# vga-group/tauray

Measured on AMD Instinct MI355X. Metric: Mray/s (closest-hit + shadow rays traced) @1920x1080, 4 bounces, 1 spp, higher is better.
Workload: dtype f32

## Files before the change

include/trhip.h:

```cpp
#ifndef TRHIP_H
#define TRHIP_H
#include <stddef.h>
#include <stdint.h>

#ifdef __cplusplus
extern "C" {
#endif

typedef struct trhip_device trhip_device;
typedef struct trhip_pt trhip_pt;

int trhip_device_create(int hip_device, trhip_device** out);
void trhip_device_destroy(trhip_device* dev);
const char* trhip_last_error(void);
int trhip_malloc(trhip_device* dev, size_t bytes, void** out);
int trhip_free(trhip_device* dev, void* ptr);
int trhip_upload(trhip_device* dev, void* dst_dev, const void* src_host, size_t bytes, void* stream);
int trhip_download(trhip_device* dev, void* dst_host, const void* src_dev, size_t bytes, void* stream);
int trhip_memset(trhip_device* dev, void* dst_dev, int value, size_t bytes, void* stream);
int trhip_sync(trhip_device* dev, void* stream);
int trhip_stream_create(trhip_device* dev, void** stream_out);
int trhip_stream_destroy(trhip_device* dev, void* stream);
int trhip_stream_wait(trhip_device* dev, void* stream, void* on);
int trhip_stream_pipe_class(trhip_device* dev, void* stream, int32_t* pipe_class_out);
// ... 139 lines not shown
    uint64_t stack_overflows;
} trhip_counters;

typedef struct trhip_timings {
    float path_tracing_ms;
    float trace_closest_ms, trace_shadow_ms, shade_ms, raygen_ms, resolve_ms;
    uint32_t trace_closest_launches, trace_shadow_launches, shade_launches, frames;
} trhip_timings;

int trhip_pt_create(trhip_device* dev, const trhip_pt_options* opt, trhip_pt** out);
int trhip_direct_create(trhip_device* dev, const trhip_pt_options* opt, trhip_pt** out);
void trhip_pt_destroy(trhip_pt* pt);
int trhip_pt_set_distribution(trhip_pt* pt, const trhip_distribution* dist);
int trhip_pt_reset_accumulation(trhip_pt* pt, int reset_sample_counter);
int trhip_pt_set_frame_counter(trhip_pt* pt, uint32_t frame_counter);
int trhip_pt_set_frame_batch(trhip_pt* pt, uint32_t frames);
int trhip_pt_set_lanes(trhip_pt* pt, int lanes);
int trhip_pt_set_frame_slots(trhip_pt* pt, int slots);
int trhip_pt_get_lane_pipes(trhip_pt* pt, int32_t* lanes_out, int32_t pipe_classes_out[4]);
int trhip_pt_set_shard(trhip_pt* pt, uint32_t viewport_base, uint32_t viewport_stride, uint32_t sample_base, uint32_t sample_stride);
int trhip_pt_render(trhip_pt* pt, void* color_dev, uint32_t target_w, uint32_t target_h, uint32_t viewports, void* stream);
typedef struct trhip_pt_targets {
    void* color;
    void* diffuse;
    void* reflection;
    void* albedo;
    void* material;
    void* normal;
    void* pos;
    void* instance_id;
    void* screen_motion;
} trhip_pt_targets;
int trhip_pt_render_targets(trhip_pt* pt, const trhip_pt_targets* targets, uint32_t target_w, uint32_t target_h, uint32_t viewports, void* stream);
int trhip_pt_set_shading_arithmetic(trhip_pt* pt, int ieee);
int trhip_pt_set_specialization(trhip_pt* pt, int enable);
int trhip_pt_precompile(const trhip_pt_options* opt, int shade_tris, int ieee, int count_work, const char* arch);
typedef struct trhip_program_info { int32_t kind, ieee; uint64_t identity; char key[240]; } trhip_program_info;
int trhip_pt_get_program(trhip_pt* pt, trhip_program_info* out);
uint64_t trhip_build_id(void);
const char* trhip_kernel_cache_dir(void);
int trhip_pt_set_profiling(trhip_pt* pt, int count_work, int detailed_timing);
int trhip_pt_get_counters(trhip_pt* pt, trhip_counters* out);
int trhip_pt_reset_counters(trhip_pt* pt);
int trhip_pt_get_timings(trhip_pt* pt, trhip_timings* out);
typedef struct trhip_phase_counters {
    uint64_t lane_node_phases, lane_tri_phases, quad_node_phases, quad_tri_phases;
    uint64_t lane_node_phases_le16, lane_node_visits_le16;
    uint64_t lane_node_phase_hist[8];
    uint64_t closest_node_visits;
} trhip_phase_counters;
int trhip_pt_get_phase_counters(trhip_pt* pt, trhip_phase_counters* out);
typedef struct trhip_light_counters { uint64_t sphere_tests, node_visits, walk_fallbacks; } trhip_light_counters;
int trhip_pt_get_light_counters(trhip_pt* pt, trhip_light_counters* out);
int trhip_calibrate_valu(trhip_device* dev, float* ginst_per_s);
int trhip_calibrate_l1(trhip_device* dev, float* gaccesses_per_s);

int trhip_feature_render(trhip_device* dev, int feature, const trhip_distribution* dist, int projection,
                         uint32_t viewport, float min_ray_dist, const float default_value[4],
                         void* color_dev, uint32_t target_w, uint32_t target_h, void* stream);

int trhip_trace_closest(trhip_device* dev, uint32_t n, const void* rays_dev, const void* seeds_dev,
                        int include_lights, void* hits_dev, void* stream);
int trhip_trace_shadow(trhip_device* dev, uint32_t n, const void* rays_dev, void* visibility_dev, void* stream);

int trhip_stitch(trhip_device* dev, const trhip_distribution* partial_dist, const void* partial_dev,
                 uint32_t partial_w, uint32_t partial_h, void* primary_dev, uint32_t viewports,
                 float blend_ratio, void* stream);
int trhip_stitch_batch(trhip_device* dev, uint32_t count, const trhip_distribution* partial_dists, const void* const* partials_dev,
                       const uint32_t* partial_ws, const uint32_t* partial_hs, void* primary_dev, uint32_t viewports,
                       float blend_ratio, void* stream);

typedef struct trhip_tonemap_info {
    int32_t op;
    float exposure, gamma;
    int32_t alpha_grid_background;
} trhip_tonemap_info;
int trhip_tonemap(trhip_device* dev, const void* in_dev, void* out_dev, uint32_t width, uint32_t height,
                  uint32_t layers, const trhip_tonemap_info* info, void* stream);
int trhip_pt_set_fused_tonemap(trhip_pt* pt, void* display_dev, const trhip_tonemap_info* info);

#ifdef __cplusplus
}
#endif
#endif
```

tauray_amd/_lib.py:

```python
from __future__ import annotations

import ctypes as C
import os

os.environ.setdefault("GPU_MAX_HW_QUEUES", "8")
os.environ.setdefault("HSA_ENABLE_IPC_MODE_LEGACY", "0")

_HERE = os.path.dirname(os.path.abspath(__file__))
LIB_PATH = os.environ.get("TRHIP_LIB", os.path.join(_HERE, "libtrhip.so"))


class TrhipError(RuntimeError):
    pass


class SceneDescC(C.Structure):
    _fields_ = [
        ("instances", C.c_void_p), ("spans", C.c_void_p), ("instance_count", C.c_uint32),
        ("vertices", C.c_void_p), ("vertex_count", C.c_uint32),
        ("indices", C.c_void_p), ("index_count", C.c_uint32),
        ("point_lights", C.c_void_p), ("point_light_count", C.c_uint32),
        ("directional_lights", C.c_void_p), ("directional_light_count", C.c_uint32),
        ("texture_infos", C.c_void_p), ("texture_count", C.c_uint32), ("texels", C.c_void_p),
        ("envmap", C.c_void_p), ("envmap_width", C.c_uint32), ("envmap_height", C.c_uint32),
        ("alias_table", C.c_void_p), ("environment_factor", C.c_float * 4),
        ("cameras", C.c_void_p), ("camera_count", C.c_uint32),
        ("non_opaque", C.c_void_p), ("gather_emissive_triangles", C.c_uint32)]


class AccelInfoC(C.Structure):
    _fields_ = [("triangle_count", C.c_uint32), ("node_count", C.c_uint32), ("tri_light_count", C.c_uint32),
                ("build_ms", C.c_float), ("bounds_min", C.c_float * 3), ("bounds_max", C.c_float * 3),
                ("node_bytes", C.c_uint32), ("leaf_count", C.c_uint32)]


class AccelLayoutC(C.Structure):
    _fields_ = [("strategy", C.c_int32), ("blas_count", C.c_uint32), ("tlas_leaf_count", C.c_uint32), ("blas_updated", C.c_uint32),
                ("node_bytes", C.c_uint64), ("record_bytes", C.c_uint64), ("blas_ms", C.c_float), ("tlas_ms", C.c_float)]


AS_ALL_MERGED, AS_PER_MESH, AS_STATIC_MERGED_DYNAMIC_PER_MESH = 0, 1, 2


class LightAccelInfoC(C.Structure):
    _fields_ = [("requested", C.c_int32), ("in_effect", C.c_int32), ("sphere_lights", C.c_uint32), ("tree_lights", C.c_uint32),
                ("node_count", C.c_uint32), ("auto_threshold", C.c_uint32), ("tree_bytes", C.c_uint64), ("last_ms", C.c_float),
                ("last_was_refit", C.c_int32)]


class LightCountersC(C.Structure):
    _fields_ = [("sphere_tests", C.c_uint64), ("node_visits", C.c_uint64), ("walk_fallbacks", C.c_uint64)]


LIGHT_ACCEL_AUTO, LIGHT_ACCEL_LOOP, LIGHT_ACCEL_TREE = 0, 1, 2


class PtOptionsC(C.Structure):
    _fields_ = [
        ("max_bounces", C.c_int32), ("min_ray_dist", C.c_float), ("rng_seed", C.c_uint32), ("sampler", C.c_int32),
        ("samples_per_pixel", C.c_int32), ("samples_per_pass", C.c_int32), ("projection", C.c_int32),
        ("film", C.c_int32), ("film_radius", C.c_float), ("mis_mode", C.c_int32),
        ("russian_roulette_delta", C.c_float), ("indirect_clamping", C.c_float), ("regularization_gamma", C.c_float),
        ("depth_of_field", C.c_int32), ("nee_point", C.c_float), ("nee_directional", C.c_float),
        ("nee_envmap", C.c_float), ("nee_triangles", C.c_float), ("bounce_mode", C.c_int32),
        ("tri_light_mode", C.c_int32), ("hide_lights", C.c_int32), ("use_white_albedo_on_first_bounce", C.c_int32),
        ("transparent_background", C.c_int32), ("pre_transformed_vertices", C.c_int32)]


class DistributionC(C.Structure):
    _fields_ = [("size_x", C.c_uint32), ("size_y", C.c_uint32), ("strategy", C.c_int32),
                ("index", C.c_uint32), ("count", C.c_uint32), ("primary", C.c_uint32)]


class CountersC(C.Structure):
    _fields_ = [(n, C.c_uint64) for n in ("closest_rays", "shadow_rays", "node_visits", "tri_tests", "alpha_tests",
                                          "surface_hits", "stack_overflows")]


class TimingsC(C.Structure):
    _fields_ = ([(n, C.c_float) for n in ("path_tracing_ms", "trace_closest_ms", "trace_shadow_ms", "shade_ms", "raygen_ms", "resolve_ms")]
                + [(n, C.c_uint32) for n in ("trace_closest_launches", "trace_shadow_launches", "shade_launches", "frames")])


class PhaseCountersC(C.Structure):
    _fields_ = ([(n, C.c_uint64) for n in ("lane_node_phases", "lane_tri_phases", "quad_node_phases", "quad_tri_phases",
                                           "lane_node_phases_le16", "lane_node_visits_le16")] + [("lane_node_phase_hist", C.c_uint64 * 8),
                                                                                                 ("closest_node_visits", C.c_uint64)])


class ProgramInfoC(C.Structure):
    _fields_ = [("kind", C.c_int32), ("ieee", C.c_int32), ("identity", C.c_uint64), ("key", C.c_char * 240)]


class PtTargetsC(C.Structure):
    _fields_ = [(n, C.c_void_p) for n in ("color", "diffuse", "reflection", "albedo", "material", "normal", "pos", "instance_id", "screen_motion")]


class TonemapInfoC(C.Structure):
    _fields_ = [("op", C.c_int32), ("exposure", C.c_float), ("gamma", C.c_float), ("alpha_grid_background", C.c_int32)]


_vp, _u32, _i, _f = C.c_void_p, C.c_uint32, C.c_int, C.c_float
SYMBOLS = {
    "trhip_image_decode": (_i, [_vp, C.c_size_t, C.POINTER(_u32), C.POINTER(_u32), C.POINTER(_u32), C.POINTER(C.POINTER(C.c_uint8))]),
    "trhip_image_free": (None, [C.POINTER(C.c_uint8)]),
    "trhip_exr_decode": (_i, [_vp, C.c_size_t, C.POINTER(_u32), C.POINTER(_u32), C.POINTER(_u32), C.POINTER(C.POINTER(C.c_float))]),
    "trhip_exr_encode": (_i, [_vp, _u32, _u32, _i, _i, _i, C.POINTER(C.POINTER(C.c_uint8)), C.POINTER(C.c_size_t)]),
    "trhip_exr_free": (None, [_vp]),
    "trhip_device_create": (_i, [_i, C.POINTER(_vp)]),
    "trhip_device_destroy": (None, [_vp]),
    "trhip_last_error": (C.c_char_p, []),
    "trhip_malloc": (_i, [_vp, C.c_size_t, C.POINTER(_vp)]),
    "trhip_image_decode_texels": (_i, [C.c_char_p, C.c_size_t, C.POINTER(C.c_uint32), C.POINTER(C.c_uint32), C.POINTER(C.c_uint32), C.POINTER(C.c_uint32), C.POINTER(C.POINTER(C.c_uint8))]),
    "trhip_free": (_i, [_vp, _vp]),
    "trhip_upload": (_i, [_vp, _vp, _vp, C.c_size_t, _vp]),
    "trhip_download": (_i, [_vp, _vp, _vp, C.c_size_t, _vp]),
    "trhip_memset": (_i, [_vp, _vp, _i, C.c_size_t, _vp]),
    "trhip_sync": (_i, [_vp, _vp]),
    "trhip_copy_peer": (_i, [_vp, _vp, _vp, _vp, C.c_size_t, _vp]),
    "trhip_scene_upload": (_i, [_vp, C.POINTER(SceneDescC)]),
    "trhip_scene_update_cameras": (_i, [_vp, _vp, _u32]),
    "trhip_scene_set_previous_cameras": (_i, [_vp, _vp, _u32]),
    "trhip_scene_update_instances": (_i, [_vp, _vp, _u32]),
    "trhip_scene_build_accel": (_i, [_vp, C.POINTER(AccelInfoC)]),
    "trhip_scene_refit_accel": (_i, [_vp, C.POINTER(AccelInfoC)]),
    "trhip_pt_set_frame_batch": (_i, [_vp, C.c_uint32]),
    "trhip_scene_update_lights": (_i, [_vp, _vp, C.c_uint32, _vp, C.c_uint32]),
    "trhip_scene_set_build_mode": (_i, [_vp, _i]),
    "trhip_scene_set_accel_strategy": (_i, [_vp, _i]),
    "trhip_scene_set_dynamic_instances": (_i, [_vp, _vp, _u32]),
    "trhip_scene_get_accel_layout": (_i, [_vp, C.POINTER(AccelLayoutC)]),
    "trhip_scene_set_light_accel": (_i, [_vp, _i]),
    "trhip_scene_get_light_accel": (_i, [_vp, C.POINTER(LightAccelInfoC)]),
    "trhip_pt_get_light_counters": (_i, [_vp, C.POINTER(LightCountersC)]),
    "trhip_stitch_batch": (_i, [_vp, _u32, _vp, _vp, _vp, _vp, _vp, _u32, C.c_float, _vp]),
    "trhip_stream_create": (_i, [_vp, C.POINTER(C.c_void_p)]),
    "trhip_stream_destroy": (_i, [_vp, _vp]),
    "trhip_stream_pipe_class": (_i, [_vp, _vp, C.POINTER(C.c_int32)]),
    "trhip_device_get_info": (_i, [_vp, _vp]),
    "trhip_build_id": (C.c_uint64, []),
    "trhip_stream_wait": (_i, [_vp, _vp, _vp]),
    "trhip_stream_wait_peer": (_i, [_vp, _vp, _vp, _vp]),
    "trhip_pt_set_frame_counter": (_i, [_vp, _u32]),
    "trhip_pt_set_lanes": (_i, [_vp, C.c_int]),
    "trhip_pt_set_frame_slots": (_i, [_vp, C.c_int]),
    "trhip_pt_set_fused_tonemap": (_i, [_vp, _vp, _vp]),
    "trhip_pt_get_lane_pipes": (_i, [_vp, C.POINTER(C.c_int32), C.POINTER(C.c_int32)]),
    "trhip_pt_set_shading_arithmetic": (_i, [_vp, C.c_int]),
    "trhip_pt_set_specialization": (_i, [_vp, C.c_int]),
    "trhip_pt_precompile": (_i, [C.POINTER(PtOptionsC), C.c_int, C.c_int, C.c_int, C.c_char_p]),
    "trhip_kernel_cache_dir": (C.c_char_p, []),
    "trhip_pt_set_shard": (_i, [_vp, _u32, _u32, _u32, _u32]),
    "trhip_scene_set_skin": (_i, [_vp, _u32, _vp, _vp, _u32]),
    "trhip_scene_skin": (_i, [_vp, _u32, _vp, _u32]),
    "trhip_scene_get_vertices": (_i, [_vp, _u32, _vp, _u32]),
    "trhip_scene_get_tri_lights": (_i, [_vp, _vp, _u32]),
    "trhip_pt_create": (_i, [_vp, C.POINTER(PtOptionsC), C.POINTER(_vp)]),
    "trhip_direct_create": (_i, [_vp, C.POINTER(PtOptionsC), C.POINTER(_vp)]),
    "trhip_pt_destroy": (None, [_vp]),
    "trhip_pt_set_distribution": (_i, [_vp, C.POINTER(DistributionC)]),
    "trhip_pt_reset_accumulation": (_i, [_vp, _i]),
    "trhip_pt_render": (_i, [_vp, _vp, _u32, _u32, _u32, _vp]),
    "trhip_pt_render_targets": (_i, [_vp, C.POINTER(PtTargetsC), _u32, _u32, _u32, _vp]),
    "trhip_pt_set_profiling": (_i, [_vp, _i, _i]),
    "trhip_pt_get_counters": (_i, [_vp, C.POINTER(CountersC)]),
    "trhip_pt_reset_counters": (_i, [_vp]),
    "trhip_pt_get_timings": (_i, [_vp, C.POINTER(TimingsC)]),
    "trhip_pt_get_phase_counters": (_i, [_vp, C.POINTER(PhaseCountersC)]),
    "trhip_pt_get_program": (_i, [_vp, C.POINTER(ProgramInfoC)]),
    "trhip_calibrate_valu": (_i, [_vp, C.POINTER(C.c_float)]),
    "trhip_calibrate_l1": (_i, [_vp, C.POINTER(C.c_float)]),
    "trhip_feature_render": (_i, [_vp, _i, C.POINTER(DistributionC), _i, _u32, _f, C.POINTER(_f), _vp, _u32, _u32, _vp]),
    "trhip_trace_closest": (_i, [_vp, _u32, _vp, _vp, _i, _vp, _vp]),
    "trhip_trace_shadow": (_i, [_vp, _u32, _vp, _vp, _vp]),
    "trhip_stitch": (_i, [_vp, C.POINTER(DistributionC), _vp, _u32, _u32, _vp, _u32, _f, _vp]),
    "trhip_tonemap": (_i, [_vp, _vp, _vp, _u32, _u32, _u32, C.POINTER(TonemapInfoC), _vp]),
}

_LIB = None


def lib():
    global _LIB
    if _LIB is None:
        if not os.path.exists(LIB_PATH):
            raise TrhipError(f"{LIB_PATH} is missing: build it with `make -C tauray_amd/csrc` (or __graft_entry__.build())")
        L = C.CDLL(LIB_PATH)
# ... 17 lines not shown
```

tauray_amd/csrc/api.hip:

```cpp
#include <cstdlib>
#include <cstring>
#include <mutex>
#include <string>
#include <vector>

#include "pt.h"
#include "trace.h"
#include "trace_quad.h"
#include "specialize.h"
#include "tonemap.h"
#include "../../include/tauray_image.hh"
#include "../../include/tauray_exr.hh"

namespace tr {

static thread_local std::string g_error;
int set_error(const std::string& msg) { g_error = msg; return 1; }

#define HIPCHK(x) do { hipError_t e_ = (x); if (e_ != hipSuccess) return set_error(std::string(#x) + ": " + hipGetErrorString(e_)); } while (0)

namespace {

constexpr int KB = TR_BLOCK;

// ... 72 lines not shown
            asm volatile("global_load_dwordx4 %0, %1, off" : "=v"(v[u]) : "v"(q) : "memory");
        }
        asm volatile("s_waitcnt vmcnt(0)" ::: "memory");
#pragma unroll
        for (int u = 0; u < 8; ++u) acc += v[u];
    }
    if (acc.x == 123.456f) out[0] = acc.y + acc.z + acc.w;
}

template <bool TWO_LEVEL>
__global__ __launch_bounds__(KB) void k_query_closest(SceneView sv, uint n, const float* rays, const uint* seeds, int include_lights,
                                                      HitRecord* out, uint* overflow_flag, int* qspill) {
    __shared__ int s_stack_rows[TR_STACK_WORDS];
    int* const s_stack = s_stack_rows + TR_STACK_ROW0;
    __shared__ int s_owner[(KB / 64) * TR_OWNER_WORDS];
    int* my_stack = s_stack + threadIdx.x;
    QuadCtx qc;
    qc.wave_stack = s_stack + (threadIdx.x & ~63u);
    qc.owner_tab = s_owner + (threadIdx.x >> 6) * TR_OWNER_WORDS;
    qc.spill = qspill + ((size_t)blockIdx.x * (KB / 64) + (threadIdx.x >> 6)) * (16u * TR_QSPILL);
    int overflow = 0;
    TraceStats st = {};
    for (uint base = blockIdx.x * KB; base < n; base += gridDim.x * KB) {
        const uint i = base + threadIdx.x;
        const bool valid = i < n;
        float r[8] = {0, 0, 0, 0, 0, 0, 0, 0};
        if (valid) for (int k = 0; k < 8; ++k) r[k] = rays[(size_t)i * 8 + k];
        const uint seed = (valid && seeds) ? seeds[i] : 0u;
        HitRecord hit;
#if TR_QUAD_SWITCH > 0
        if (seeds) trace_closest_wave4<0, false, TWO_LEVEL>(sv, valid, F3(r[0], r[1], r[2]), F3(r[4], r[5], r[6]), r[3], r[7], seed, my_stack, qc, hit, st, overflow);
        else trace_closest_wave4<1, false, TWO_LEVEL>(sv, valid, F3(r[0], r[1], r[2]), F3(r[4], r[5], r[6]), r[3], r[7], 0u, my_stack, qc, hit, st, overflow);
#else
        if (valid) {
            if (seeds) trace_closest4<0, false, TWO_LEVEL>(sv, F3(r[0], r[1], r[2]), F3(r[4], r[5], r[6]), r[3], r[7], seed, my_stack, hit, st, overflow);
            else trace_closest4<1, false, TWO_LEVEL>(sv, F3(r[0], r[1], r[2]), F3(r[4], r[5], r[6]), r[3], r[7], 0u, my_stack, hit, st, overflow);
        }
#endif
        if (valid) out[i] = hit;
        if (valid && include_lights) {
            const float tri_t = hit.instance_id >= 0 ? hit.t : r[7];
            uint ri = i;
            asm volatile("" : "+v"(ri));
            const float* q = rays + (size_t)ri * 8;
            const f3 o = F3(q[0], q[1], q[2]), d = F3(q[4], q[5], q[6]);
            if (ray_is_finite(o, d)) {
                const LightHit lh = trace_sphere_lights<false>(sv, o, d, q[3], tri_t, my_stack, st);
                if (lh.light >= 0) out[ri] = HitRecord{-1, lh.light, lh.t, 0.0f, lh.t};
            }
        }
    }
    if (overflow) *overflow_flag = 1;
}
template <bool TWO_LEVEL>
__global__ __launch_bounds__(KB) void k_query_shadow(SceneView sv, uint n, const float* rays, float* out, uint* overflow_flag) {
    __shared__ int s_stack_rows[TR_STACK_WORDS];
    int* const s_stack = s_stack_rows + TR_STACK_ROW0;
    int overflow = 0;
    TraceStats st = {};
    for (uint i = blockIdx.x * KB + threadIdx.x; i < n; i += gridDim.x * KB) {
        const float* r = rays + (size_t)i * 8;
        out[i] = trace_shadow4<false, TWO_LEVEL>(sv, F3(r[0], r[1], r[2]), F3(r[4], r[5], r[6]), r[3], r[7], s_stack + threadIdx.x, st, overflow);
    }
    if (overflow) *overflow_flag = 1;
}

__global__ __launch_bounds__(KB) void k_stitch(LaunchCtx L, const f4* partial, uint pw, uint ph, f4* primary, uint viewports, float blend_ratio) {
    uint per_view = L.strategy == 2 ? L.launch_w : pw * ph;
    uint i = blockIdx.x * KB + threadIdx.x;
    if (i >= per_view * viewports) return;
    uint z = i / per_view, p = i % per_view;
    uint sx, sy, ox, oy;
    if (L.strategy == 2) {
        uint j = permute_region_id(L.index + p, L.size_x, L.size_y, L.count);
        if (j >= L.size_x * L.size_y) return;
        sx = p % L.size_x; sy = p / L.size_x;
        ox = j % L.size_x; oy = j / L.size_x;
    } else {
        sx = p % pw; sy = p / pw;
        ox = sx; oy = sy * L.count + L.index;
        if (oy >= L.size_y) return;
    }
    f4 c = partial[((size_t)z * ph + sy) * pw + sx];
    size_t o = ((size_t)z * L.size_y + oy) * L.size_x + ox;
    if (blend_ratio < 1.0f) c = mix4(primary[o], c, blend_ratio);
    primary[o] = c;
}

#define TR_STITCH_BATCH 15
struct StitchBatch { LaunchCtx L[TR_STITCH_BATCH]; const f4* partial[TR_STITCH_BATCH]; uint pw[TR_STITCH_BATCH], ph[TR_STITCH_BATCH]; };
__global__ __launch_bounds__(KB) void k_stitch_batch(StitchBatch B, f4* primary, uint viewports, float blend_ratio) {
    const uint e = blockIdx.y;
    const LaunchCtx L = B.L[e];
    const uint pw = B.pw[e], ph = B.ph[e];
    const f4* partial = B.partial[e];
    uint per_view = L.strategy == 2 ? L.launch_w : pw * ph;
    uint i = blockIdx.x * KB + threadIdx.x;
    if (i >= per_view * viewports) return;
    uint z = i / per_view, p = i % per_view;
    uint sx, sy, ox, oy;
    if (L.strategy == 2) {
        uint j = permute_region_id(L.index + p, L.size_x, L.size_y, L.count);
        if (j >= L.size_x * L.size_y) return;
        sx = p % L.size_x; sy = p / L.size_x;
        ox = j % L.size_x; oy = j / L.size_x;
    } else {
// ... 573 lines not shown
    return 0;
}
int trhip_pt_set_fused_tonemap(trhip_pt* pt, void* display_dev, const trhip_tonemap_info* info) {
    if (!pt) return set_error("null trhip_pt");
    if (display_dev && !info) return set_error("trhip_pt_set_fused_tonemap: null info");
    if (display_dev && pt->stage->direct) return set_error("trhip_pt_set_fused_tonemap: the direct stage resolves its samples in a kernel of its own; run trhip_tonemap");
    pt->stage->tm_display = display_dev;
    if (info) { pt->stage->tm_info = *info; if (info->op == 0) pt->stage->tm_info.gamma = 1.0f; }
    return 0;
}
int trhip_pt_get_lane_pipes(trhip_pt* pt, int32_t* lanes_out, int32_t pipe_classes_out[4]) {
    if (!pt || !lanes_out || !pipe_classes_out) return set_error("trhip_pt_get_lane_pipes: null argument");
    *lanes_out = pt->stage->last_lanes;
    for (int l = 0; l < 4; ++l) pipe_classes_out[l] = l < pt->stage->last_lanes ? pt->stage->last_lane_pipes[l] : -1;
    return 0;
}
int trhip_pt_set_shading_arithmetic(trhip_pt* pt, int ieee) {
    if (!pt) return set_error("null trhip_pt");
    pt->stage->ieee_shading = ieee ? 1 : 0;
    return 0;
}
int trhip_pt_set_specialization(trhip_pt* pt, int enable) {
    if (!pt) return set_error("null trhip_pt");
    pt->stage->specialize = enable ? 1 : 0;
    return 0;
}
int trhip_pt_precompile(const trhip_pt_options* opt, int shade_tris, int ieee, int count_work, const char* arch) {
    if (!opt) return set_error("trhip_pt_precompile: null options");
    if (is_cli_default_set(*opt) && shade_tris) return 0;
    SpecRequest rq{*opt, shade_tris != 0 && !opt->pre_transformed_vertices, ieee != 0, count_work != 0, SPEC_SHADE, false};
    std::string why;
    for (int program : {SPEC_SHADE, SPEC_RAYGEN}) {
        rq.program = program;
        if (spec_precompile(rq, arch, &why)) return set_error("trhip_pt_precompile: " + why);
    }
    return 0;
}
const char* trhip_kernel_cache_dir(void) {
    static const std::string dir = spec_cache_dir();
    return dir.c_str();
}
int trhip_pt_set_profiling(trhip_pt* pt, int count_work, int detailed_timing) {
    if (!pt) return set_error("null trhip_pt");
    pt->stage->count_work = count_work; pt->stage->detailed_timing = detailed_timing;
    return 0;
}
int trhip_pt_get_counters(trhip_pt* pt, trhip_counters* out) { if (!pt) return set_error("null trhip_pt"); DEVCHK(pt->dev); return pt->stage->get_counters(out, pt->stage->last_stream); }
int trhip_pt_get_light_counters(trhip_pt* pt, trhip_light_counters* out) {
    if (!pt) return set_error("null trhip_pt");
    if (!out) return set_error("trhip_pt_get_light_counters: null output");
    DEVCHK(pt->dev);
    return pt->stage->get_light_counters(out, pt->stage->last_stream);
}
int trhip_pt_reset_counters(trhip_pt* pt) { if (!pt) return set_error("null trhip_pt"); DEVCHK(pt->dev); HIPCHK(hipStreamSynchronize(pt->stage->last_stream)); return pt->stage->reset_counters(); }
int trhip_pt_get_timings(trhip_pt* pt, trhip_timings* out) { if (!pt) return set_error("null trhip_pt"); DEVCHK(pt->dev); return pt->stage->get_timings(out); }
int trhip_pt_get_program(trhip_pt* pt, trhip_program_info* out) { if (!pt) return set_error("null trhip_pt"); if (!out) return set_error("trhip_pt_get_program: null out"); DEVCHK(pt->dev); return pt->stage->get_program(out); }
int trhip_pt_get_phase_counters(trhip_pt* pt, trhip_phase_counters* out) { if (!pt) return set_error("null trhip_pt"); DEVCHK(pt->dev); return pt->stage->get_phase_counters(out, pt->stage->last_stream); }

int trhip_calibrate_valu(trhip_device* dev, float* ginst_per_s) {
    DEVCHK(dev);
    if (!ginst_per_s) return set_error("trhip_calibrate_valu: null out");
    int cus = 256;
    HIPCHK(hipDeviceGetAttribute(&cus, hipDeviceAttributeMultiprocessorCount, dev->hip_device));
    const int blocks = cus * 8, iters = 4096;
    hipEvent_t a, b;
    HIPCHK(hipEventCreate(&a)); HIPCHK(hipEventCreate(&b));
    float best = 0.0f;
    for (int rep = 0; rep < 4; ++rep) {
        HIPCHK(hipEventRecord(a, nullptr));
        hipLaunchKernelGGL(k_calibrate_fma, dim3(blocks), dim3(KB), 0, nullptr, reinterpret_cast<float*>(dev->overflow_flag), iters, 1.0001f, 0.5f);
        HIPCHK(hipEventRecord(b, nullptr));
        HIPCHK(hipEventSynchronize(b));
        float ms = 0;
        HIPCHK(hipEventElapsedTime(&ms, a, b));
        const float g = (float)((double)blocks * (KB / 64) * (double)iters * 64.0 / ((double)ms * 1e6));
        if (rep > 0 && g > best) best = g;
    }
    (void)hipEventDestroy(a); (void)hipEventDestroy(b);
    *ginst_per_s = best;
    return 0;
}

int trhip_calibrate_l1(trhip_device* dev, float* gaccesses_per_s) {
    DEVCHK(dev);
    if (!gaccesses_per_s) return set_error("trhip_calibrate_l1: null out");
    int cus = 256;
    HIPCHK(hipDeviceGetAttribute(&cus, hipDeviceAttributeMultiprocessorCount, dev->hip_device));
    const int blocks = cus * 4, iters = 400;
    char* buf = nullptr;
    HIPCHK(hipMalloc(&buf, 16384 + 64));
    HIPCHK(hipMemset(buf, 0, 16384 + 64));
    hipEvent_t a, b;
    HIPCHK(hipEventCreate(&a)); HIPCHK(hipEventCreate(&b));
    float best = 0.0f;
    for (int rep = 0; rep < 4; ++rep) {
        HIPCHK(hipEventRecord(a, nullptr));
        hipLaunchKernelGGL(k_calibrate_l1, dim3(blocks), dim3(KB), 0, nullptr, buf, iters, reinterpret_cast<float*>(dev->overflow_flag));
        HIPCHK(hipEventRecord(b, nullptr));
        HIPCHK(hipEventSynchronize(b));
        float ms = 0;
        HIPCHK(hipEventElapsedTime(&ms, a, b));
        const float g = (float)((double)blocks * (KB / 64) * (double)iters * 8.0 * 64.0 / ((double)ms * 1e6));
        if (rep > 0 && g > best) best = g;
    }
    (void)hipEventDestroy(a); (void)hipEventDestroy(b);
    (void)hipFree(buf);
    *gaccesses_per_s = best;
    return 0;
}

static LaunchCtx make_launch(const trhip_distribution& d) {
    LaunchCtx L{};
    uint lw, lh;
    get_ray_count(d, lw, lh);
    L.size_x = d.size_x; L.size_y = d.size_y; L.strategy = d.strategy; L.index = d.index; L.primary = d.primary;
    L.count = d.count;
    if (d.strategy == 2) { uint n = d.size_x * d.size_y, b = 31; while ((n >> b) < 128 && b > 0) b--; L.count = b; }
    L.launch_w = lw; L.launch_h = lh;
    return L;
}

int trhip_feature_render(trhip_device* dev, int feature, const trhip_distribution* dist, int projection, uint32_t viewport,
                         float min_ray_dist, const float default_value[4], void* color_dev, uint32_t target_w, uint32_t target_h, void* stream) {
    DEVCHK(dev);
    if (!dev->scene.accel_built) return set_error("trhip_feature_render: call trhip_scene_build_accel first");
    if (viewport >= dev->scene.camera_count) return set_error("trhip_feature_render: viewport out of range");
    LaunchCtx L = make_launch(*dist);
    size_t n = (size_t)L.launch_w * L.launch_h;
    if (n == 0) return 0;
    f4 dv = F4(default_value[0], default_value[1], default_value[2], default_value[3]);
    hipLaunchKernelGGL(dev->scene.two_level ? k_feature<true> : k_feature<false>, dim3((uint)((n + KB - 1) / KB)), dim3(KB), 0, (hipStream_t)stream, dev->scene.view(), L, feature, projection,
                       viewport, min_ray_dist, dv, (f4*)color_dev, target_w, target_h, dev->overflow_flag);
    HIPCHK(hipGetLastError());
    return 0;
}

int trhip_trace_closest(trhip_device* dev, uint32_t n, const void* rays_dev, const void* seeds_dev, int include_lights, void* hits_dev, void* stream) {
    DEVCHK(dev);
    if (!dev->scene.accel_built) return set_error("trhip_trace_closest: call trhip_scene_build_accel first");
    if (n == 0) return 0;
    uint blocks = std::min((n + KB - 1) / KB, QUERY_BLOCKS);
    if (!dev->qspill) HIPCHK(hipMalloc(&dev->qspill, (size_t)QUERY_BLOCKS * (KB / 64) * 16u * TR_QSPILL * sizeof(int)));
    hipLaunchKernelGGL(dev->scene.two_level ? k_query_closest<true> : k_query_closest<false>, dim3(blocks), dim3(KB), 0, (hipStream_t)stream, dev->scene.view(), n, (const float*)rays_dev,
                       (const uint*)seeds_dev, include_lights, (HitRecord*)hits_dev, dev->overflow_flag, dev->qspill);
    HIPCHK(hipGetLastError());
    return 0;
}
int trhip_trace_shadow(trhip_device* dev, uint32_t n, const void* rays_dev, void* visibility_dev, void* stream) {
    DEVCHK(dev);
    if (!dev->scene.accel_built) return set_error("trhip_trace_shadow: call trhip_scene_build_accel first");
    if (n == 0) return 0;
    uint blocks = std::min((n + KB - 1) / KB, 2048u);
    hipLaunchKernelGGL(dev->scene.two_level ? k_query_shadow<true> : k_query_shadow<false>, dim3(blocks), dim3(KB), 0, (hipStream_t)stream, dev->scene.view(), n, (const float*)rays_dev,
                       (float*)visibility_dev, dev->overflow_flag);
    HIPCHK(hipGetLastError());
    return 0;
}

int trhip_stitch(trhip_device* dev, const trhip_distribution* pd, const void* partial_dev, uint32_t pw, uint32_t ph, void* primary_dev,
                 uint32_t viewports, float blend_ratio, void* stream) {
    DEVCHK(dev);
    if (!pd || pd->strategy == 0) return set_error("trhip_stitch: needs a scanline or shuffled-strips partial");
    LaunchCtx L = make_launch(*pd);
    size_t per_view = pd->strategy == 2 ? L.launch_w : (size_t)pw * ph;
    size_t n = per_view * viewports;
    if (n == 0) return 0;
    hipLaunchKernelGGL(k_stitch, dim3((uint)((n + KB - 1) / KB)), dim3(KB), 0, (hipStream_t)stream, L, (const f4*)partial_dev, pw, ph,
                       (f4*)primary_dev, viewports, blend_ratio);
    HIPCHK(hipGetLastError());
    return 0;
}

int trhip_stitch_batch(trhip_device* dev, uint32_t count, const trhip_distribution* pds, const void* const* partials_dev, const uint32_t* pws,
                       const uint32_t* phs, void* primary_dev, uint32_t viewports, float blend_ratio, void* stream) {
    DEVCHK(dev);
    if (count == 0) return 0;
    if (!pds || !partials_dev || !pws || !phs) return set_error("trhip_stitch_batch: null argument");
    for (uint32_t first = 0; first < count; first += TR_STITCH_BATCH) {
        const uint32_t m = std::min<uint32_t>(TR_STITCH_BATCH, count - first);
        StitchBatch B{};
        size_t n_max = 0;
        for (uint32_t k = 0; k < m; ++k) {
            const trhip_distribution& pd = pds[first + k];
            if (pd.strategy == 0) return set_error("trhip_stitch_batch: needs scanline or shuffled-strips partials");
            B.L[k] = make_launch(pd);
            B.partial[k] = (const f4*)partials_dev[first + k]; B.pw[k] = pws[first + k]; B.ph[k] = phs[first + k];
            const size_t per_view = pd.strategy == 2 ? B.L[k].launch_w : (size_t)B.pw[k] * B.ph[k];
            n_max = std::max(n_max, per_view * viewports);
        }
        if (n_max == 0) continue;
        hipLaunchKernelGGL(k_stitch_batch, dim3((uint)((n_max + KB - 1) / KB), m), dim3(KB), 0, (hipStream_t)stream, B, (f4*)primary_dev, viewports,
                           blend_ratio);
    }
    HIPCHK(hipGetLastError());
    return 0;
}

int trhip_tonemap(trhip_device* dev, const void* in_dev, void* out_dev, uint32_t width, uint32_t height, uint32_t layers,
                  const trhip_tonemap_info* info, void* stream) {
    DEVCHK(dev);
// ... 12 lines not shown
```

tauray_amd/csrc/build.h:

```cpp
#pragma once
#include <string>
#include <vector>

#include "common.h"
#include "shading.h"

namespace tr {

int set_error(const std::string& msg);

struct DeviceScene {
    Instance* instances = nullptr;
    MeshSpan* spans = nullptr;
    Vertex* vertices = nullptr;
    uint* indices = nullptr;
    PointLight* point_lights = nullptr;
    DirectionalLight* directional_lights = nullptr;
    TextureInfo* tex_infos = nullptr;
    uint8_t* texels = nullptr;
    f4* envmap = nullptr;
    AliasEntry* alias_table = nullptr;
    CameraData* cameras = nullptr;
    CameraData* prev_cameras = nullptr;
    uint8_t* non_opaque = nullptr;
// ... 22 lines not shown
    uint build_rounds = 0;
    int ploc_radius = 16;
    int optimise_rounds = 8;
    uint leaf_count = 0;
    uint accel_tri_count = 0;
    bool collapse_by_cost = true;
    bool fast_build = false;
    int optimise_modulus = 1;
    int dfs_layout = 1;
    bool accel_built = false;
    uint accel_capacity = 0xFFFFFFFFu;
    void* scratch = nullptr;
    float bounds_lo[3] = {0, 0, 0}, bounds_hi[3] = {0, 0, 0};
    uint* level_nodes = nullptr;
    float* node_bounds = nullptr;
    std::vector<uint> level_offsets;
    bool levels_valid = false;
    size_t scratch_bytes = 0;
    int accel_strategy = TRHIP_AS_ALL_MERGED;
    std::vector<uint8_t> dynamic_marks;
    std::vector<Instance> host_instances;
    struct Blas {
        int root;
        uint node_off, node_slots, tri_off, tri_count;
        uint rep;
        bool world;
    };
    std::vector<Blas> blases;
    std::vector<int> inst_blas;
    std::vector<uint> tlas_src;
    std::vector<uint8_t> blas_dirty;
    bool static_dirty = false;
    std::vector<uint8_t> alpha_dirty;
    uint* alpha_list = nullptr;
    size_t alpha_list_words = 0;
    bool two_level = false;
    TlasLeaf* tlas = nullptr;
    TlasLeaf* tlas_src_leaves = nullptr;
    uint tlas_leaf_count = 0, tlas_node_slots = 0, tlas_capacity = 0;
    size_t node_capacity = 0, tri_capacity = 0;
    trhip_accel_layout layout = {};
    std::vector<uint> host_alpha_base;
    std::vector<uint8_t> host_non_opaque;
    void* tl_aux = nullptr;
    size_t tl_aux_bytes = 0;
    int light_accel_requested = -1;
    int light_in_effect = TRHIP_LIGHT_ACCEL_LOOP;
    std::vector<PointLight> host_point_lights;
    std::vector<uint> light_tree_set;
    std::vector<Bvh4Node> light_nodes;
    uint light_tree_nodes = 0;
    float light_ms = 0.0f;
    int light_last_refit = -1;

    SceneView view() const {
        SceneView v;
        v.instances = instances; v.spans = spans; v.vertices = vertices; v.indices = indices;
        v.point_lights = point_lights; v.directional_lights = directional_lights; v.tri_lights = tri_lights;
        v.tex_infos = tex_infos; v.texels = texels; v.envmap = envmap; v.alias_table = alias_table;
        v.cameras = cameras; v.prev_cameras = prev_cameras ? prev_cameras : cameras; v.obj_spans = spans; v.obj_vertices = vertices; v.shade_tris = shade_tris; v.shade_tangents = shade_tangents; v.tris = tris; v.alpha_tris = alpha_tris; v.nodes4 = nodes4;
        v.environment_factor = environment_factor; v.environment_proj = environment_proj;
        v.instance_count = instance_count; v.point_light_count = point_light_count;
        v.directional_light_count = directional_light_count; v.tri_light_count = tri_light_count;
        v.env_w = env_w; v.env_h = env_h; v.wide_textures = wide_textures; v.tri_count = accel_built ? tri_count : 0; v.node_count = node_count;
        return v;
    }
    void free_accel() {
        if (nodes) (void)hipFree(nodes);
        if (nodes4) (void)hipFree(nodes4);
        if (tris) (void)hipFree(tris);
        if (tri_lights) (void)hipFree(tri_lights);
        if (tlas_src_leaves) (void)hipFree(tlas_src_leaves);
        if (tl_aux) (void)hipFree(tl_aux);
        tl_aux = nullptr; tl_aux_bytes = 0;
        if (alpha_list) (void)hipFree(alpha_list);
        alpha_list = nullptr; alpha_list_words = 0; alpha_dirty.clear();
        tlas = nullptr; tlas_src_leaves = nullptr; tlas_capacity = 0; node_capacity = 0; tri_capacity = 0; two_level = false;
        blases.clear(); inst_blas.clear(); tlas_src.clear(); blas_dirty.clear(); static_dirty = false;
        nodes = nullptr; nodes4 = nullptr; tris = nullptr; tri_lights = nullptr; node_count = 0; tri_light_count = 0; accel_built = false;
        accel_capacity = 0xFFFFFFFFu;
        if (level_nodes) (void)hipFree(level_nodes);
        if (node_bounds) (void)hipFree(node_bounds);
        level_nodes = nullptr; node_bounds = nullptr; level_offsets.clear(); levels_valid = false;
    }
    struct SkinSlot { Vertex* source = nullptr; Skin* skins = nullptr; m4* joints = nullptr; uint joint_capacity = 0; uint vertex_count = 0; };
    std::vector<SkinSlot> skin_slots;
    void free_skins() {
        for (SkinSlot& k : skin_slots) { if (k.source) (void)hipFree(k.source); if (k.skins) (void)hipFree(k.skins); if (k.joints) (void)hipFree(k.joints); }
        skin_slots.clear();
    }
    void free_all() {
        free_accel();
        free_skins();
        void* ptrs[] = {instances, spans, vertices, indices, point_lights, directional_lights, tex_infos, texels, envmap,
                        alias_table, cameras, prev_cameras, non_opaque, tri_prefix, world_spans, world_vertices, scratch, shade_tris, alpha_base, alpha_tris};
        for (void* p : ptrs) if (p) (void)hipFree(p);
        const int strategy = accel_strategy, light_mode = light_accel_requested;
        *this = DeviceScene();
        accel_strategy = strategy;
        light_accel_requested = light_mode;
    }
};

int build_accel(DeviceScene& ds, hipStream_t stream, trhip_accel_info* info);
int ensure_world_vertices(DeviceScene& ds, hipStream_t stream);
int build_shade_tris(DeviceScene& ds, int instance, hipStream_t stream);
int skin_instance(DeviceScene& ds, uint instance, const float* joint_transforms, uint joint_count, hipStream_t stream);
int refit_accel(DeviceScene& ds, hipStream_t stream, trhip_accel_info* info);
void mark_skinned(DeviceScene& ds, uint instance);
int update_light_accel(DeviceScene& ds, bool moved);
uint light_accel_auto_threshold();
int light_accel_requested(const DeviceScene& ds);

}
```

tauray_amd/csrc/bvh_build.hip:

```cpp
#include <algorithm>
#include <cctype>
#include <chrono>
#include <cmath>
#include <map>
#include <tuple>
#include <vector>
#include "build.h"

#include <rocprim/rocprim.hpp>

namespace tr {

namespace {

constexpr int BT = 256;

TR_DEV uint float_flip(float f) { uint u = __float_as_uint(f); return (u & 0x80000000u) ? ~u : (u | 0x80000000u); }
TR_HD float float_unflip(uint u) {
    uint v = (u & 0x80000000u) ? (u & 0x7FFFFFFFu) : ~u;
    float f;
#if defined(__HIP_DEVICE_COMPILE__)
    f = __uint_as_float(v);
#else
    memcpy(&f, &v, 4);
// ... 378 lines not shown
    if (dec) ncand = collapse_children(children, dec, (int)i, cand);
    while (!dec && ncand < W) {
        int best = -1; float best_area = -1.0f;
        for (int c = 0; c < ncand; ++c) {
            if (cand[c] < 0) continue;
            const float* b = node_box + 6 * (size_t)cand[c];
            float dx = b[3] - b[0], dy = b[4] - b[1], dz = b[5] - b[2];
            float area = dx * dy + dy * dz + dz * dx;
            if (area > best_area) { best_area = area; best = c; }
        }
        if (best < 0) break;
        const int2 ch = children[cand[best]];
        cand[best] = ch.x; cand[ncand++] = ch.y;
    }
    Bvh4Node out;
    for (int c = 0; c < 4; ++c) {
        if (c < ncand) {
            const float* b = cand[c] >= 0 ? node_box + 6 * (size_t)cand[c] : leaf_box + 6 * (size_t)(~cand[c]);
            out.lox[c] = b[0]; out.loy[c] = b[1]; out.loz[c] = b[2]; out.hix[c] = b[3]; out.hiy[c] = b[4]; out.hiz[c] = b[5];
            out.child[c] = cand[c] >= 0 ? new_id[cand[c]] : cand[c];
        } else {
            out.lox[c] = out.loy[c] = out.loz[c] = __builtin_huge_valf();
            out.hix[c] = out.hiy[c] = out.hiz[c] = -__builtin_huge_valf();
            out.child[c] = 0x7FFFFFFF;
        }
        out.pad[c] = 0;
    }
    nodes4[(size_t)new_id[i]] = out;
}

__global__ __launch_bounds__(BT) void k_extract_tri_lights(SceneView sv, const uint* tri_prefix, TriLight* out) {
    uint gid = blockIdx.x * BT + threadIdx.x;
    if (gid >= sv.tri_count) return;
    uint inst, prim;
    locate_triangle(tri_prefix, sv.instance_count, gid, inst, prim);
    const Instance& o = sv.instances[inst];
    if (o.light_base_id < 0) return;
    const MeshSpan sp = sv.spans[inst];
    const uint* ix = sv.indices + sp.index_offset + 3u * prim;
    const Vertex* vb = sv.vertices + sp.vertex_offset;
    const Vertex v0 = vb[ix[0]], v1 = vb[ix[1]], v2 = vb[ix[2]];
    TriLight l;
    l.emission_tex_id = o.mat.emission_tex_id;
    l.emission_factor = rgb_to_r9g9b9e5(F3(o.mat.emission_factor));
    l.instance_id = inst;
    l.primitive_id = prim;
    l.pos[0] = transform_point(o.model, v0.pos);
    l.pos[1] = transform_point(o.model, v1.pos);
    l.pos[2] = transform_point(o.model, v2.pos);
    l.uv[0] = pack_half2x16(v0.uv); l.uv[1] = pack_half2x16(v1.uv); l.uv[2] = pack_half2x16(v2.uv);
    out[(uint)o.light_base_id + prim] = l;
}

#define HIPCHK(x) do { hipError_t e_ = (x); if (e_ != hipSuccess) return set_error(std::string(#x) + ": " + hipGetErrorString(e_)); } while (0)

}

__global__ __launch_bounds__(BT) void k_pre_transform_vertices(uint vertex_count, const Instance* instance, const Vertex* in, Vertex* out) {
    uint i = blockIdx.x * BT + threadIdx.x;
    if (i >= vertex_count) return;
    const m4 model = instance->model;
    const m3 mn = upper3(instance->model_normal);
    const float det = mn.c[0].x * (mn.c[1].y * mn.c[2].z - mn.c[2].y * mn.c[1].z)
                    - mn.c[1].x * (mn.c[0].y * mn.c[2].z - mn.c[2].y * mn.c[0].z)
                    + mn.c[2].x * (mn.c[0].y * mn.c[1].z - mn.c[1].y * mn.c[0].z);
    Vertex v = in[i];
    v.pos = transform_point(model, v.pos);
    v.normal = normalize(mul(mn, v.normal));
    f3 t = normalize(mul(mn, F3(v.tangent)));
    v.tangent = F4(t, v.tangent.w);
    if (det < 0) { v.normal = -v.normal; v.tangent = F4(-t.x, -t.y, -t.z, -v.tangent.w); }
    out[i] = v;
}

int ensure_world_vertices(DeviceScene& ds, hipStream_t stream) {
    if (ds.world_vertices || ds.world_vertex_count == 0) return 0;
    HIPCHK(hipMalloc(&ds.world_vertices, (size_t)ds.world_vertex_count * sizeof(Vertex)));
    for (uint i = 0; i < ds.instance_count; ++i) {
        const MeshSpan& sp = ds.host_spans[i];
        if (sp.vertex_count == 0) continue;
        hipLaunchKernelGGL(k_pre_transform_vertices, dim3((sp.vertex_count + BT - 1) / BT), dim3(BT), 0, stream, sp.vertex_count, ds.instances + i,
                           ds.vertices + sp.vertex_offset, ds.world_vertices + ds.host_world_spans[i].vertex_offset);
    }
    HIPCHK(hipGetLastError());
    return 0;
}

__global__ __launch_bounds__(BT) void k_skinning(uint vertex_count, const Vertex* source, const Skin* skins, const m4* joints, uint joint_count, Vertex* destination) {
    uint i = blockIdx.x * BT + threadIdx.x;
    if (i >= vertex_count) return;
    const Skin s = skins[i];
    float a[4][4];
    for (int c = 0; c < 4; ++c) {
        f4 col = F4(0);
        for (int k = 0; k < 4; ++k) {
            const uint j = s.joints[k] < joint_count ? s.joints[k] : 0u;
            const f4 t = joints[j].c[c] * s.weights[k];
            col = k == 0 ? t : col + t;
        }
        a[0][c] = col.x; a[1][c] = col.y; a[2][c] = col.z; a[3][c] = col.w;
    }
    const float s0 = a[0][0] * a[1][1] - a[1][0] * a[0][1], s1 = a[0][0] * a[1][2] - a[1][0] * a[0][2], s2 = a[0][0] * a[1][3] - a[1][0] * a[0][3];
    const float s3 = a[0][1] * a[1][2] - a[1][1] * a[0][2], s4 = a[0][1] * a[1][3] - a[1][1] * a[0][3], s5 = a[0][2] * a[1][3] - a[1][2] * a[0][3];
    const float c5 = a[2][2] * a[3][3] - a[3][2] * a[2][3], c4 = a[2][1] * a[3][3] - a[3][1] * a[2][3], c3 = a[2][1] * a[3][2] - a[3][1] * a[2][2];
    const float c2 = a[2][0] * a[3][3] - a[3][0] * a[2][3], c1 = a[2][0] * a[3][2] - a[3][0] * a[2][2], c0 = a[2][0] * a[3][1] - a[3][0] * a[2][1];
    const float det = s0 * c5 - s1 * c4 + s2 * c3 + s3 * c2 - s4 * c1 + s5 * c0;
    float inv[3][3];
    inv[0][0] = ( a[1][1] * c5 - a[1][2] * c4 + a[1][3] * c3) / det;
    inv[0][1] = (-a[0][1] * c5 + a[0][2] * c4 - a[0][3] * c3) / det;
    inv[0][2] = ( a[3][1] * s5 - a[3][2] * s4 + a[3][3] * s3) / det;
    inv[1][0] = (-a[1][0] * c5 + a[1][2] * c2 - a[1][3] * c1) / det;
    inv[1][1] = ( a[0][0] * c5 - a[0][2] * c2 + a[0][3] * c1) / det;
    inv[1][2] = (-a[3][0] * s5 + a[3][2] * s2 - a[3][3] * s1) / det;
    inv[2][0] = ( a[1][0] * c4 - a[1][1] * c2 + a[1][3] * c0) / det;
    inv[2][1] = (-a[0][0] * c4 + a[0][1] * c2 - a[0][3] * c0) / det;
    inv[2][2] = ( a[3][0] * s4 - a[3][1] * s2 + a[3][3] * s0) / det;
    const Vertex src = source[i];
    Vertex dst = src;
    dst.pos = F3(a[0][0] * src.pos.x + a[0][1] * src.pos.y + a[0][2] * src.pos.z + a[0][3],
                 a[1][0] * src.pos.x + a[1][1] * src.pos.y + a[1][2] * src.pos.z + a[1][3],
                 a[2][0] * src.pos.x + a[2][1] * src.pos.y + a[2][2] * src.pos.z + a[2][3]);
    const f3 n = src.normal, t = F3(src.tangent);
    dst.normal = normalize(F3(inv[0][0] * n.x + inv[1][0] * n.y + inv[2][0] * n.z + 0.0f, inv[0][1] * n.x + inv[1][1] * n.y + inv[2][1] * n.z + 0.0f,
                              inv[0][2] * n.x + inv[1][2] * n.y + inv[2][2] * n.z + 0.0f));
    const f3 tt = normalize(F3(inv[0][0] * t.x + inv[1][0] * t.y + inv[2][0] * t.z + 0.0f, inv[0][1] * t.x + inv[1][1] * t.y + inv[2][1] * t.z + 0.0f,
// ... 144 lines not shown
int refit_accel(DeviceScene& ds, hipStream_t stream, trhip_accel_info* info) {
    if (ds.two_level) {
        if (ds.accel_tri_count != ds.tri_count || ds.tlas_capacity != ds.tlas_leaf_count)
            return set_error("trhip_scene_refit_accel: no acceleration structure to refit; call trhip_scene_build_accel first");
        return refit_two_level(ds, stream, info);
    }
    const uint n = ds.leaf_count;
    if (ds.accel_tri_count != ds.tri_count || ds.accel_capacity == 0xFFFFFFFFu || (n > 0 && !ds.tris) || (n > 1 && !ds.nodes4))
        return set_error("trhip_scene_refit_accel: no acceleration structure to refit; call trhip_scene_build_accel first");
    hipEvent_t e0, e1;
    HIPCHK(hipEventCreate(&e0)); HIPCHK(hipEventCreate(&e1));
    HIPCHK(hipEventRecord(e0, stream));
    SceneView sv = ds.view();
    const uint n1 = ds.node_count;
    if (n1 > 0 && !ds.levels_valid) {
        if (!ds.level_nodes) HIPCHK(hipMalloc(&ds.level_nodes, (size_t)n1 * 4));
        if (!ds.node_bounds) HIPCHK(hipMalloc(&ds.node_bounds, (size_t)n1 * 24));
        uint* counter = nullptr;
        HIPCHK(hipMalloc(&counter, 4));
        const uint root = 0;
        HIPCHK(hipMemcpyAsync(ds.level_nodes, &root, 4, hipMemcpyHostToDevice, stream));
        ds.level_offsets.assign(1, 0u);
        uint begin = 0, count = 1;
        while (count > 0) {
            ds.level_offsets.push_back(begin + count);
            if (begin + count >= n1) break;
            HIPCHK(hipMemsetAsync(counter, 0, 4, stream));
            hipLaunchKernelGGL(k_expand_level, dim3((count + BT - 1) / BT), dim3(BT), 0, stream, count, ds.level_nodes + begin, ds.nodes4,
                               ds.level_nodes + begin + count, counter);
            uint next = 0;
            HIPCHK(hipMemcpyAsync(&next, counter, 4, hipMemcpyDeviceToHost, stream));
            HIPCHK(hipStreamSynchronize(stream));
            begin += count; count = next;
            if (ds.level_offsets.size() > 4096) { (void)hipFree(counter); return set_error("trhip_scene_refit_accel: hierarchy too deep"); }
        }
        (void)hipFree(counter);
        ds.levels_valid = true;
        if (getenv("TRHIP_DEBUG"))
            fprintf(stderr, "[trhip] 4-wide tree: %u live nodes of %u slots in %zu levels, %.3f children per node\n", ds.level_offsets.back(), n1,
                    ds.level_offsets.size() - 1, (double)(n + ds.level_offsets.back() - 1) / (double)ds.level_offsets.back());
    }
    if (n > 0) hipLaunchKernelGGL(k_retransform, dim3((n + BT - 1) / BT), dim3(BT), 0, stream, sv, n, ds.tris, ds.alpha_base, ds.alpha_tris);
    for (size_t l = ds.level_offsets.size(); l-- > 1;) {
        const uint lo = ds.level_offsets[l - 1], cnt = ds.level_offsets[l] - lo;
        if (cnt) hipLaunchKernelGGL(k_refit_level, dim3((cnt + BT - 1) / BT), dim3(BT), 0, stream, cnt, ds.level_nodes + lo, ds.nodes4, ds.tris, ds.node_bounds);
    }
    HIPCHK(hipGetLastError());
    ds.accel_built = true;
    if (ds.gather_emissive_triangles && ds.host_tri_light_count > 0 && ds.tri_lights) {
        HIPCHK(hipMemsetAsync(ds.tri_lights, 0, (size_t)ds.host_tri_light_count * sizeof(TriLight), stream));
        SceneView sv2 = ds.view();
        hipLaunchKernelGGL(k_extract_tri_lights, dim3((ds.tri_count + BT - 1) / BT), dim3(BT), 0, stream, sv2, ds.tri_prefix, ds.tri_lights);
    }
    HIPCHK(hipEventRecord(e1, stream));
    HIPCHK(hipEventSynchronize(e1));
    float ms = 0;
    HIPCHK(hipEventElapsedTime(&ms, e0, e1));
    (void)hipEventDestroy(e0); (void)hipEventDestroy(e1);
    ds.layout.blas_updated = 1; ds.layout.blas_ms = ms;
    if (info) {
        memset(info, 0, sizeof(*info));
        info->triangle_count = ds.tri_count; info->leaf_count = n; info->node_count = ds.node_count; info->node_bytes = 112u; info->tri_light_count = ds.tri_light_count;
        info->build_ms = ms;
        for (int k = 0; k < 3; ++k) { info->bounds_min[k] = ds.bounds_lo[k]; info->bounds_max[k] = ds.bounds_hi[k]; }
    }
    return 0;
}

static int reorder_into_treelets(DeviceScene& ds, hipStream_t stream, uint n_nodes, uint n_tris, uint treelet_nodes, bool reorder_tris) {
    if (n_nodes == 0 || n_tris == 0) return 0;
    HIPCHK(hipStreamSynchronize(stream));
    std::vector<Bvh4Node> nodes(n_nodes), out_nodes;
    std::vector<TriRecord> tris(n_tris), out_tris;
    HIPCHK(hipMemcpy(nodes.data(), ds.nodes4, (size_t)n_nodes * sizeof(Bvh4Node), hipMemcpyDeviceToHost));
    HIPCHK(hipMemcpy(tris.data(), ds.tris, (size_t)n_tris * sizeof(TriRecord), hipMemcpyDeviceToHost));
    std::vector<int> new_id(n_nodes, -1);
    std::vector<uint> order;
    order.reserve(n_nodes);
    std::vector<uint> roots = {0u};
    auto area = [&](const Bvh4Node& nd, int c) {
        const float dx = nd.hix[c] - nd.lox[c], dy = nd.hiy[c] - nd.loy[c], dz = nd.hiz[c] - nd.loz[c];
        return dx * dy + dy * dz + dz * dx;
    };
    std::vector<std::pair<float, uint>> heap;
    while (!roots.empty()) {
        const uint root = roots.back(); roots.pop_back();
        heap.clear();
        heap.push_back({__builtin_huge_valf(), root});
        uint taken = 0;
        std::vector<uint> rest;
        while (!heap.empty()) {
            std::pop_heap(heap.begin(), heap.end());
            const uint nd = heap.back().second; heap.pop_back();
            if (taken >= treelet_nodes) { rest.push_back(nd); continue; }
            new_id[nd] = (int)order.size(); order.push_back(nd); taken++;
            for (int c = 0; c < 4; ++c) {
                const int ch = nodes[nd].child[c];
                if (ch >= 0 && ch != 0x7FFFFFFF) { heap.push_back({area(nodes[nd], c), (uint)ch}); std::push_heap(heap.begin(), heap.end()); }
            }
        }
        for (size_t k = rest.size(); k-- > 0;) roots.push_back(rest[k]);
    }
    out_nodes.resize(n_nodes);
    std::vector<int> new_tri(n_tris, -1);
    uint next_tri = 0;
    for (size_t k = 0; k < order.size(); ++k) {
// ... 289 lines not shown
                const uint8_t* dec = nullptr;
                if (dp_collapse) {
                    OptTree t{(uint)(n - 1), n, children, node_box, leaf_box, reinterpret_cast<int*>(base + o_uparent)};
                    if (!optimise) hipLaunchKernelGGL(k_opt_parents, dim3(iblocks), dim3(BT), 0, stream, t);
                    HIPCHK(hipMemsetAsync(arrive, 0, (size_t)(n - 1) * 4, stream));
                    hipLaunchKernelGGL(k_collapse_cost, dim3(blocks), dim3(BT), 0, stream, t, arrive, reinterpret_cast<float*>(base + o_ccost), reinterpret_cast<uint8_t*>(base + o_cdec));
                    dec = reinterpret_cast<const uint8_t*>(base + o_cdec);
                }
                hipLaunchKernelGGL(k_collapse4, dim3(iblocks), dim3(BT), 0, stream, n - 1, children, node_box, leaf_box, new_id, dec, out_nodes);
            }
        }
        HIPCHK(hipGetLastError());
        if (experiments && getenv("TRHIP_PAIR_LEAVES") && atoi(getenv("TRHIP_PAIR_LEAVES")) != 0 && n > 2) {
#if TR_PAIR_LEAVES
            if (int rc = pair_leaves_postpass(ds, stream, n - 1, n)) return rc;
#else
            return set_error("TRHIP_PAIR_LEAVES needs a library built with -DTR_PAIR_LEAVES=1 (the traversal has to know the pair references)");
#endif
        }
        if (const char* e = experiments ? getenv("TRHIP_TREELET") : nullptr) {
            if (n > 2 && atoi(e) > 0) if (int rc = reorder_into_treelets(ds, stream, n - 1, n, (uint)atoi(e), !getenv("TRHIP_TREELET_KEEP_TRIS"))) return rc;
        }
    }
    return 0;
}

static int build_two_level(DeviceScene& ds, hipStream_t stream, trhip_accel_info* info);
static int refit_two_level(DeviceScene& ds, hipStream_t stream, trhip_accel_info* info);

int build_accel(DeviceScene& ds, hipStream_t stream, trhip_accel_info* info) {
    if (ds.accel_strategy != TRHIP_AS_ALL_MERGED) return build_two_level(ds, stream, info);
    const uint n_scene = ds.tri_count;
    hipEvent_t e0, e1;
    HIPCHK(hipEventCreate(&e0)); HIPCHK(hipEventCreate(&e1));
    HIPCHK(hipEventRecord(e0, stream));
    ds.accel_built = false;
    ds.levels_valid = false;
    SceneView sv = ds.view();
    sv.tri_count = n_scene;
    const uint n_tri = n_scene;
    const uint n_cap = n_tri;
    uint n = n_tri;
    const size_t n1 = n_cap > 1 ? n_cap - 1 : 0;
    if (ds.two_level) ds.free_accel();
    TreePlan P;
    if (int rc = plan_tree(ds, stream, n_cap, P)) return rc;
    uint* cbounds = P.cbounds();
    {
        const uint init[32] = {0xFFFFFFFFu, 0xFFFFFFFFu, 0xFFFFFFFFu, 0, 0, 0, 0, 0, 0, 0, 0, 0, 0, 0, 0, 0, 0xFFFFFFFFu, 0xFFFFFFFFu, 0xFFFFFFFFu, 0, 0, 0, 0, 0, 0, 0, 0, 0, 0, 0, 0, 0};
        HIPCHK(hipMemcpyAsync(cbounds, init, sizeof(init), hipMemcpyHostToDevice, stream));
    }
    if (ds.accel_capacity != n_cap) {
        ds.free_accel();
        if (n_cap > 0) HIPCHK(hipMalloc(&ds.tris, (size_t)n_cap * sizeof(TriRecord)));
        if (n1 > 0) {
            if ((uint64_t)n1 * sizeof(Bvh4Node) > 0xFFFFFFFFull) return set_error("trhip_scene_build_accel: more than 2^25 nodes");
            HIPCHK(hipMalloc(&ds.nodes4, n1 * sizeof(Bvh4Node)));
        }
        ds.accel_capacity = n_cap;
    }
    if (n_tri > 0) {
        TriRecord* unsorted = P.unsorted();
        const uint tblocks = (n_tri + BT - 1) / BT;
        hipLaunchKernelGGL(k_pretransform, dim3(tblocks < 1024u ? tblocks : 1024u), dim3(BT), 0, stream, sv, ds.tri_prefix, ds.non_opaque, ds.alpha_base, ds.alpha_tris, unsorted, cbounds);
    }
    if (int rc = build_tree(ds, stream, P, n, ds.tris, ds.nodes4, true)) return rc;
    ds.leaf_count = n;
    ds.node_count = n > 1 ? n - 1 : 0;
    ds.accel_tri_count = n_tri;
    ds.accel_built = true;
    ds.tri_light_count = 0;
    if (ds.gather_emissive_triangles && ds.host_tri_light_count > 0) {
        if (!ds.tri_lights) HIPCHK(hipMalloc(&ds.tri_lights, (size_t)ds.host_tri_light_count * sizeof(TriLight)));
        HIPCHK(hipMemsetAsync(ds.tri_lights, 0, (size_t)ds.host_tri_light_count * sizeof(TriLight), stream));
        ds.tri_light_count = ds.host_tri_light_count;
        SceneView sv2 = ds.view();
        hipLaunchKernelGGL(k_extract_tri_lights, dim3((n_tri + BT - 1) / BT), dim3(BT), 0, stream, sv2, ds.tri_prefix, ds.tri_lights);
        HIPCHK(hipGetLastError());
    }
    HIPCHK(hipEventRecord(e1, stream));
    HIPCHK(hipEventSynchronize(e1));
    float ms = 0;
    HIPCHK(hipEventElapsedTime(&ms, e0, e1));
    (void)hipEventDestroy(e0); (void)hipEventDestroy(e1);
    uint hb[6];
    HIPCHK(hipMemcpy(hb, cbounds, sizeof(hb), hipMemcpyDeviceToHost));
    for (int k = 0; k < 3; ++k) { ds.bounds_lo[k] = float_unflip(hb[k]); ds.bounds_hi[k] = float_unflip(hb[3 + k]); }
    ds.layout = {};
    ds.layout.strategy = TRHIP_AS_ALL_MERGED; ds.layout.blas_count = 1; ds.layout.blas_updated = 1;
    ds.layout.node_bytes = (uint64_t)ds.node_count * sizeof(Bvh4Node); ds.layout.record_bytes = (uint64_t)n * sizeof(TriRecord);
    ds.layout.blas_ms = ms;
    if (info) {
        info->triangle_count = n_tri;
        info->leaf_count = n;
        info->node_count = ds.node_count;
        info->node_bytes = 112u;
        info->tri_light_count = ds.tri_light_count;
        info->build_ms = ms;
        for (int k = 0; k < 3; ++k) { info->bounds_min[k] = float_unflip(hb[k]); info->bounds_max[k] = float_unflip(hb[3 + k]); }
    }
    return 0;
}

namespace {

__global__ __launch_bounds__(BT) void k_group_records(SceneView sv, const uint* list, const uint* prefix, uint n_list, uint n, int world,
                                                      const uint8_t* non_opaque, const uint* alpha_base, AlphaTri* alpha_tris, TriRecord* out) {
    const uint gid = blockIdx.x * BT + threadIdx.x;
    if (gid >= n) return;
    uint slot, prim;
    locate_triangle(prefix, n_list, gid, slot, prim);
    const uint inst = list[slot];
    const MeshSpan sp = sv.obj_spans[inst];
    const uint* ix = sv.indices + sp.index_offset + 3u * prim;
    const Vertex* vb = sv.obj_vertices + sp.vertex_offset;
    f3 p0 = vb[ix[0]].pos, p1 = vb[ix[1]].pos, p2 = vb[ix[2]].pos;
    TriRecord t;
    if (world) {
        const m4 model = sv.instances[inst].model;
        p0 = transform_point(model, p0); p1 = transform_point(model, p1); p2 = transform_point(model, p2);
        t.inst_flags = inst | (non_opaque[inst] ? 0x80000000u : 0u);
        t.alpha = non_opaque[inst] ? alpha_word(sv.instances[inst].mat, alpha_base[inst] + prim, alpha_tris, vb[ix[0]].uv, vb[ix[1]].uv, vb[ix[2]].uv) : 0u;
    } else {
        t.inst_flags = inst;
        t.alpha = 0u;
    }
    t.prim = prim;
    t.v0[0] = p0.x; t.v0[1] = p0.y; t.v0[2] = p0.z;
    t.v1[0] = p1.x; t.v1[1] = p1.y; t.v1[2] = p1.z;
    t.v2[0] = p2.x; t.v2[1] = p2.y; t.v2[2] = p2.z;
    out[gid] = t;
}
// ... 615 lines not shown
```

tauray_amd/csrc/common.h:

```cpp
#pragma once
#include <hip/hip_runtime.h>
#include <hip/hip_fp16.h>
#include <stdint.h>
#include <string.h>
#include <cstring>

#include "../../include/trhip.h"

#define TR_DEV __device__ __forceinline__
#define TR_HD __host__ __device__ __forceinline__

namespace tr {

typedef uint32_t uint;

struct f2 { float x, y; };
struct f3 { float x, y, z; };
struct f4 { float x, y, z, w; };
struct u4 { uint x, y, z, w; };
struct u2 { uint x, y; };

TR_HD f2 F2(float a, float b) { return {a, b}; }
TR_HD f2 F2(float a) { return {a, a}; }
TR_HD f3 F3(float a, float b, float c) { return {a, b, c}; }
// ... 132 lines not shown
#define TR_INST_FROM_RECORD 0xFFFFFFFFu
#define TR_TLAS_IDENTITY 1u
struct alignas(64) TlasLeaf {
    float xf[12];
    int blas_root;
    uint inst_word;
    uint alpha_base;
    uint flags;
};
static_assert(sizeof(TlasLeaf) == 64, "TLAS leaf layout");

struct SceneView {
    const Instance* instances;
    const MeshSpan* spans;
    const Vertex* vertices;
    const uint* indices;
    const PointLight* point_lights;
    const DirectionalLight* directional_lights;
    const TriLight* tri_lights;
    const TextureInfo* tex_infos;
    const uint8_t* texels;
    const f4* envmap;
    const AliasEntry* alias_table;
    const CameraData* cameras;
    const CameraData* prev_cameras;
    const MeshSpan* obj_spans;
    const Vertex* obj_vertices;
    const ShadeTri* shade_tris;
    const f4* shade_tangents;
    const TriRecord* tris;
    const AlphaTri* alpha_tris;
    const Bvh4Node* nodes4;
    f4 environment_factor;
    int environment_proj;
    uint instance_count, point_light_count, directional_light_count, tri_light_count;
    uint env_w, env_h;
    uint tri_count, node_count;
    uint wide_textures;
};
TR_HD const TlasLeaf* tlas_leaves(const SceneView& sv) { return reinterpret_cast<const TlasLeaf*>(sv.nodes4 + sv.node_count); }

#define TR_LIGHT_KAPPA 0.001953125f
struct alignas(16) LightTreeHeader { uint use_tree, node_count, leaf_count, pad; };
static_assert(sizeof(LightTreeHeader) == 16, "light tree header layout");
TR_HD size_t light_tree_node_offset(uint point_light_count) { return ((size_t)point_light_count * sizeof(PointLight) + sizeof(LightTreeHeader) + 127) & ~(size_t)127; }
TR_HD size_t light_allocation_bytes(uint point_light_count) {
    return light_tree_node_offset(point_light_count) + (size_t)(point_light_count > 1 ? point_light_count - 1 : 1) * sizeof(Bvh4Node);
}
TR_HD const LightTreeHeader* light_tree_header(const SceneView& sv) { return reinterpret_cast<const LightTreeHeader*>(sv.point_lights + sv.point_light_count); }
TR_HD const Bvh4Node* light_tree_nodes(const SceneView& sv) {
    return reinterpret_cast<const Bvh4Node*>(reinterpret_cast<const char*>(sv.point_lights) + light_tree_node_offset(sv.point_light_count));
}

}
```

tauray_amd/csrc/path_tracer.hip:

```cpp
#include <cstdio>
#include <cstdlib>
#include <type_traits>
#include <vector>

#include "pt_kernels.h"
#include "resolve_kernel.h"
#include "specialize.h"
#include "build_id.inc"

namespace tr {

namespace {

#ifndef TR_CLOSEST_WAVES
#define TR_CLOSEST_WAVES 6
#endif
#ifndef TR_SHADOW_WAVES
#define TR_SHADOW_WAVES 8
#endif
#ifndef TR_CLOSEST_WAVES_2L
#define TR_CLOSEST_WAVES_2L 5
#endif
#ifndef TR_SHADOW_WAVES_2L
#define TR_SHADOW_WAVES_2L 6
#endif

template <bool COUNT, bool SOLO, bool WIDE = true, bool TWO_LEVEL = false>
__global__ __launch_bounds__(KB, TWO_LEVEL ? TR_CLOSEST_WAVES_2L : TR_CLOSEST_WAVES) void k_trace_closest(SceneView sv, PtParams P, PathBuffers pb, int bounce, const uint* queue,
                                                      uint* bc) {
    if (!WIDE) sv.wide_textures = 0;
    __shared__ int s_stack_rows[TR_STACK_WORDS];
    int* const s_stack = s_stack_rows + TR_STACK_ROW0;
    __shared__ int s_owner[(KB / 64) * TR_OWNER_WORDS];
    TL(__shared__ uint s_tl[(KB / 64) * TL_WORDS]; for (uint i = threadIdx.x; i < (KB / 64) * TL_WORDS; i += KB) s_tl[i] = 0; __syncthreads();)
    const QuadCtx qc = make_quad_ctx(s_stack, s_owner, pb TL(, s_tl));
    const uint n = queue ? bc[BC_QUEUE] : P.n_ids;
    TraceStats st = {};
    uint rays = 0, max_vis = 0;
    int overflow = 0;
    const uint wave_id = (blockIdx.x * KB + threadIdx.x) >> 6, n_waves = (gridDim.x * KB) >> 6;
    bool first = true;
    while (true) {
        uint base = 0;
        if (first) base = wave_id * 64u;
        else {
            if (n <= n_waves * 64u) break;
            if ((threadIdx.x & 63) == 0) base = n_waves * 64u + atomicAdd(&bc[BC_CUR_CLOSEST], 64u);
            base = __shfl(base, 0);
        }
        first = false;
        if (base >= n) break;
        closest_lane<COUNT, TWO_LEVEL>(sv, P, pb, bounce, queue, base + (threadIdx.x & 63), n, s_stack + threadIdx.x, qc, st, overflow, max_vis, rays);
    }
    flush_trace_counters<COUNT>(P, pb, overflow, 1000 + bounce, rays, 0u, st, max_vis);
    TL(__syncthreads(); for (uint i = threadIdx.x; i < (KB / 64) * TL_WORDS; i += KB) if (s_tl[i]) atomicAdd(&g_timeline[i % TL_WORDS], (unsigned long long)s_tl[i]);)
}

template <bool COUNT, bool WIDE = true, bool TWO_LEVEL = false>
__global__ __launch_bounds__(KB, TWO_LEVEL ? TR_SHADOW_WAVES_2L : TR_SHADOW_WAVES) void k_trace_shadow(SceneView sv, PtParams P, PathBuffers pb, uint* bc) {
    if (!WIDE) sv.wide_textures = 0;
    __shared__ int s_stack_rows[TR_STACK_WORDS];
    int* const s_stack = s_stack_rows + TR_STACK_ROW0;
    __shared__ int s_owner[(KB / 64) * TR_OWNER_WORDS];
    const QuadCtx qc = make_quad_ctx(s_stack, s_owner, pb);
    const uint n = bc[BC_SHADOW];
    TraceStats st = {};
    uint rays = 0;
    int overflow = 0;
    const uint wave_id = (blockIdx.x * KB + threadIdx.x) >> 6, n_waves = (gridDim.x * KB) >> 6;
    bool first = true;
    while (true) {
// ... 15 lines not shown
#define TR_TAIL_PIECES 0
#endif
#ifndef TR_TAIL16_DIV
#define TR_TAIL16_DIV 8
#endif
#ifndef TR_TAIL32_DIV
#define TR_TAIL32_DIV 8
#endif
template <bool WIDE, bool TWO_LEVEL = false>
__global__ __launch_bounds__(KB, TWO_LEVEL ? TR_CLOSEST_WAVES_2L : TR_CLOSEST_WAVES) void k_trace_fused(SceneView sv, PtParams P, PathBuffers pb, int bounce, const uint* queue,
                                                                      uint* bc, uint* bc_prev) {
    if (!WIDE) sv.wide_textures = 0;
    __shared__ int s_stack_rows[TR_STACK_WORDS];
    int* const s_stack = s_stack_rows + TR_STACK_ROW0;
    __shared__ int s_owner[(KB / 64) * TR_OWNER_WORDS];
    const QuadCtx qc = make_quad_ctx(s_stack, s_owner, pb);
    const uint nc = bc[BC_QUEUE], ns = bc_prev[BC_SHADOW];
    const uint chunks_c = (nc + 63u) >> 6, total = chunks_c + ((ns + 63u) >> 6);
    TraceStats st = {};
    uint closest_rays = 0, shadow_rays = 0, max_vis = 0;
    int overflow = 0;
    const uint wave_id = (blockIdx.x * KB + threadIdx.x) >> 6, n_waves = (gridDim.x * KB) >> 6;
#if TR_TAIL_PIECES
    const uint dyn = total > n_waves ? total - n_waves : 0u;
    const uint tail16 = dyn < n_waves / TR_TAIL16_DIV ? dyn : n_waves / TR_TAIL16_DIV;
    const uint tail32 = dyn - tail16 < n_waves / TR_TAIL32_DIV ? dyn - tail16 : n_waves / TR_TAIL32_DIV;
    const uint full = total - tail16 - tail32, pieces = full + 2u * tail32 + 4u * tail16;
#else
    const uint pieces = total;
#endif
    bool first = true;
    while (true) {
        uint p = 0;
        if (first) p = wave_id;
        else {
            if (pieces <= n_waves) break;
            if ((threadIdx.x & 63) == 0) p = n_waves + atomicAdd(&bc[BC_CUR_CLOSEST], 1u);
            p = __shfl(p, 0);
        }
        first = false;
        if (p >= pieces) break;
        uint g = p, off = 0u, size = 64u;
#if TR_TAIL_PIECES
        if (p >= full) {
            const uint q = p - full;
            if (q < 2u * tail32) { g = full + (q >> 1); off = (q & 1u) << 5; size = 32u; }
            else { const uint r = q - 2u * tail32; g = full + tail32 + (r >> 2); off = (r & 3u) << 4; size = 16u; }
        }
#endif
        const uint lane = threadIdx.x & 63;
        const uint slot = lane < size ? off + lane : 0xFFFFFFFFu;
        if (g < chunks_c) closest_lane<false, TWO_LEVEL>(sv, P, pb, bounce, queue, slot == 0xFFFFFFFFu ? slot : (g << 6) + slot, nc, s_stack + threadIdx.x, qc, st, overflow, max_vis, closest_rays);
        else shadow_lane<false, TWO_LEVEL>(sv, P, pb, slot == 0xFFFFFFFFu ? slot : ((g - chunks_c) << 6) + slot, ns, s_stack + threadIdx.x, qc, st, overflow, shadow_rays);
    }
    flush_trace_counters<false>(P, pb, overflow, 3000 + bounce, closest_rays, shadow_rays, st, max_vis);
}


TR_DEV void write_first_hit_gbuffer(const SceneView& sv, const PtParams& P, uint launch_id, const SurfacePoint& v, const SampledMaterial& mat, bool surface,
                                    int4 h) {
    if (P.samples_accumulated + P.previous_samples != 0) return;
    if (!(P.T.albedo || P.T.material || P.T.normal || P.T.pos || P.T.instance_id || P.T.screen_motion)) return;
    uint lx, ly, lz;
    launch_coord(P.L, launch_id, lx, ly, lz);
    int wx, wy;
    if (!get_write_pixel_pos(P.L, lx, ly, wx, wy) || (uint)wx >= P.target_w || (uint)wy >= P.target_h) return;
    const size_t pix = ((size_t)lz * P.target_h + (uint)wy) * P.target_w + (uint)wx;
    if (P.T.albedo) reinterpret_cast<f4*>(P.T.albedo)[pix] = mat.albedo;
    if (P.T.material)
        reinterpret_cast<f4*>(P.T.material)[pix] = F4(mat.metallic, mat.roughness, (mat.ior_out / mat.ior_in) * 0.25f, mat.transmittance);
    if (P.T.normal) {
        f3 nn = v.mapped_normal / (fabsf(v.mapped_normal.x) + fabsf(v.mapped_normal.y) + fabsf(v.mapped_normal.z));
        f2 o = nn.z >= 0.0f ? F2(nn.x, nn.y)
                            : F2((1 - fabsf(nn.y)) * ((nn.x >= 0.0f ? 1.0f : 0.0f) * 2 - 1), (1 - fabsf(nn.x)) * ((nn.y >= 0.0f ? 1.0f : 0.0f) * 2 - 1));
        reinterpret_cast<f2*>(P.T.normal)[pix] = o;
    }
    if (P.T.pos) reinterpret_cast<f4*>(P.T.pos)[pix] = F4(v.pos, 0);
    if (P.T.instance_id) reinterpret_cast<int*>(P.T.instance_id)[pix] = surface ? h.x : -1;
    if (P.T.screen_motion) {
        const f3 prev_pos = surface ? surface_prev_pos(sv, h.x, h.y, __int_as_float(h.z), __int_as_float(h.w)) : v.pos;
        const f3 m = get_camera_projection(sv.prev_cameras[global_viewport(P, lz)], P.opt.projection, prev_pos);
        reinterpret_cast<f2*>(P.T.screen_motion)[pix] = F2(m.x, m.y);
    }
}

__global__ __launch_bounds__(KB) void k_first_hit_gbuffer(SceneView sv, PtParams P, PathBuffers pb) {
    uint i = blockIdx.x * KB + threadIdx.x;
    if (i >= P.n_ids) return;
    const uint id = i + P.id_offset;
    const u4 misc = pb.misc[id];
    if (misc.w & 1u) return;
    const int4 h = pb.hit[id];
    uint lx, ly, lz;
    launch_coord(P.L, misc.z, lx, ly, lz);
    int px, py;
    if (!get_pixel_pos(P.L, lx, ly, px, py)) return;
    LocalSampler ls = init_local_sampler(u4{(uint)px, (uint)py, global_viewport(P, lz), P.rng_sample}, sample_counter_of(P, lz), P.rng_seed, P.opt.sampler);
    f2 cam_offset = F2(0.0f);
    if (P.opt.film != 0) {
        f4 r = u4_to_unit(pcg4d(ls.rs));
        if (P.opt.film == 1) cam_offset = F2(r.x, r.y) * 2.0f - 1.0f;
        else cam_offset = sample_blackman_harris_concentric_disk(F2(r.x, r.y)) * 2.0f;
        cam_offset = cam_offset * (2.0f * P.opt.film_radius);
    }
    f2 dof_u = F2(0.5f);
    if (P.opt.depth_of_field) { f4 r = u4_to_unit(pcg4d(ls.rs)); dof_u = F2(r.x, r.y); }
// ... 368 lines not shown
    if (frame_batch > 1 && (accumulated_samples != 0 || direct)) return set_error("trhip_pt_render: a frame batch renders independent frames of the path tracer (reset the accumulation first)");
    if (opt.samples_per_pass <= 0 || opt.samples_per_pixel % opt.samples_per_pass != 0)
        return set_error("trhip_pt_render: samples_per_pixel must be a multiple of samples_per_pass");
    if (dist.size_x == 0 || dist.size_y == 0) return set_error("trhip_pt_render: distribution not set");
    PtParams P{};
    P.opt = opt;
    uint lw, lh;
    get_ray_count(dist, lw, lh);
    P.L.size_x = dist.size_x; P.L.size_y = dist.size_y; P.L.strategy = dist.strategy; P.L.index = dist.index;
    P.L.count = dist.strategy == 2 ? calculate_shuffled_strips_b(dist.size_x, dist.size_y) : dist.count;
    P.L.primary = dist.primary; P.L.launch_w = lw; P.L.launch_h = lh;
    P.viewports = viewports;
    const size_t n = (size_t)lw * lh * viewports;
    if (n == 0) return 0;
    if (n > 0xFFFFFFF0ull) return set_error("trhip_pt_render: launch too large");
    P.n_launch = (uint)n; P.id_offset = 0; P.n_ids = (uint)n;
    P.max_sobol_bounces = (uint)(opt.max_bounces > 8 ? 8 : opt.max_bounces);
    P.sample_counter = frame_counter * (uint)opt.samples_per_pixel * shard_sample_stride;
    P.vp_base = shard_vp_base; P.vp_stride = shard_vp_stride;
    P.frame_views = frame_views; P.frame_counter_step = (uint)opt.samples_per_pixel * shard_sample_stride;
    { uint s = opt.rng_seed; P.rng_seed = s != 0 ? pcg(s) : 0; }
    P.samples_accumulated = accumulated_samples;
    P.target_w = target_w; P.target_h = target_h;
    P.nee_point = opt.nee_point > 0; P.nee_dir = opt.nee_directional > 0; P.nee_env = opt.nee_envmap > 0; P.nee_tri = opt.nee_triangles > 0;
    {
        float point = (P.nee_point && scene->point_light_count > 0) ? opt.nee_point : 0.0f;
        float tri = (P.nee_tri && scene->tri_light_count > 0) ? opt.nee_triangles : 0.0f;
        float dir = (P.nee_dir && scene->directional_light_count > 0) ? opt.nee_directional : 0.0f;
        float env = (P.nee_env && scene->environment_proj >= 0) ? opt.nee_envmap : 0.0f;
        float sum = point + tri + dir + env;
        float inv_sum = sum <= 0.0f ? 0.0f : (1.0f / sum + 1e-5f);
        P.prob_point = point * inv_sum; P.prob_tri = tri * inv_sum; P.prob_dir = dir * inv_sum; P.prob_env = env * inv_sum;
    }
    P.count_work = 1;
    P.bounce_words = (uint)BC_STRIDE * ((uint)opt.max_bounces + 2u);
    P.fused_resolve = opt.samples_per_pass == 1;
    P.T = targets;
    P.tm_display = nullptr; P.tm_op = tm_info.op; P.tm_exposure = tm_info.exposure; P.tm_gamma = tm_info.gamma; P.tm_grid = tm_info.alpha_grid_background;
    const bool timing = detailed_timing != 0;
    static const bool sample_lanes_enabled = !(getenv("TRHIP_SAMPLE_LANES") && atoi(getenv("TRHIP_SAMPLE_LANES")) == 0);
    const int passes_total = opt.samples_per_pixel / opt.samples_per_pass;
    const int sample_lane_count = std::min(passes_total, PT_LANES);
    const bool sample_lanes = sample_lanes_enabled && !direct && !timing && lanes == 0 && opt.samples_per_pass == 1 && passes_total >= 2 &&
                              n * (size_t)sample_lane_count * 224u <= ((size_t)8 << 30);
    if (int rc = ensure_buffers(sample_lanes ? n * (size_t)sample_lane_count : n, targets.diffuse || targets.reflection)) return rc;
    PathBuffers& pb = impl->pb;
    SceneView sv = scene->view();
    if (opt.pre_transformed_vertices) {
        if (int rc = ensure_world_vertices(*scene, stream)) return rc;
        sv.vertices = scene->world_vertices; sv.spans = scene->world_spans;
    }
    const bool count = count_work != 0;
    const bool two_level = scene->two_level;
    const Program prog = choose_program();
    const bool wide = prog.wide, cli_set = prog.cli_set, shade_fast = prog.shade_fast;
    const SpecKernels *spec_shade = prog.shade, *spec_raygen = prog.raygen;
    auto launch_raygen = [&](uint blocks, hipStream_t on, const PtParams& LP, const PathBuffers& lb) {
        if (spec_raygen) {
            SceneView a0 = sv; PtParams a1 = LP; PathBuffers a2 = lb;
            void* args[] = {&a0, &a1, &a2};
            (void)hipModuleLaunchKernel(spec_raygen->raygen, blocks, 1, 1, KB, 1, 1, 0, on, args, nullptr);
        } else hipLaunchKernelGGL(k_raygen<SpecGeneral>, dim3(blocks), dim3(KB), 0, on, sv, LP, lb);
    };
    auto launch_shade = [&](bool count, bool last, uint blocks, hipStream_t on, const PtParams& LP, const PathBuffers& lb, int bounce, const uint* q, uint* bc, uint* qn) {
        if (spec_shade) {
            SceneView a0 = sv; PtParams a1 = LP; PathBuffers a2 = lb;
            void* args[] = {&a0, &a1, &a2, &bounce, &q, &bc, &qn};
            (void)hipModuleLaunchKernel(last ? spec_shade->shade_last : spec_shade->shade, blocks, 1, 1, KB, 1, 1, 0, on, args, nullptr);
        } else if (shade_fast) launch_shade_fast(cli_set, count, last, blocks, on, sv, LP, lb, bounce, q, bc, qn);
        else if (last) {
            if (count) hipLaunchKernelGGL((k_shade<true, true>), dim3(blocks), dim3(KB), 0, on, sv, LP, lb, bounce, q, bc, qn);
            else if (cli_set) hipLaunchKernelGGL((k_shade<false, true, SpecCli>), dim3(blocks), dim3(KB), 0, on, sv, LP, lb, bounce, q, bc, qn);
            else hipLaunchKernelGGL((k_shade<false, true>), dim3(blocks), dim3(KB), 0, on, sv, LP, lb, bounce, q, bc, qn);
        }
        else if (count) hipLaunchKernelGGL((k_shade<true, false>), dim3(blocks), dim3(KB), 0, on, sv, LP, lb, bounce, q, bc, qn);
        else if (cli_set) hipLaunchKernelGGL((k_shade<false, false, SpecCli>), dim3(blocks), dim3(KB), 0, on, sv, LP, lb, bounce, q, bc, qn);
        else hipLaunchKernelGGL((k_shade<false, false>), dim3(blocks), dim3(KB), 0, on, sv, LP, lb, bounce, q, bc, qn);
    };
    static const int lanes_env = getenv("TRHIP_LANES") ? atoi(getenv("TRHIP_LANES")) : PT_LANES;
    static const bool overlap_enabled = !(getenv("TRHIP_OVERLAP") && atoi(getenv("TRHIP_OVERLAP")) == 0);
    static const size_t lanes_min_paths = getenv("TRHIP_LANES_MIN_PATHS") ? (size_t)atol(getenv("TRHIP_LANES_MIN_PATHS")) : (size_t)100000;
    static const size_t slots2_min_paths = getenv("TRHIP_SLOTS2_MIN_PATHS") ? (size_t)atol(getenv("TRHIP_SLOTS2_MIN_PATHS")) : (size_t)50000;
    const int auto_lanes = frame_slots >= 3 ? 1
                         : frame_slots == 2 ? (n < slots2_min_paths ? 1 : std::min(lanes_env, 2))
                         : (n < lanes_min_paths ? 1 : std::max(1, std::min(n < 2 * lanes_min_paths ? std::min(lanes_env, 2) : lanes_env, PT_LANES)));
    const int n_lanes = sample_lanes ? sample_lane_count : (timing ? 1 : (lanes > 0 ? std::min(lanes, PT_LANES) : auto_lanes));
    static const bool fused_enabled = !(getenv("TRHIP_FUSED") && atoi(getenv("TRHIP_FUSED")) == 0);
    const bool first_hit_targets = targets.albedo || targets.material || targets.normal || targets.pos || targets.instance_id || targets.screen_motion;
    const bool fused = fused_enabled && !timing && !count;
    const bool overlap = overlap_enabled && !timing && !fused && n_lanes == 1;
    if (!direct && (overlap || n_lanes > 1)) {
        int main_cls = -1;
        if (stream == last_main && impl->main_cls >= 0) main_cls = impl->main_cls;
        else if (stream != last_main || impl->main_tries < 16) {
            (void)stream_pool_class(stream, &main_cls, false);
            impl->main_tries = stream != last_main ? 1 : impl->main_tries + 1;
        }
        const bool main_changed = stream != last_main || main_cls != impl->main_cls;
        impl->main_cls = main_cls;
        if (main_changed && main_cls >= 0 && impl->side) {
            bool collide = false;
            for (int l = 1; l < PT_LANES; ++l) {
                hipStream_t ls = l == 1 ? impl->side : impl->lane_stream[l];
                int c = -1;
                if (ls && stream_pool_class(ls, &c, false) == 0 && c == main_cls) collide = true;
            }
// ... 114 lines not shown
    struct LaneCtx { hipStream_t ls; PtParams LP; PathBuffers lb; uint blocks_all, blocks_q, blocks_f; bool shadow_in_flight; };
    LaneCtx lane_ctx[PT_LANES * 4];
    int lanes_used = 0;
    for (int slice = 0; slice < n_slices; ++slice) {
        const int lane = slice % n_lanes;
        LaneCtx& c = lane_ctx[slice];
        c.ls = lane == 0 ? stream : (lane == 1 ? impl->side : impl->lane_stream[lane]);
        c.LP = P;
        c.LP.id_offset = sample_lanes ? 0u : (uint)slice * per_lane;
        if (c.LP.id_offset >= n) break;
        c.LP.n_ids = std::min(per_lane, (uint)n - c.LP.id_offset);
        PathBuffers& lb = c.lb;
        lb = pb;
        lb.counters = pb.counters + lane * CNT_WORDS;
        lb.bounce = pb.bounce + (size_t)lane * P.bounce_words;
        lb.qspill = pb.qspill + (size_t)lane * impl->qspill_lane_words;
        const size_t q0 = sample_lanes ? (size_t)lane * n : (size_t)c.LP.id_offset;
        lb.queue[0] = pb.queue[0] + q0; lb.queue[1] = pb.queue[1] + q0;
        lb.sh_org_tmax = pb.sh_org_tmax + q0; lb.sh_dir_id = pb.sh_dir_id + q0;
        lb.sh_contrib = pb.sh_contrib + q0; lb.sh_lobes = pb.sh_lobes + q0;
        if (sample_lanes) {
            const size_t o = (size_t)lane * n;
            lb.org_pdf += o; lb.dir_reg += o; lb.atten_alpha += o; lb.diffuse += o; lb.reflection += o; lb.plobes += o; lb.first_mat += o; lb.first_emis += o;
            lb.rng += o; lb.misc += o; lb.hit += o;
        }
        c.blocks_all = (c.LP.n_ids + KB - 1) / KB;
        c.blocks_q = c.blocks_all < grid_cap ? c.blocks_all : grid_cap;
        c.blocks_f = std::min(grid_cap, c.blocks_all * fused_grid_factor());
        c.shadow_in_flight = false;
        lanes_used = slice + 1;
    }
    const int passes = passes_total;
    bool merged_raygen = false;
    auto enqueue_pass = [&](int lane, int pass, int only) -> int {
        LaneCtx& c = lane_ctx[lane];
        const hipStream_t ls = c.ls;
        PtParams& LP = c.LP;
        PathBuffers& lb = c.lb;
        const uint blocks_all = c.blocks_all, blocks_q = c.blocks_q, blocks_f = c.blocks_f;
        bool& shadow_in_flight = c.shadow_in_flight;
        {
            LP.previous_samples = (uint)pass * (uint)opt.samples_per_pass;
            for (int s = 0; s < opt.samples_per_pass; ++s) {
                LP.sample_in_pass = (uint)s;
                LP.rng_sample = shard_sample_base + shard_sample_stride * (LP.previous_samples + LP.sample_in_pass);
                if ((only == -2 || only == -1) && !merged_raygen) timed(T_RAYGEN, ls, [&] {
                    launch_raygen(blocks_all, ls, LP, lb);
                });
                for (int bounce = 0; bounce < opt.max_bounces; ++bounce) {
                    if (only != -2 && only != bounce) continue;
                    const uint* q = bounce == 0 ? nullptr : lb.queue[bounce & 1];
                    uint* qn = lb.queue[(bounce + 1) & 1];
                    uint* bc = lb.bounce + BC_STRIDE * bounce;
                    if (fused && bounce > 0) {
                        hipLaunchKernelGGL((two_level ? k_trace_fused<true, true> : (wide ? k_trace_fused<true> : k_trace_fused<false>)), dim3(blocks_f), dim3(KB), 0, ls, sv, LP, lb, bounce, q, bc, bc - BC_STRIDE);
                    } else {
                        timed(T_CLOSEST, ls, [&] {
                            auto kc = two_level ? (count ? k_trace_closest<true, false, true, true> : k_trace_closest<false, false, true, true>)
                                    : count ? k_trace_closest<true, false> : (timing ? (wide ? k_trace_closest<false, true, true> : k_trace_closest<false, true, false>)
                                                                                     : (wide ? k_trace_closest<false, false, true> : k_trace_closest<false, false, false>));
                            hipLaunchKernelGGL(kc, dim3(std::min(blocks_all, closest_cap)), dim3(KB), 0, ls, sv, LP, lb, bounce, q, bc);
                        });
                    }
                    if (shadow_in_flight) { HIPCHK(hipStreamWaitEvent(ls, impl->ev_join, 0)); shadow_in_flight = false; }
                    timed(T_SHADE, ls, [&] {
#if TR_SHADE_NOLOOP
                        const uint blocks_s = blocks_all;
#else
                        static const uint shade_cap_env = getenv("TRHIP_SHADE_BLOCKS") ? (uint)atoi(getenv("TRHIP_SHADE_BLOCKS")) : 0u;
                        const uint shade_cap = shade_cap_env ? shade_cap_env : ((pixel_lanes || (n_lanes == 2 && frame_slots == 2)) ? 768u : 2048u);
                        const uint blocks_s = timing ? blocks_q : (blocks_all < shade_cap ? blocks_all : shade_cap);
#endif
                        static const bool last_variant = !(getenv("TRHIP_SHADE_LAST") && atoi(getenv("TRHIP_SHADE_LAST")) == 0);
                        const bool last = last_variant && bounce == opt.max_bounces - 1;
                        launch_shade(count, last, blocks_s, ls, LP, lb, bounce, q, bc, qn);
                    });
                    if (bounce == 0 && first_hit_targets && s == opt.samples_per_pass - 1 && LP.samples_accumulated + LP.previous_samples == 0)
                        hipLaunchKernelGGL(k_first_hit_gbuffer, dim3(blocks_all), dim3(KB), 0, ls, sv, LP, lb);
                    if (bounce < opt.max_bounces - 1 && !fused) {
                        hipStream_t ss = ls;
                        if (overlap) {
                            HIPCHK(hipEventRecord(impl->ev_fork, ls));
                            HIPCHK(hipStreamWaitEvent(impl->side, impl->ev_fork, 0));
                            ss = impl->side;
                        }
                        timed(T_SHADOW, ss, [&] {
                            auto ks = two_level ? (count ? k_trace_shadow<true, true, true> : k_trace_shadow<false, true, true>)
                                                : count ? k_trace_shadow<true> : (wide ? k_trace_shadow<false, true> : k_trace_shadow<false, false>);
                            PathBuffers sb = lb;
                            if (overlap) sb.qspill = pb.qspill + impl->qspill_lane_words;
                            hipLaunchKernelGGL(ks, dim3(std::min(blocks_all, shadow_cap)), dim3(KB), 0, ss, sv, LP, sb, bc);
                        });
                        if (overlap) { HIPCHK(hipEventRecord(impl->ev_join, impl->side)); shadow_in_flight = true; }
                    }
                }
                if (only != -2 && only != opt.max_bounces) continue;
                if (shadow_in_flight) { HIPCHK(hipStreamWaitEvent(ls, impl->ev_join, 0)); shadow_in_flight = false; }
                if (!LP.fused_resolve) hipLaunchKernelGGL(k_accumulate_sample, dim3(blocks_all), dim3(KB), 0, ls, LP, lb);
            }
            if (only != -2 && only != opt.max_bounces) return 0;
            if (sample_lanes && pass > 0) HIPCHK(hipStreamWaitEvent(ls, impl->pass_done[(pass - 1) % n_lanes], 0));
            LP.tm_display = (pass == passes - 1 && !direct) ? reinterpret_cast<f4*>(tm_display) : nullptr;
            timed(T_RESOLVE, ls, [&] { hipLaunchKernelGGL(k_resolve, dim3(blocks_all), dim3(KB), 0, ls, LP, lb); });
            if (sample_lanes && pass + 1 < passes) HIPCHK(hipEventRecord(impl->pass_done[lane], ls));
        }
        return 0;
    };
    static const char* order_env = getenv("TRHIP_ENQUEUE");
    const bool interleave = order_env ? strcmp(order_env, "lanes") != 0 : (impl->prev_frame_ms > 0.0f && impl->prev_frame_ms < 3.0f);
    static const bool merged_raygen_enabled = !(getenv("TRHIP_MERGED_RAYGEN") && atoi(getenv("TRHIP_MERGED_RAYGEN")) == 0);
    merged_raygen = merged_raygen_enabled && interleave && !sample_lanes && lanes_used > 1 && lanes_used == n_lanes && passes == 1 &&
                               opt.samples_per_pass == 1;
    if (merged_raygen) {
        PtParams RP = lane_ctx[0].LP;
        RP.id_offset = 0; RP.n_ids = (uint)n;
        RP.bounce_words = P.bounce_words * (uint)n_lanes;
        RP.previous_samples = 0; RP.sample_in_pass = 0;
        RP.rng_sample = shard_sample_base;
        launch_raygen((RP.n_ids + KB - 1) / KB, stream, RP, lane_ctx[0].lb);
    }
    if (n_lanes > 1) {
        HIPCHK(hipEventRecord(impl->ev_fork, stream));
        HIPCHK(hipStreamWaitEvent(impl->side, impl->ev_fork, 0));
        for (int l = 2; l < n_lanes; ++l) HIPCHK(hipStreamWaitEvent(impl->lane_stream[l], impl->ev_fork, 0));
    }
    if (sample_lanes) {
        for (int pass = 0; pass < passes; ++pass) if (int rc = enqueue_pass(pass % lanes_used, pass, -2)) return rc;
    } else if (interleave && lanes_used > 1 && passes == 1 && opt.samples_per_pass == 1) {
// ... 30 lines not shown
}

int PtStage::get_counters(trhip_counters* out, hipStream_t stream) {
    memset(out, 0, sizeof(*out));
    if (!impl->pb.counters) return 0;
    HIPCHK(hipStreamSynchronize(stream));
    uint hl[PT_LANES][CNT_WORDS];
    HIPCHK(hipMemcpy(hl, impl->pb.counters, sizeof(hl), hipMemcpyDeviceToHost));
    uint* h = hl[0];
    auto rd = [&](int i) { uint64_t v = 0; for (int l = 0; l < PT_LANES; ++l) v += (uint64_t)hl[l][i] | ((uint64_t)hl[l][i + 1] << 32); return v; };
    out->closest_rays = rd(CNT_CLOSEST); out->shadow_rays = rd(CNT_SHADOWRAYS); out->node_visits = rd(CNT_NODES);
    out->tri_tests = rd(CNT_TRIS); out->alpha_tests = rd(CNT_ALPHA); out->surface_hits = rd(CNT_SURF);
    for (int l = 1; l < PT_LANES; ++l) { h[CNT_OVERFLOW] |= hl[l][CNT_OVERFLOW]; h[CNT_MAXSP] = std::max(h[CNT_MAXSP], hl[l][CNT_MAXSP]); h[CNT_MAXVIS] = std::max(h[CNT_MAXVIS], hl[l][CNT_MAXVIS]); }
    out->stack_overflows = h[CNT_OVERFLOW];
    if (getenv("TRHIP_DEBUG"))
        fprintf(stderr, "[trhip] closest-hit loop: %llu node phases (%llu with <= 16 active rays serving %llu visits, %llu with <= 8), %llu triangle phases; quad tail: %llu node phases, %llu triangle phases; %llu node visits\n",
                (unsigned long long)rd(CNT_PH_NODE), (unsigned long long)rd(CNT_PH_NODE16), (unsigned long long)rd(CNT_LV_NODE16), (unsigned long long)rd(CNT_PH_NODE8),
                (unsigned long long)rd(CNT_PH_TRI), (unsigned long long)rd(CNT_PH_QNODE), (unsigned long long)rd(CNT_PH_QTRI), (unsigned long long)rd(CNT_NODES));
    if (getenv("TRHIP_DEBUG")) {
        fprintf(stderr, "[trhip] per-lane node phases by live rays (1-8, 9-16, ..., 57-64):");
        for (int b = 0; b < 8; ++b) fprintf(stderr, " %llu", (unsigned long long)rd(CNT_PH_HIST + 2 * b));
        fprintf(stderr, "\n");
    }
    if (getenv("TRHIP_DEBUG")) { float* f = (float*)(h + CNT_DBG); fprintf(stderr, "[trhip] overflow %u src %u; max stack depth %u; max node visits per ray %u; worst ray o=(%g %g %g) d=(%g %g %g) bounce %g id %g pdf %g reg %g\n", h[CNT_OVERFLOW], h[CNT_DBG + 12], h[CNT_MAXSP], h[CNT_MAXVIS], f[0], f[1], f[2], f[3], f[4], f[5], f[6], f[7], f[8], f[9]); }
    return 0;
}

int PtStage::get_phase_counters(trhip_phase_counters* out, hipStream_t stream) {
    memset(out, 0, sizeof(*out));
    if (!impl->pb.counters) return 0;
    HIPCHK(hipStreamSynchronize(stream));
    uint hl[PT_LANES][CNT_WORDS];
    HIPCHK(hipMemcpy(hl, impl->pb.counters, sizeof(hl), hipMemcpyDeviceToHost));
    auto rd = [&](int i) { uint64_t v = 0; for (int l = 0; l < PT_LANES; ++l) v += (uint64_t)hl[l][i] | ((uint64_t)hl[l][i + 1] << 32); return v; };
    out->lane_node_phases = rd(CNT_PH_NODE); out->lane_tri_phases = rd(CNT_PH_TRI);
    out->quad_node_phases = rd(CNT_PH_QNODE); out->quad_tri_phases = rd(CNT_PH_QTRI);
    out->lane_node_phases_le16 = rd(CNT_PH_NODE16); out->lane_node_visits_le16 = rd(CNT_LV_NODE16);
    out->closest_node_visits = rd(CNT_CNODES);
    for (int b = 0; b < 8; ++b) out->lane_node_phase_hist[b] = rd(CNT_PH_HIST + 2 * b);
    return 0;
}

int PtStage::get_light_counters(trhip_light_counters* out, hipStream_t stream) {
    memset(out, 0, sizeof(*out));
    if (!impl->pb.counters) return 0;
    HIPCHK(hipStreamSynchronize(stream));
    uint hl[PT_LANES][CNT_WORDS];
    HIPCHK(hipMemcpy(hl, impl->pb.counters, sizeof(hl), hipMemcpyDeviceToHost));
    auto rd = [&](int i) { uint64_t v = 0; for (int l = 0; l < PT_LANES; ++l) v += (uint64_t)hl[l][i] | ((uint64_t)hl[l][i + 1] << 32); return v; };
    out->sphere_tests = rd(CNT_LTESTS); out->node_visits = rd(CNT_LNODES); out->walk_fallbacks = rd(CNT_LFALLBACKS);
    return 0;
}

int PtStage::reset_counters() {
    if (impl->pb.counters) HIPCHK(hipMemset(impl->pb.counters, 0, PT_LANES * CNT_WORDS * sizeof(uint)));
    if (int rc = resolve_pending()) return rc;
    for (int k = 0; k < T_KINDS; ++k) { impl->acc_ms[k] = 0; impl->acc_launches[k] = 0; }
    impl->frames = 0;
    return 0;
}

int PtStage::resolve_pending() {
    for (auto& sp : impl->pending) {
        HIPCHK(hipEventSynchronize(sp.b));
        float ms = 0;
        HIPCHK(hipEventElapsedTime(&ms, sp.a, sp.b));
        impl->acc_ms[sp.kind] += ms;
        impl->acc_launches[sp.kind]++;
        impl->pool.push_back(sp.a); impl->pool.push_back(sp.b);
    }
    impl->pending.clear();
    return 0;
}

int PtStage::get_timings(trhip_timings* out) {
    memset(out, 0, sizeof(*out));
    if (timing_pending) {
        HIPCHK(hipEventSynchronize(impl->ev[1]));
        HIPCHK(hipEventElapsedTime(&out->path_tracing_ms, impl->ev[0], impl->ev[1]));
    }
    if (int rc = resolve_pending()) return rc;
    out->trace_closest_ms = impl->acc_ms[T_CLOSEST]; out->trace_shadow_ms = impl->acc_ms[T_SHADOW]; out->shade_ms = impl->acc_ms[T_SHADE];
    out->raygen_ms = impl->acc_ms[T_RAYGEN]; out->resolve_ms = impl->acc_ms[T_RESOLVE];
    out->trace_closest_launches = impl->acc_launches[T_CLOSEST]; out->trace_shadow_launches = impl->acc_launches[T_SHADOW];
    out->shade_launches = impl->acc_launches[T_SHADE]; out->frames = impl->frames;
    return 0;
}

}

extern "C" uint64_t trhip_build_id(void) { return (uint64_t)TRHIP_BUILD_ID; }

#if TR_TIMELINE
extern "C" int trhip_debug_timeline(unsigned long long* out, int reset) {
    if (hipDeviceSynchronize() != hipSuccess) return 1;
    if (out && hipMemcpyFromSymbol(out, HIP_SYMBOL(tr::g_timeline), sizeof(unsigned long long) * tr::TL_WORDS) != hipSuccess) return 1;
    if (reset) { static unsigned long long zero[tr::TL_WORDS]; if (hipMemcpyToSymbol(HIP_SYMBOL(tr::g_timeline), zero, sizeof(zero)) != hipSuccess) return 1; }
    return 0;
}
#endif
```

tauray_amd/csrc/pt.h:

```cpp
#pragma once
#include "build.h"

namespace tr {

void get_ray_count(const trhip_distribution& d, uint& w, uint& h);

int stream_pool_acquire(hipStream_t* out, const hipStream_t* overlap_with = nullptr, int n_overlap = 0);
void stream_pool_release(hipStream_t s);
int stream_pool_class(hipStream_t s, int* cls, bool blocking = false);
int stream_pool_pipe_classes(int* classes_out, int* streams_out);

class PtStage {
public:
    PtStage(DeviceScene* scene, const trhip_pt_options& opt);
    ~PtStage();
    int render(const trhip_pt_targets& targets, uint target_w, uint target_h, uint viewports, hipStream_t stream);
    int get_counters(trhip_counters* out, hipStream_t stream);
    int reset_counters();
    int get_timings(trhip_timings* out);
    int get_phase_counters(trhip_phase_counters* out, hipStream_t stream);
    int get_light_counters(trhip_light_counters* out, hipStream_t stream);
    int get_program(trhip_program_info* out);

    DeviceScene* scene;
    trhip_pt_options opt;
    trhip_distribution dist;
    uint frame_counter = 0;
    uint accumulated_samples = 0;
    int count_work = 0, detailed_timing = 0;
    uint shard_vp_base = 0, shard_vp_stride = 1, shard_sample_base = 0, shard_sample_stride = 1;
    int frame_slots = 0;
    int lanes = 0;
    int last_lanes = 0, last_lane_pipes[4] = {-1, -1, -1, -1};
    hipStream_t last_main = nullptr;
    void* tm_display = nullptr;
    trhip_tonemap_info tm_info{};
    uint frame_batch = 1;
    int ieee_shading = -1;
    int specialize = -1;
    bool direct = false;
    hipStream_t last_stream = nullptr;

    struct Program { bool cli_set, shade_fast, wide; const struct SpecKernels *shade, *raygen; };
    Program choose_program();

private:
    struct Impl;
    Impl* impl;
    bool timing_pending = false;
    int ensure_buffers(size_t n, bool lobe_sums);
    int resolve_pending();
    void free_buffers();
};

}
```

tauray_amd/csrc/pt_state.h:

```cpp
#pragma once
#include "shading.h"

#ifndef TR_BLOCK
#define TR_BLOCK 256
#endif

namespace tr {

constexpr int KB = TR_BLOCK;

struct PathBuffers {
    f4* org_pdf;
    f4* dir_reg;
    f4* atten_alpha;
    f4* diffuse;
    f4* reflection;
    f2* plobes;
    f4* first_mat;
    f4* first_emis;
    u4* rng;
    u4* misc;
    int4* hit;
    f4* sum_color;
    f4* sum_diffuse;
    f4* sum_reflection;
    f4* sh_org_tmax;
    f4* sh_dir_id;
    f4* sh_contrib;
    f2* sh_lobes;
    f4* sh_cweight;
    uint* queue[2];
    uint* bounce;
    int* qspill;
    uint* counters;
};

enum { BC_QUEUE = 0, BC_SHADOW = 64, BC_CUR_CLOSEST = 128, BC_CUR_SHADOW = 192, BC_STRIDE = 256 };
enum { CNT_OVERFLOW = 2, CNT_CLOSEST = 4, CNT_SHADOWRAYS = 6, CNT_NODES = 8, CNT_TRIS = 10, CNT_ALPHA = 12, CNT_SURF = 14, CNT_MAXVIS = 16, CNT_DBG = 17,
       CNT_MAXSP = 30, CNT_CNODES = 32, CNT_PH_NODE = 34, CNT_PH_TRI = 36, CNT_PH_NODE16 = 38, CNT_PH_NODE8 = 40, CNT_LV_NODE16 = 42, CNT_PH_QNODE = 44, CNT_PH_QTRI = 46, CNT_PH_HIST = 48, CNT_LTESTS = 64, CNT_LNODES = 66, CNT_LFALLBACKS = 68, CNT_WORDS = 70 };

struct PtParams {
    trhip_pt_options opt;
    LaunchCtx L;
    uint viewports;
    uint n_launch;
    uint id_offset, n_ids;
    uint max_sobol_bounces;
    uint sample_counter, rng_seed;
    uint previous_samples;
    uint sample_in_pass;
    uint rng_sample;
    uint vp_base, vp_stride;
    uint frame_views;
    uint frame_counter_step;
    uint samples_accumulated;
    uint target_w, target_h;
    float prob_point, prob_tri, prob_dir, prob_env;
    int nee_point, nee_tri, nee_dir, nee_env;
    int count_work;
    uint bounce_words;
    int fused_resolve;
    trhip_pt_targets T;
    f4* tm_display;
    int tm_op; float tm_exposure, tm_gamma; int tm_grid;
};


namespace {

TR_DEV void add64(uint* counters, int idx, uint v) {
    if (v) atomicAdd(reinterpret_cast<unsigned long long*>(counters + idx), (unsigned long long)v);
}

TR_DEV uint wave_append(uint* counter, bool pred) {
    unsigned long long mask = __ballot(pred);
    uint n = __popcll(mask);
    uint base = 0;
    int lane = threadIdx.x & 63;
    int leader = __ffsll((long long)mask) - 1;
    if (pred && lane == leader) base = atomicAdd(counter, n);
    base = __shfl(base, leader < 0 ? 0 : leader);
    uint rank = __popcll(mask & ((1ull << lane) - 1ull));
    return base + rank;
}

TR_DEV void block_append2(uint* counter_a, bool pred_a, uint& slot_a, uint* counter_b, bool pred_b, uint& slot_b) {
    __shared__ uint s_cnt[2][KB / 64];
    __shared__ uint s_base[2];
    const unsigned long long ma = __ballot(pred_a), mb = __ballot(pred_b);
    const uint lane = threadIdx.x & 63u, wave = threadIdx.x >> 6;
    if (lane == 0) { s_cnt[0][wave] = (uint)__popcll(ma); s_cnt[1][wave] = (uint)__popcll(mb); }
    __syncthreads();
// ... 21 lines not shown
```

tauray_amd/csrc/trace.h:

```cpp
#pragma once
#include "common.h"
#include "rng.h"
#include "texture.h"
#include "trace_timeline.h"

namespace tr {

#ifndef TR_BLOCK
#define TR_BLOCK 256
#endif
#ifndef TR_VOTE
#define TR_VOTE 32
#endif
#ifndef TR_VOTE_SHADOW_WAVE
#define TR_VOTE_SHADOW_WAVE 16
#endif
#ifndef TR_SLAB_PAD
#define TR_SLAB_PAD 1.000004f
#endif
#define TR_LDS_STACK 16
#ifndef TR_SPILL_STACK
#define TR_SPILL_STACK 112
#endif

struct RayPre {
    f3 op;
    f3 ip;
    float Sx, Sy;
    uint nkx, nky, nkz;
};
TR_DEV uint tri_component_offset(uint nk) { return (nk >> 3) & 12u; }

TR_DEV RayPre make_ray(f3 org, f3 dir) {
    RayPre r;
    float ax = fabsf(dir.x), ay = fabsf(dir.y), az = fabsf(dir.z);
    int kz = (ax > ay) ? (ax > az ? 0 : 2) : (ay > az ? 1 : 2);
    int kx = kz + 1; if (kx == 3) kx = 0;
    int ky = kx + 1; if (ky == 3) ky = 0;
    if (comp(dir, kz) < 0.0f) { int t = kx; kx = ky; ky = t; }
    const float dkx = comp(dir, kx), dky = comp(dir, ky), dkz = comp(dir, kz);
    r.Sx = dkx / dkz;
    r.Sy = dky / dkz;
    r.op = F3(comp(org, kx), comp(org, ky), comp(org, kz));
    r.ip = F3(1.0f / dkx, 1.0f / dky, 1.0f / dkz);
    r.nkx = ((uint)kx << 5) | ((__float_as_uint(r.ip.x) >> 31) << 4);
    r.nky = ((uint)ky << 5) | ((__float_as_uint(r.ip.y) >> 31) << 4);
    r.nkz = ((uint)kz << 5) | ((__float_as_uint(r.ip.z) >> 31) << 4);
    return r;
}

TR_DEV bool ray_is_finite(f3 o, f3 d) {
    return isfinite(o.x) && isfinite(o.y) && isfinite(o.z) && isfinite(d.x) && isfinite(d.y) && isfinite(d.z) &&
           (d.x != 0.0f || d.y != 0.0f || d.z != 0.0f);
}

#ifndef TR_PAIR_LEAVES
#define TR_PAIR_LEAVES 0
#endif
TR_DEV uint leaf_index(uint complemented_ref) { return TR_PAIR_LEAVES ? (complemented_ref & 0x3FFFFFFFu) : complemented_ref; }
TR_DEV bool leaf_is_pair(uint complemented_ref) { return TR_PAIR_LEAVES && (complemented_ref & 0x40000000u) != 0; }
#if TR_PAIR_LEAVES
#define TR_LEAF_MEMBERS(ref, more) for (uint member = 0; member <= (leaf_is_pair(ref) ? 1u : 0u) && (more); ++member)
#else
#define TR_LEAF_MEMBERS(ref, more) constexpr uint member = 0;
#endif

struct TriHit { float t, bu, bv; uint inst_flags, prim, alpha; };

#ifndef TR_SETPRIO
#define TR_SETPRIO 0
#endif
#if TR_SETPRIO == 1
#define TR_PRIO_BEGIN() __builtin_amdgcn_s_setprio(0)
#define TR_PRIO_ISSUED() __builtin_amdgcn_s_setprio(2)
#elif TR_SETPRIO == 2
#define TR_PRIO_BEGIN() __builtin_amdgcn_s_setprio(2)
#define TR_PRIO_ISSUED() __builtin_amdgcn_s_setprio(0)
#else
#define TR_PRIO_BEGIN()
#define TR_PRIO_ISSUED()
#endif

TR_DEV bool tri_intersect(const RayPre& r, const TriRecord* tris, uint index, float tmin, float tmax, TriHit& o TL(, TlPhase* tlp = nullptr)) {
#pragma clang fp contract(off)
    TR_PRIO_BEGIN();
#ifndef TR_TRI_FETCH_DWORDS
    const f4* p = reinterpret_cast<const f4*>(reinterpret_cast<const char*>(tris) + (size_t)index * (uint)sizeof(TriRecord));
    const f4 q0 = p[0], q1 = p[1], q2 = p[2];
    TR_PRIO_ISSUED();
    o.inst_flags = __float_as_uint(q2.y); o.prim = __float_as_uint(q2.z); o.alpha = __float_as_uint(q2.w);
    const uint kx4 = tri_component_offset(r.nkx), ky4 = tri_component_offset(r.nky), kz4 = tri_component_offset(r.nkz);
    auto pick = [](float x, float y, float z, uint k4) { const float xy = k4 == 4u ? y : x; return k4 == 8u ? z : xy; };
    const float v0x = pick(q0.x, q0.y, q0.z, kx4), v1x = pick(q0.w, q1.x, q1.y, kx4), v2x = pick(q1.z, q1.w, q2.x, kx4);
    const float v0y = pick(q0.x, q0.y, q0.z, ky4), v1y = pick(q0.w, q1.x, q1.y, ky4), v2y = pick(q1.z, q1.w, q2.x, ky4);
    const float v0z = pick(q0.x, q0.y, q0.z, kz4), v1z = pick(q0.w, q1.x, q1.y, kz4), v2z = pick(q1.z, q1.w, q2.x, kz4);
#else
    const char* base = reinterpret_cast<const char*>(tris);
    const uint rec = index * (uint)sizeof(TriRecord);
    const uint ox = rec + tri_component_offset(r.nkx), oy = rec + tri_component_offset(r.nky), oz = rec + tri_component_offset(r.nkz);
    const float v0x = *reinterpret_cast<const float*>(base + (size_t)ox), v1x = *reinterpret_cast<const float*>(base + (size_t)ox + 12), v2x = *reinterpret_cast<const float*>(base + (size_t)ox + 24);
    const float v0y = *reinterpret_cast<const float*>(base + (size_t)oy), v1y = *reinterpret_cast<const float*>(base + (size_t)oy + 12), v2y = *reinterpret_cast<const float*>(base + (size_t)oy + 24);
    const float v0z = *reinterpret_cast<const float*>(base + (size_t)oz), v1z = *reinterpret_cast<const float*>(base + (size_t)oz + 12), v2z = *reinterpret_cast<const float*>(base + (size_t)oz + 24);
    const uint* tail = reinterpret_cast<const uint*>(base + (size_t)rec + 36);
    o.inst_flags = tail[0]; o.prim = tail[1]; o.alpha = tail[2];
#endif
    TL(if (tlp) tlp->loads_issued();)
    const float Akz = v0z - r.op.z, Bkz = v1z - r.op.z, Ckz = v2z - r.op.z;
    const float Ax = (v0x - r.op.x) - r.Sx * Akz, Ay = (v0y - r.op.y) - r.Sy * Akz;
    const float Bx = (v1x - r.op.x) - r.Sx * Bkz, By = (v1y - r.op.y) - r.Sy * Bkz;
    const float Cx = (v2x - r.op.x) - r.Sx * Ckz, Cy = (v2y - r.op.y) - r.Sy * Ckz;
    float U = Cx * By - Cy * Bx;
    float V = Ax * Cy - Ay * Cx;
    float W = Bx * Ay - By * Ax;
    if (U == 0.0f || V == 0.0f || W == 0.0f) {
        double CxBy = (double)Cx * (double)By, CyBx = (double)Cy * (double)Bx;
        U = (float)(CxBy - CyBx);
        double AxCy = (double)Ax * (double)Cy, AyCx = (double)Ay * (double)Cx;
        V = (float)(AxCy - AyCx);
// ... 533 lines not shown
```

tauray_amd/csrc/trace_lanes.h:

```cpp
#pragma once
#include "trace.h"
#include "trace_quad.h"
#include "pt_state.h"

namespace tr {

namespace {

template <bool COUNT, bool TWO_LEVEL = false>
TR_DEV void closest_lane(const SceneView& sv, const PtParams& P, const PathBuffers& pb, int bounce, const uint* queue, uint qi, uint n, int* lds_stack,
                         const QuadCtx& qc, TraceStats& st, int& overflow, uint& max_vis, uint& rays) {
    bool valid = qi < n;
    uint id = 0;
    u4 misc = {0, 0, 0, 1};
    f4 o = F4(0), d = F4(0);
    TL(const unsigned long long tl_chunk = tl_now();)
    if (valid) { id = queue ? queue[qi] : qi + P.id_offset; misc = pb.misc[id]; o = pb.org_pdf[id]; d = pb.dir_reg[id]; valid = !(misc.w & 1u); }
    TL(tl_data_arrived(); tl_misc(qc.tl, 3, tl_now() - tl_chunk);)
    for (int b = 0; b < bounce; ++b) pcg(misc.x);
    HitRecord hit;
    const uint before = st.nodes;
#if TR_QUAD_SWITCH > 0
    trace_closest_wave4<0, COUNT, TWO_LEVEL>(sv, valid, F3(o), F3(d), bounce == 0 ? 0.0f : P.opt.min_ray_dist, __builtin_huge_valf(), misc.x,
                                  lds_stack, qc, hit, st, overflow);
#else
    if (valid) trace_closest4<0, COUNT, TWO_LEVEL>(sv, F3(o), F3(d), bounce == 0 ? 0.0f : P.opt.min_ray_dist, __builtin_huge_valf(),
                                        misc.x, lds_stack, hit, st, overflow);
#endif
    if (COUNT) st.cnodes += st.nodes - before;
    if (!valid) return;
    if (COUNT) {
        const uint vis = st.nodes - before;
        max_vis = max(max_vis, vis);
        if (vis > 100000u && vis > atomicMax(&pb.counters[CNT_MAXVIS], vis)) {
            float* dbg = reinterpret_cast<float*>(pb.counters + CNT_DBG);
            dbg[0] = o.x; dbg[1] = o.y; dbg[2] = o.z; dbg[3] = d.x; dbg[4] = d.y; dbg[5] = d.z; dbg[6] = (float)bounce; dbg[7] = (float)id;
            dbg[8] = o.w; dbg[9] = d.w;
        }
    }
    const float tri_t = hit.instance_id >= 0 ? hit.t : __builtin_huge_valf();
    pb.hit[id] = make_int4(hit.instance_id, hit.primitive_id, __float_as_int(hit.u), __float_as_int(hit.v));
    if (!(P.opt.hide_lights && bounce == 0)) {
        uint rid = id;
        asm volatile("" : "+v"(rid));
        const f3 lo = F3(pb.org_pdf[rid]), ld = F3(pb.dir_reg[rid]);
        if (ray_is_finite(lo, ld)) {
            const LightHit lh = trace_sphere_lights<COUNT>(sv, lo, ld, bounce == 0 ? 0.0f : P.opt.min_ray_dist, tri_t, lds_stack, st);
            if (lh.light >= 0) pb.hit[rid] = make_int4(-1, lh.light, __float_as_int(lh.t), 0);
        }
    }
    rays++;
    TL(tl_misc(qc.tl, 5, tl_now() - tl_chunk);)
}

TR_DEV QuadCtx make_quad_ctx(int* s_stack, int* s_owner, const PathBuffers& pb TL(, uint* s_tl = nullptr)) {
    QuadCtx qc;
    TL(qc.tl = s_tl ? s_tl + (threadIdx.x >> 6) * TL_WORDS : nullptr;)
    const uint wave = threadIdx.x >> 6;
    qc.wave_stack = s_stack + (threadIdx.x & ~63u);
    qc.owner_tab = s_owner + wave * TR_OWNER_WORDS;
    qc.spill = pb.qspill + ((size_t)blockIdx.x * (KB / 64) + wave) * (16u * TR_QSPILL);
    return qc;
}

template <bool COUNT, bool TWO_LEVEL, typename CONTRIB, typename LOBES>
TR_DEV void shadow_ray(const SceneView& sv, const PtParams& P, const PathBuffers& pb, bool valid, f4 o, f4 d, CONTRIB&& contrib, LOBES&& lobes, int* lds_stack, const QuadCtx& qc,
                       TraceStats& st, int& overflow, uint& rays) {
#if TR_QUAD_SWITCH > 0 && !defined(TR_NO_SHADOW_QUADS)
    float vis = trace_shadow_wave4<COUNT, TWO_LEVEL>(sv, valid, F3(o), F3(d), P.opt.min_ray_dist, o.w, lds_stack, qc, st, overflow);
#else
    float vis = 1.0f;
    if (valid) vis = trace_shadow4<COUNT, TWO_LEVEL>(sv, F3(o), F3(d), P.opt.min_ray_dist, o.w, lds_stack, st, overflow);
#endif
    if (!valid) return;
    const uint id = __float_as_uint(d.w);
    if (vis != 0.0f) {
        const f4 c = contrib();
        float m = c.w * vis;
        if (c.w > 0.0f && m > P.opt.indirect_clamping) vis *= P.opt.indirect_clamping / m;
        const f3 radiance = F3(c.x * vis, c.y * vis, c.z * vis);
        const f2 w = lobes();
        if (w.x != 0.0f) { f4 d4 = pb.diffuse[id]; d4.x += radiance.x * w.x; d4.y += radiance.y * w.x; d4.z += radiance.z * w.x; pb.diffuse[id] = d4; }
        if (w.y != 0.0f) { f4 r4 = pb.reflection[id]; r4.x += radiance.x * w.y; r4.y += radiance.y * w.y; r4.z += radiance.z * w.y; pb.reflection[id] = r4; }
    }
    rays++;
}
template <bool COUNT, bool TWO_LEVEL = false>
TR_DEV void shadow_lane(const SceneView& sv, const PtParams& P, const PathBuffers& pb, uint qi, uint n, int* lds_stack, const QuadCtx& qc,
                        TraceStats& st, int& overflow, uint& rays) {
    const bool valid = qi < n;
    f4 o = F4(0), d = F4(0);
    if (valid) { o = pb.sh_org_tmax[qi]; d = pb.sh_dir_id[qi]; }
    shadow_ray<COUNT, TWO_LEVEL>(sv, P, pb, valid, o, d, [&] { return pb.sh_contrib[qi]; }, [&] { return pb.sh_lobes[qi]; }, lds_stack, qc, st, overflow, rays);
}

template <bool COUNT>
TR_DEV void flush_trace_counters(const PtParams& P, const PathBuffers& pb, int overflow, int overflow_tag, uint closest_rays, uint shadow_rays,
                                 TraceStats st, uint max_vis) {
    if (overflow) { pb.counters[CNT_OVERFLOW] = 1; pb.counters[CNT_DBG + 12] = (uint)overflow_tag; }
    if (!P.count_work) return;
    for (int off = 32; off > 0; off >>= 1) {
        closest_rays += __shfl_xor(closest_rays, off); shadow_rays += __shfl_xor(shadow_rays, off);
        if (COUNT) {
            st.nodes += __shfl_xor(st.nodes, off); st.tris += __shfl_xor(st.tris, off); st.alpha += __shfl_xor(st.alpha, off);
            st.ph_node += __shfl_xor(st.ph_node, off); st.ph_tri += __shfl_xor(st.ph_tri, off); st.ph_node16 += __shfl_xor(st.ph_node16, off);
            st.ph_node8 += __shfl_xor(st.ph_node8, off); st.lv_node16 += __shfl_xor(st.lv_node16, off);
            st.ph_qnode += __shfl_xor(st.ph_qnode, off); st.ph_qtri += __shfl_xor(st.ph_qtri, off); st.cnodes += __shfl_xor(st.cnodes, off);
            st.ltests += __shfl_xor(st.ltests, off); st.lnodes += __shfl_xor(st.lnodes, off); st.lfallbacks += __shfl_xor(st.lfallbacks, off);
            for (int b = 0; b < 8; ++b) st.ph_hist[b] += __shfl_xor(st.ph_hist[b], off);
            st.maxsp = max(st.maxsp, (uint)__shfl_xor(st.maxsp, off)); max_vis = max(max_vis, (uint)__shfl_xor(max_vis, off));
        }
    }
    if ((threadIdx.x & 63) == 0) {
        add64(pb.counters, CNT_CLOSEST, closest_rays);
        add64(pb.counters, CNT_SHADOWRAYS, shadow_rays);
        if (COUNT) {
            add64(pb.counters, CNT_NODES, st.nodes); add64(pb.counters, CNT_TRIS, st.tris); add64(pb.counters, CNT_ALPHA, st.alpha);
            add64(pb.counters, CNT_PH_NODE, st.ph_node); add64(pb.counters, CNT_PH_TRI, st.ph_tri); add64(pb.counters, CNT_PH_NODE16, st.ph_node16);
            add64(pb.counters, CNT_PH_NODE8, st.ph_node8); add64(pb.counters, CNT_LV_NODE16, st.lv_node16);
            add64(pb.counters, CNT_PH_QNODE, st.ph_qnode); add64(pb.counters, CNT_PH_QTRI, st.ph_qtri); add64(pb.counters, CNT_CNODES, st.cnodes);
            add64(pb.counters, CNT_LTESTS, st.ltests); add64(pb.counters, CNT_LNODES, st.lnodes); add64(pb.counters, CNT_LFALLBACKS, st.lfallbacks);
            for (int b = 0; b < 8; ++b) add64(pb.counters, CNT_PH_HIST + 2 * b, st.ph_hist[b]);
            atomicMax(&pb.counters[CNT_MAXSP], st.maxsp); atomicMax(&pb.counters[CNT_MAXVIS], max_vis);
        }
    }
}

}

}
```

tauray_amd/csrc/trace_quad.h:

```cpp
#pragma once
#include "trace.h"

namespace tr {

#ifndef TR_QUAD_SWITCH
#define TR_QUAD_SWITCH 16
#endif
#ifndef TR_QUAD_VOTE
#define TR_QUAD_VOTE 4
#endif
#define TR_QSPILL TR_SPILL_STACK
static_assert(TR_QUAD_SWITCH <= 16, "a wave has sixteen quads");

#define TR_OWNER_WORDS 16

struct QuadCtx {
    int* wave_stack;
    int* owner_tab;
    int* spill;
    TL(uint* tl;)
};

template <int CTRL> TR_DEV int quad_perm(int v) { return __builtin_amdgcn_update_dpp(0, v, CTRL, 0xF, 0xF, true); }
TR_DEV int qrot1(int v) { return quad_perm<0x39>(v); }
TR_DEV int qrot2(int v) { return quad_perm<0x4E>(v); }
TR_DEV int qrot3(int v) { return quad_perm<0x93>(v); }
TR_DEV float qrot1f(float v) { return __int_as_float(qrot1(__float_as_int(v))); }
TR_DEV float qrot2f(float v) { return __int_as_float(qrot2(__float_as_int(v))); }
TR_DEV int bperm(int byte_addr, int v) { return __builtin_amdgcn_ds_bpermute(byte_addr, v); }
TR_DEV float bpermf(int byte_addr, float v) { return __int_as_float(__builtin_amdgcn_ds_bpermute(byte_addr, __float_as_int(v))); }

TR_DEV int quad_lane() {
    int l;
    asm volatile("v_mbcnt_lo_u32_b32 %0, -1, 0\n\tv_mbcnt_hi_u32_b32 %0, -1, %0" : "=v"(l));
    return l & 3;
}

TR_DEV void wave_sync_lds() {
    __builtin_amdgcn_fence(__ATOMIC_RELEASE, "workgroup");
    __builtin_amdgcn_wave_barrier();
    __builtin_amdgcn_fence(__ATOMIC_ACQUIRE, "workgroup");
}

#ifndef TR_QUAD_FETCH
#define TR_QUAD_FETCH 0
#endif
struct QuadRay {
    RayPre r;
    float tmin;
#if TR_QUAD_FETCH
    uint off_a, off_b;
#endif
};

TR_DEV void quad_transpose(int q, float& r0, float& r1, float& r2, float& r3) {
    const bool odd = (q & 1) != 0, hi = (q & 2) != 0;
    auto swap1 = [&](float& a, float& b) {
        const float t = __int_as_float(quad_perm<0xB1>(__float_as_int(odd ? a : b)));
        a = odd ? t : a; b = odd ? b : t;
    };
    auto swap2 = [&](float& a, float& b) {
        const float t = __int_as_float(quad_perm<0x4E>(__float_as_int(hi ? a : b)));
// ... 90 lines not shown
            const int k = e - TR_LDS_STACK;
            if (k < TR_QSPILL) qc.spill[d.my_rank * TR_QSPILL + k] = spill[k < TR_SPILL_STACK ? k : TR_SPILL_STACK - 1];
            else overflow++;
        }
    }
    wave_sync_lds();
    d.has_ray = d.qd < n_act;
    const int owner = d.has_ray ? qc.owner_tab[d.qd] : lane;
    d.src = owner << 2;
    d.back = d.my_rank << 4;
    const int src = d.src;
    qr.r.op = F3(bpermf(src, r.op.x), bpermf(src, r.op.y), bpermf(src, r.op.z));
    qr.r.ip = F3(bpermf(src, r.ip.x), bpermf(src, r.ip.y), bpermf(src, r.ip.z));
    qr.r.Sx = bpermf(src, r.Sx); qr.r.Sy = bpermf(src, r.Sy);
    const uint packed = (uint)bperm(src, (int)(r.nkx | (r.nky << 8) | (r.nkz << 16)));
    qr.r.nkx = packed & 0xFFu; qr.r.nky = (packed >> 8) & 0xFFu; qr.r.nkz = (packed >> 16) & 0xFFu;
    qr.tmin = bpermf(src, tmin);
#if TR_QUAD_FETCH
    {
        const uint flip = (uint)(d.q & 1) << 4;
        qr.off_a = ((d.q & 2) ? qr.r.nky : qr.r.nkx) ^ flip;
        qr.off_b = (d.q & 2) ? 96u : (qr.r.nkz ^ flip);
    }
#endif
    qnode = bperm(src, node);
    qs.lds = qc.wave_stack + owner;
    qs.glob = qc.spill + d.qd * TR_QSPILL;
    qs.sp = bperm(src, stk.sp);
    qs.overflow = 0;
    return d;
}

TR_DEV void quad_descend(bool inner, uint key, int c, QuadStack& qs, int& qnode, bool& qlive) {
    const uint k1 = (uint)qrot1((int)key), k2 = (uint)qrot2((int)key), k3 = (uint)qrot3((int)key);
    const int rank = (int)(k1 < key) + (int)(k2 < key) + (int)(k3 < key);
    int n_inner = inner ? 1 : 0;
    n_inner += qrot1(n_inner); n_inner += qrot2(n_inner);
    int nx = (inner && rank == 0) ? c : 0;
    nx |= qrot1(nx); nx |= qrot2(nx);
    if (n_inner > 0) {
        if (inner && rank >= 1) qs.store(qs.sp + n_inner - 1 - rank, c);
        qs.sp += n_inner - 1;
        qnode = nx;
    } else if (qs.sp == 0) qlive = false;
    else { qs.sp--; qnode = qs.load(qs.sp); }
}

TR_DEV void quad_inherited_leaf(int q, int& pend, QuadStack& qs, int& qnode, bool& qlive) {
    if (q == 0) pend = ~qnode;
    if (qs.sp == 0) qlive = false;
    else { qs.sp--; qnode = qs.load(qs.sp); }
}

template <int ALPHA_MODE, bool COUNT, bool TWO_LEVEL = false>
TR_DEV void trace_closest_wave4(const SceneView& sv, bool valid, f3 org, f3 dir, float tmin, float tmax, uint seed,
                                int* lds_stack, const QuadCtx& qc, HitRecord& hit, TraceStats& st, int& overflow) {
    hit.instance_id = -1; hit.primitive_id = -1; hit.u = 0; hit.v = 0; hit.t = -1.0f;
    if constexpr (TWO_LEVEL) {
        if (valid) trace_closest4_2l<ALPHA_MODE, COUNT>(sv, org, dir, tmin, tmax, seed, lds_stack, hit, st, overflow);
        return;
    }
    float best_t = tmax, best_u = 0.0f, best_v = 0.0f;
    uint best_inst = 0xFFFFFFFFu, best_prim = 0xFFFFFFFFu;
    RayPre r = make_ray(org, dir);
    const bool finite_ray = valid && ray_is_finite(org, dir);
    bool live = finite_ray && sv.tri_count > 0;
    LaneStack stk;
    int spill[TR_SPILL_STACK];
    stk.init(lds_stack);
    int node = sv.node_count > 0 ? 0 : -1;
    TL(const unsigned long long tl_enter = tl_now(), tl_wall0 = tl_wall();)

    auto consider = [&](const TriHit& tr, float t, float bu, float bv) {
        const uint inst = tr.inst_flags & 0x7FFFFFFFu;
        const bool closer = t < best_t || (t == best_t && best_inst != 0xFFFFFFFFu && (inst < best_inst || (inst == best_inst && tr.prim < best_prim)));
        if (closer) {
            bool accept = true;
            if (tr.inst_flags & 0x80000000u) {
                if (COUNT) st.alpha++;
                const float a = candidate_alpha(sv, tr.alpha, bu, bv);
                const float cutoff = ALPHA_MODE == 0 ? alpha_cutoff_hash(seed, (int)inst, (int)tr.prim) : 0.0001f;
                accept = !(a <= cutoff);
            }
            if (accept) { best_t = t; best_inst = inst; best_prim = tr.prim; best_u = bu; best_v = bv; }
        }
    };

    while (true) {
        const unsigned long long act = __ballot(live);
        if (__popcll(act) <= TR_QUAD_SWITCH) break;
        if (live) {
            const bool at_leaf = node < 0;
#if TR_VOTE > 0
            const int n_leaf = __popcll(__ballot(at_leaf)), n_all = __popcll(__ballot(true));
            const bool leaf_phase = n_leaf >= (TR_VOTE < ((n_all + 1) >> 1) ? TR_VOTE : ((n_all + 1) >> 1)) || n_leaf == n_all;
#else
            const bool leaf_phase = at_leaf;
#endif
            if (COUNT) {
                const unsigned long long m = __ballot(true);
                if ((int)(threadIdx.x & 63) == __ffsll((long long)m) - 1) {
                    if (!leaf_phase) { st.ph_node++; st.ph_hist[(__popcll(m) - 1) >> 3]++; if (__popcll(m) <= 16) { st.ph_node16++; st.lv_node16 += (uint)__popcll(__ballot(!at_leaf)); } if (__popcll(m) <= 8) st.ph_node8++; }
                    else st.ph_tri++;
                }
            }
            if (at_leaf == leaf_phase) {
                bool descend = false;
                TL(TlPhase tlp; const int tl_units = __popcll(__ballot(true)); tlp.begin();)
                if (!at_leaf) {
                    Hit4 h;
                    box4_intersect(r, sv.nodes4, node, tmin, best_t, h TL(, &tlp));
                    if (COUNT) st.nodes++;
                    TR_CE4(0, 1) TR_CE4(2, 3) TR_CE4(0, 2) TR_CE4(1, 3) TR_CE4(1, 2)
                    TL(asm volatile("" : "+v"(h.t[0]), "+v"(h.t[1]), "+v"(h.t[2]), "+v"(h.t[3]), "+v"(h.c[0]), "+v"(h.c[1]), "+v"(h.c[2]), "+v"(h.c[3])); tlp.mark_a();)
                    if (h.t[0] < __builtin_huge_valf()) {
                        const int m = (int)(h.t[1] < __builtin_huge_valf()) + (int)(h.t[2] < __builtin_huge_valf()) + (int)(h.t[3] < __builtin_huge_valf());
                        stk.push_sorted(spill, m, h.c[1], h.c[2], h.c[3]);
                        if (COUNT) st.maxsp = max(st.maxsp, (uint)stk.sp);
                        node = h.c[0];
                        descend = true;
                    }
                } else {
                    TriHit tr;
                    if (COUNT) st.tris++;
#if TR_TIMELINE
                    const bool tl_hit = tri_intersect(r, sv.tris, (uint)~node, tmin, __builtin_huge_valf(), tr, &tlp);
                    tlp.mark_a();
                    if (tl_hit) { tlp.alpha = (tr.inst_flags & 0x80000000u) != 0 && (tr.t < best_t || tr.t == best_t); consider(tr, tr.t, tr.bu, tr.bv); }
                    tlp.mark_b();
#else
                    TR_LEAF_MEMBERS((uint)~node, true)
                    if (tri_intersect(r, sv.tris, leaf_index((uint)~node) + member, tmin, __builtin_huge_valf(), tr)) consider(tr, tr.t, tr.bu, tr.bv);
#endif
                }
                if (!descend) {
                    if (stk.sp == 0) live = false;
                    else node = stk.pop(spill);
                }
                TL(tlp.end(qc.tl, leaf_phase ? TL_LT : TL_LN, tl_units, (tl_units - 1) >> 3, leaf_phase ? TL_LT_WAIT_HIST : TL_LN_WAIT_HIST);)
            }
        }
    }

    const unsigned long long act = __ballot(live);
    const int n_act = __popcll(act);
#ifdef TR_QUAD_DEBUG
    const float dbg_u = live ? (float)stk.sp : -1.0f, dbg_v = live ? (float)((node < 0 ? 1000 : 0) + n_act) : -1.0f;
#endif
    if (n_act > 0) {
        QuadRay qr; QuadStack qs; int qnode;
        TL(const unsigned long long tl_deal = tl_now();)
        if (live) stk.flush(spill);
        const QuadDeal deal = quad_deal(act, live, r, tmin, node, stk, spill, qc, overflow, qr, qs, qnode);
        const int src = deal.src;
        const uint qseed = (uint)bperm(src, (int)seed);
        float lt = bpermf(src, best_t), lu = bpermf(src, best_u), lv = bpermf(src, best_v);
        uint linst = (uint)bperm(src, (int)best_inst), lprim = (uint)bperm(src, (int)best_prim);
        float qbest = lt;
        bool qlive = deal.has_ray;
        int pend = -1;
#if TR_TAIL_PREFETCH
        int qpf = 0;
#endif
        TL(tl_misc(qc.tl, 2, tl_now() - tl_deal);)
        while (true) {
            int w = pend >= 0 ? 1 : 0;
            w |= qrot1(w); w |= qrot2(w);
            const bool qwait = w != 0;
            if (__ballot(qlive || qwait) == 0) break;
            const bool can_node = qlive && !qwait;
            const bool tri_phase = __popcll(__ballot(pend >= 0)) >= TR_QUAD_VOTE || __ballot(can_node) == 0;
            if (COUNT && (threadIdx.x & 63) == 0) { if (tri_phase) st.ph_qtri++; else st.ph_qnode++; }
            if (tri_phase) {
                if (pend >= 0) {
                    TL(TlPhase tlp; const int tl_units = __popcll(__ballot(true)); tlp.begin();)
                    TriHit tr;
                    if (COUNT) st.tris++;
                    TR_LEAF_MEMBERS((uint)pend, true)
                    if (tri_intersect(qr.r, sv.tris, leaf_index((uint)pend) + member, qr.tmin, __builtin_huge_valf(), tr TL(, &tlp))) {
                        const float t = tr.t, bu = tr.bu, bv = tr.bv;
                        const uint inst = tr.inst_flags & 0x7FFFFFFFu;
                        bool accept = t < lt || (t == lt && linst != 0xFFFFFFFFu && (inst < linst || (inst == linst && tr.prim < lprim)));
                        if (accept && (tr.inst_flags & 0x80000000u)) {
                            if (COUNT) st.alpha++;
                            const float a = candidate_alpha(sv, tr.alpha, bu, bv);
                            const float cutoff = ALPHA_MODE == 0 ? alpha_cutoff_hash(qseed, (int)inst, (int)tr.prim) : 0.0001f;
                            accept = !(a <= cutoff);
                        }
                        lt = accept ? t : lt; lu = accept ? bu : lu; lv = accept ? bv : lv;
                        linst = accept ? inst : linst; lprim = accept ? tr.prim : lprim;
                    }
                    TL(tlp.end(qc.tl, TL_QT, tl_units, (tl_units - 1) >> 3, -1);)
                }
                pend = -1;
                float m = lt;
                m = fminf(m, qrot1f(m)); m = fminf(m, qrot2f(m));
                qbest = fminf(qbest, m);
            } else if (can_node && qnode < 0) quad_inherited_leaf(quad_lane(), pend, qs, qnode, qlive);
            else if (can_node) {
                bool hitb; float t0;
                TL(TlPhase tlp; const int tl_units = __popcll(__ballot(true)) >> 2; tlp.begin();)
                const int q = quad_lane();
#if TR_TAIL_PREFETCH
                const int c = quad_child_box(qr, sv.nodes4, qnode, q, qbest, hitb, t0 TL(, &tlp), qpf);
#else
                const int c = quad_child_box(qr, sv.nodes4, qnode, q, qbest, hitb, t0 TL(, &tlp));
#endif
                if (COUNT && q == 0) st.nodes++;
                const bool inner = hitb && c >= 0;
#if TR_TAIL_PREFETCH
                if (inner) qpf = *reinterpret_cast<const int*>(reinterpret_cast<const char*>(sv.nodes4) + ((size_t)(uint)c << 7) + 96);
#endif
                if (hitb && c < 0) pend = ~c;
                quad_descend(inner, inner ? ((__float_as_uint(t0) & ~3u) | (uint)q) : 0xFFFFFFFFu, c, qs, qnode, qlive);
                if (COUNT) st.maxsp = max(st.maxsp, (uint)qs.sp);
                TL(tlp.end(qc.tl, TL_QN, tl_units, (tl_units - 1) >> 1, TL_QN_WAIT_HIST);)
            }
        }
        {
            float ot = qrot1f(lt), ou = qrot1f(lu), ov = qrot1f(lv); uint oi = (uint)qrot1((int)linst), op = (uint)qrot1((int)lprim);
            bool take = ot < lt || (ot == lt && (oi < linst || (oi == linst && op < lprim)));
            lt = take ? ot : lt; lu = take ? ou : lu; lv = take ? ov : lv; linst = take ? oi : linst; lprim = take ? op : lprim;
            ot = qrot2f(lt); ou = qrot2f(lu); ov = qrot2f(lv); oi = (uint)qrot2((int)linst); op = (uint)qrot2((int)lprim);
            take = ot < lt || (ot == lt && (oi < linst || (oi == linst && op < lprim)));
            lt = take ? ot : lt; lu = take ? ou : lu; lv = take ? ov : lv; linst = take ? oi : linst; lprim = take ? op : lprim;
        }
        int qo = qs.overflow;
        qo += qrot1(qo); qo += qrot2(qo);
        const int back = deal.back;
        const float rt = bpermf(back, lt), ru = bpermf(back, lu), rv = bpermf(back, lv);
        const uint ri = (uint)bperm(back, (int)linst), rp = (uint)bperm(back, (int)lprim);
        const int ro = bperm(back, qo);
        if (live) { best_t = rt; best_u = ru; best_v = rv; best_inst = ri; best_prim = rp; overflow += ro; }
    }
    overflow += stk.overflow ? 1 : 0;
    TL(tl_misc(qc.tl, 0, 1); tl_misc(qc.tl, 1, tl_now() - tl_enter); tl_misc(qc.tl, 4, tl_wall() - tl_wall0);)

    bool found = best_inst != 0xFFFFFFFFu;
    if (found) { hit.instance_id = (int)best_inst; hit.primitive_id = (int)best_prim; hit.u = best_u; hit.v = best_v; }
    hit.t = found ? best_t : -1.0f;
#ifdef TR_QUAD_DEBUG
    hit.u = dbg_u; hit.v = dbg_v;
#endif
}

template <bool COUNT, bool TWO_LEVEL = false>
TR_DEV float trace_shadow_wave4(const SceneView& sv, bool valid, f3 org, f3 dir, float tmin, float tmax, int* lds_stack, const QuadCtx& qc,
                                TraceStats& st, int& overflow) {
    if constexpr (TWO_LEVEL) return valid ? trace_shadow4_2l<COUNT>(sv, org, dir, tmin, tmax, lds_stack, st, overflow) : 1.0f;
    float visibility = 1.0f;
    bool live = valid && sv.tri_count > 0 && ray_is_finite(org, dir);
    RayPre r = make_ray(org, dir);
    LaneStack stk;
    int spill[TR_SPILL_STACK];
    stk.init(lds_stack);
    int node = sv.node_count > 0 ? 0 : -1;
    while (true) {
        if (__popcll(__ballot(live)) <= TR_QUAD_SWITCH) break;
#if TR_VOTE_SHADOW_WAVE > 0
        bool go = live;
        if (live) {
            const bool at_leaf = node < 0;
            const int n_leaf = __popcll(__ballot(at_leaf)), n_all = __popcll(__ballot(true));
            const bool leaf_phase = n_leaf >= TR_VOTE_SHADOW_WAVE || n_leaf == n_all;
            go = at_leaf == leaf_phase;
        }
        if (go) {
#else
        if (live) {
#endif
            bool descend = false;
            if (node >= 0) {
                Hit4 h;
                box4_intersect(r, sv.nodes4, node, tmin, tmax, h);
                if (COUNT) st.nodes++;
                descend = shadow_descend(h, stk, spill, node);
            } else {
                TriHit tr;
                if (COUNT) st.tris++;
                TR_LEAF_MEMBERS((uint)~node, live)
                if (tri_intersect(r, sv.tris, leaf_index((uint)~node) + member, tmin, tmax, tr)) {
                    if (!(tr.inst_flags & 0x80000000u)) { visibility = 0.0f; live = false; }
                    else {
                        if (COUNT) st.alpha++;
                        const float alpha = candidate_alpha(sv, tr.alpha, tr.bu, tr.bv);
                        visibility *= 1.0f - alpha;
                        if (visibility == 0.0f) live = false;
// ... 71 lines not shown
```

tauray_amd/renderer.py:

```python
from __future__ import annotations

import ctypes as C
import os
from dataclasses import dataclass, field
from typing import List, Optional

import numpy as np

from . import _lib
from ._lib import (AccelInfoC, AccelLayoutC, CountersC, DistributionC, LightAccelInfoC, LightCountersC, PtOptionsC, SceneDescC, TimingsC,
                   TonemapInfoC, TrhipError, check)
from .distribution import (DISTRIBUTION_DUPLICATE, DISTRIBUTION_SCANLINE, DISTRIBUTION_SHUFFLED_STRIPS, DistributionParams,
                           get_device_distribution_params, get_distribution_target_size)
from .scene import SceneDesc, build_alias_table

FILM_POINT, FILM_BOX, FILM_BLACKMAN_HARRIS = 0, 1, 2
MIS_DISABLED, MIS_BALANCE_HEURISTIC, MIS_POWER_HEURISTIC = 0, 1, 2
BOUNCE_HEMISPHERE, BOUNCE_COSINE_HEMISPHERE, BOUNCE_MATERIAL = 0, 1, 2
TRI_LIGHT_AREA, TRI_LIGHT_SOLID_ANGLE, TRI_LIGHT_HYBRID = 0, 1, 2
SAMPLER_UNIFORM_RANDOM, SAMPLER_SOBOL_OWEN, SAMPLER_SOBOL_Z_ORDER_2D, SAMPLER_SOBOL_Z_ORDER_3D = 0, 1, 2, 3
TONEMAP_LINEAR, TONEMAP_GAMMA_CORRECTION, TONEMAP_FILMIC, TONEMAP_REINHARD, TONEMAP_REINHARD_LUMINANCE = 0, 1, 2, 3, 4
FEATURE_ALBEDO, FEATURE_WORLD_NORMAL, FEATURE_VIEW_NORMAL, FEATURE_WORLD_POS, FEATURE_VIEW_POS, FEATURE_DISTANCE = 0, 1, 2, 3, 4, 5
FEATURE_INSTANCE_ID = 9


def make_options(**kw) -> PtOptionsC:
    o = PtOptionsC(max_bounces=8, min_ray_dist=1e-4, rng_seed=0, sampler=SAMPLER_UNIFORM_RANDOM, samples_per_pixel=1,
                   samples_per_pass=1, projection=0, film=FILM_POINT, film_radius=0.5, mis_mode=MIS_POWER_HEURISTIC,
                   russian_roulette_delta=0.0, indirect_clamping=0.0, regularization_gamma=0.0, depth_of_field=0,
                   nee_point=1.0, nee_directional=1.0, nee_envmap=1.0, nee_triangles=1.0, bounce_mode=BOUNCE_MATERIAL,
                   tri_light_mode=TRI_LIGHT_SOLID_ANGLE, hide_lights=0, use_white_albedo_on_first_bounce=0,
                   transparent_background=0, pre_transformed_vertices=0)
    for k, v in kw.items():
        if not hasattr(o, k):
            raise AttributeError(f"unknown path tracer option {k!r}")
        setattr(o, k, v)
    return o


def options_for_scene(scene: SceneDesc, **kw) -> PtOptionsC:
    o = make_options(**kw)
    if len(scene.point_lights) == 0:
        o.nee_point = 0.0
    if len(scene.directional_lights) == 0:
        o.nee_directional = 0.0
    if scene.envmap is None:
        o.nee_envmap = 0.0
    if not scene.has_tri_lights():
        o.nee_triangles = 0.0
    if scene.cameras and "projection" not in kw:
        o.projection = scene.cameras[0].projection
    return o


def copy_options(o: PtOptionsC, **changes) -> PtOptionsC:
    c = PtOptionsC()
    C.memmove(C.byref(c), C.byref(o), C.sizeof(PtOptionsC))
    for k, v in changes.items():
        setattr(c, k, v)
    return c


class DeviceBuffer:
# ... 223 lines not shown
            check(_lib.lib().trhip_scene_build_accel(self.ctx.h, C.byref(info)))
        self.accel.update(node_count=info.node_count, build_ms=info.build_ms, tri_light_count=info.tri_light_count,
                          bounds_min=tuple(info.bounds_min), bounds_max=tuple(info.bounds_max), leaf_count=info.leaf_count)
        return self.accel

    def set_skin(self, instance: int, skins: np.ndarray, source: Optional[np.ndarray] = None):
        from .scene import SKIN
        skins = np.ascontiguousarray(skins, dtype=SKIN)
        src_ptr = None
        if source is not None:
            source = np.ascontiguousarray(source)
            if len(source) != len(skins):
                raise ValueError("set_skin: source and skins differ in length")
            src_ptr = source.ctypes.data
        check(_lib.lib().trhip_scene_set_skin(self.ctx.h, instance, src_ptr, skins.ctypes.data if len(skins) else None, len(skins)))

    def skin(self, instance: int, joint_transforms: np.ndarray, refit: Optional[bool] = True):
        j = np.ascontiguousarray(np.asarray(joint_transforms, dtype=np.float32).reshape(-1, 4, 4).transpose(0, 2, 1))
        check(_lib.lib().trhip_scene_skin(self.ctx.h, instance, j.ctypes.data, len(j)))
        return None if refit is None else self._accel_after_change(refit)

    def vertices(self, instance: int) -> np.ndarray:
        from .scene import VERTEX
        n = int(self.scene.spans[instance]["vertex_count"])
        out = np.zeros(n, dtype=VERTEX)
        if n:
            check(_lib.lib().trhip_scene_get_vertices(self.ctx.h, instance, out.ctypes.data, n))
        return out

    def tri_lights(self) -> np.ndarray:
        from .scene import TRI_LIGHT
        n = self.accel["tri_light_count"]
        out = np.zeros(n, dtype=TRI_LIGHT)
        if n:
            check(_lib.lib().trhip_scene_get_tri_lights(self.ctx.h, out.ctypes.data, n))
        return out

    def trace_closest(self, rays: np.ndarray, seeds: Optional[np.ndarray] = None, include_lights=False) -> np.ndarray:
        rays = np.ascontiguousarray(rays, dtype=np.float32).reshape(-1, 8)
        n = len(rays)
        hit_dtype = np.dtype([("instance_id", "<i4"), ("primitive_id", "<i4"), ("bary_u", "<f4"), ("bary_v", "<f4"), ("t", "<f4")])
        if n == 0:
            return np.zeros(0, dtype=hit_dtype)
        d_rays = self.ctx.alloc(rays.nbytes).upload(rays)
        d_seeds = None
        if seeds is not None:
            seeds = np.ascontiguousarray(seeds, dtype=np.uint32)
            d_seeds = self.ctx.alloc(seeds.nbytes).upload(seeds)
        d_hits = self.ctx.alloc(n * 20)
        check(_lib.lib().trhip_trace_closest(self.ctx.h, n, d_rays.ptr, d_seeds.ptr if d_seeds else None,
                                             1 if include_lights else 0, d_hits.ptr, None))
        return d_hits.download((n,), hit_dtype)

    def trace_shadow(self, rays: np.ndarray) -> np.ndarray:
        rays = np.ascontiguousarray(rays, dtype=np.float32).reshape(-1, 8)
        n = len(rays)
        if n == 0:
            return np.zeros(0, dtype=np.float32)
        d_rays = self.ctx.alloc(rays.nbytes).upload(rays)
        d_vis = self.ctx.alloc(n * 4)
        check(_lib.lib().trhip_trace_shadow(self.ctx.h, n, d_rays.ptr, d_vis.ptr, None))
        return d_vis.download((n,), np.float32)


def _dist_c(p: DistributionParams) -> DistributionC:
    return DistributionC(int(p.size[0]), int(p.size[1]), int(p.strategy), int(p.index), int(p.count), 1 if p.primary else 0)


class PathTracerStage:

    _create = "trhip_pt_create"

    def __init__(self, ctx: Context, scene_stage: SceneStage, options: PtOptionsC, distribution: Optional[DistributionParams] = None):
        self.ctx, self.ss, self.opt = ctx, scene_stage, options
        h = C.c_void_p()
        check(getattr(_lib.lib(), self._create)(ctx.h, C.byref(options), C.byref(h)))
        self.h = h.value
        self.distribution = None
        if distribution is not None:
            self.reset_distribution_params(distribution)

    def reset_distribution_params(self, distribution: DistributionParams):
        d = _dist_c(distribution)
        check(_lib.lib().trhip_pt_set_distribution(self.h, C.byref(d)))
        self.distribution = distribution

    def set_shard(self, viewport_base=0, viewport_stride=1, sample_base=0, sample_stride=1):
        check(_lib.lib().trhip_pt_set_shard(self.h, viewport_base, viewport_stride, sample_base, sample_stride))

    def set_frame_counter(self, frame_counter: int):
        check(_lib.lib().trhip_pt_set_frame_counter(self.h, frame_counter))

    def set_frame_batch(self, frames: int):
        check(_lib.lib().trhip_pt_set_frame_batch(self.h, int(frames)))

    def set_shading_arithmetic(self, ieee: bool):
        check(_lib.lib().trhip_pt_set_shading_arithmetic(self.h, int(bool(ieee))))

    def set_specialization(self, enable: bool):
        check(_lib.lib().trhip_pt_set_specialization(self.h, int(bool(enable))))

    def set_lanes(self, lanes: int):
        check(_lib.lib().trhip_pt_set_lanes(self.h, lanes))

    def set_fused_tonemap(self, display, info):
        check(_lib.lib().trhip_pt_set_fused_tonemap(self.h, None if display is None else _ptr(display), None if info is None else C.byref(info)))

    def lane_pipes(self):
        if not hasattr(_lib.lib(), "trhip_pt_get_lane_pipes"):
            return 0, []
        n = C.c_int32(0)
        cls = (C.c_int32 * 4)()
        check(_lib.lib().trhip_pt_get_lane_pipes(self.h, C.byref(n), cls))
        return n.value, [cls[i] for i in range(n.value)]

    def set_frame_slots(self, slots: int):
        if hasattr(_lib.lib(), "trhip_pt_set_frame_slots"):
            check(_lib.lib().trhip_pt_set_frame_slots(self.h, slots))

    def reset_accumulated_samples(self):
        check(_lib.lib().trhip_pt_reset_accumulation(self.h, 0))

    def reset_sample_counter(self):
        check(_lib.lib().trhip_pt_reset_accumulation(self.h, 1))

    def run(self, color_target, viewports=1, stream=None):
        tw, th = get_distribution_target_size(self.distribution)
        check(_lib.lib().trhip_pt_render(self.h, _ptr(color_target), tw, th, viewports, stream))

    TARGETS = {"color": (4, np.float32), "diffuse": (4, np.float32), "reflection": (4, np.float32), "albedo": (4, np.float32),
               "material": (4, np.float32), "normal": (2, np.float32), "pos": (4, np.float32), "instance_id": (1, np.int32),
               "screen_motion": (2, np.float32)}

    def run_targets(self, targets: dict, viewports=1, stream=None):
        unknown = set(targets) - set(self.TARGETS)
        if unknown:
            raise ValueError(f"unknown gbuffer targets: {sorted(unknown)}")
        t = _lib.PtTargetsC()
        for name, buf in targets.items():
            setattr(t, name, _ptr(buf))
        tw, th = get_distribution_target_size(self.distribution)
        check(_lib.lib().trhip_pt_render_targets(self.h, C.byref(t), tw, th, viewports, stream))

    def set_profiling(self, count_work=False, detailed_timing=False):
        check(_lib.lib().trhip_pt_set_profiling(self.h, int(count_work), int(detailed_timing)))

    def counters(self) -> dict:
        c = CountersC()
        check(_lib.lib().trhip_pt_get_counters(self.h, C.byref(c)))
        return {n: int(getattr(c, n)) for n, _ in CountersC._fields_}

    def reset_counters(self):
        check(_lib.lib().trhip_pt_reset_counters(self.h))

    def light_counters(self) -> dict:
        c = LightCountersC()
        check(_lib.lib().trhip_pt_get_light_counters(self.h, C.byref(c)))
        return {n: int(getattr(c, n)) for n, _ in LightCountersC._fields_}

    def timings(self) -> dict:
        t = TimingsC()
        check(_lib.lib().trhip_pt_get_timings(self.h, C.byref(t)))
        return {n: float(getattr(t, n)) for n, _ in TimingsC._fields_}

    def program(self) -> dict:
        from ._lib import ProgramInfoC
        p = ProgramInfoC()
        if not hasattr(_lib.lib(), "trhip_pt_get_program"):
            return {"kind": "general", "ieee": False, "identity": 0, "key": "unknown: the library predates trhip_pt_get_program"}
        check(_lib.lib().trhip_pt_get_program(self.h, C.byref(p)))
        return {"kind": ("general", "cli", "compiled")[p.kind], "ieee": bool(p.ieee), "identity": int(p.identity), "key": p.key.decode()}

    def phase_counters(self) -> dict:
        from ._lib import PhaseCountersC
        p = PhaseCountersC()
        check(_lib.lib().trhip_pt_get_phase_counters(self.h, C.byref(p)))
        out = {n: int(getattr(p, n)) for n, _ in PhaseCountersC._fields_ if n != "lane_node_phase_hist"}
        out["lane_node_phase_hist"] = [int(x) for x in p.lane_node_phase_hist]
        return out

    def close(self):
        if self.h:
            _lib.lib().trhip_pt_destroy(self.h)
            self.h = None

    def __del__(self):
        try:
            self.close()
        except Exception:
            pass


class DirectStage(PathTracerStage):
    _create = "trhip_direct_create"


class FeatureStage:

    def __init__(self, ctx: Context, scene_stage: SceneStage, feature: int, distribution: DistributionParams, projection=0,
                 min_ray_dist=1e-4, default_value=(np.nan,) * 4):
        self.ctx, self.ss, self.feature, self.distribution = ctx, scene_stage, feature, distribution
        self.projection, self.min_ray_dist, self.default_value = projection, min_ray_dist, default_value

    def run(self, color_target, viewport=0, stream=None):
        tw, th = get_distribution_target_size(self.distribution)
        d = _dist_c(self.distribution)
        dv = (C.c_float * 4)(*self.default_value)
        check(_lib.lib().trhip_feature_render(self.ctx.h, self.feature, C.byref(d), self.projection, viewport, self.min_ray_dist, dv,
                                              _ptr(color_target), tw, th, stream))


# ... 367 lines not shown
```

Measured before the change: 3739.

## Add terminal-bounce closest query that tests emitters first and stops early when blocked

On the last bounce, a closest-hit ray only matters if it reaches an emitter. The new terminal kernel first intersects a small gathered set of emitter triangles, bounded by their box, to set a tight best_t. The BVH walk then stops as soon as a closer non-emitter surface is found, and the ray is marked blocked. Emitter gathering runs at build time, and the query is auto-enabled when there are few emitters and a merged structure. The cost is extra kernel variants, more register pressure in the shared traversal template, and a host sync during accel build.

Result: faster. 3924, median of 6 (+5.0%).

```diff
diff --git a/include/trhip.h b/include/trhip.h
--- a/include/trhip.h
+++ b/include/trhip.h
@@ -215,6 +215,11 @@
 int trhip_pt_get_phase_counters(trhip_pt* pt, trhip_phase_counters* out);
 typedef struct trhip_light_counters { uint64_t sphere_tests, node_visits, walk_fallbacks; } trhip_light_counters;
 int trhip_pt_get_light_counters(trhip_pt* pt, trhip_light_counters* out);
+#define TRHIP_TERMINAL_QUERY_AUTO 0
+#define TRHIP_TERMINAL_QUERY_OFF 1
+int trhip_pt_set_terminal_query(trhip_pt* pt, int mode);
+typedef struct trhip_terminal_counters { uint64_t blocked_rays, fallback_rays; uint32_t in_effect, emitter_triangles, threshold, pad; } trhip_terminal_counters;
+int trhip_pt_get_terminal_counters(trhip_pt* pt, trhip_terminal_counters* out);
 int trhip_calibrate_valu(trhip_device* dev, float* ginst_per_s);
 int trhip_calibrate_l1(trhip_device* dev, float* gaccesses_per_s);
 
@@ -224,6 +229,8 @@
 
 int trhip_trace_closest(trhip_device* dev, uint32_t n, const void* rays_dev, const void* seeds_dev,
                         int include_lights, void* hits_dev, void* stream);
+int trhip_trace_terminal(trhip_device* dev, uint32_t n, const void* rays_dev, const void* seeds_dev, const void* fallback_dev,
+                         void* hits_dev, void* stream);
 int trhip_trace_shadow(trhip_device* dev, uint32_t n, const void* rays_dev, void* visibility_dev, void* stream);
 
 int trhip_stitch(trhip_device* dev, const trhip_distribution* partial_dist, const void* partial_dev,
diff --git a/tauray_amd/_lib.py b/tauray_amd/_lib.py
--- a/tauray_amd/_lib.py
+++ b/tauray_amd/_lib.py
@@ -53,6 +53,15 @@
 
 
 LIGHT_ACCEL_AUTO, LIGHT_ACCEL_LOOP, LIGHT_ACCEL_TREE = 0, 1, 2
+
+
+class TerminalCountersC(C.Structure):
+    _fields_ = [("blocked_rays", C.c_uint64), ("fallback_rays", C.c_uint64), ("in_effect", C.c_uint32), ("emitter_triangles", C.c_uint32),
+                ("threshold", C.c_uint32), ("pad", C.c_uint32)]
+
+
+TERMINAL_QUERY_AUTO, TERMINAL_QUERY_OFF = 0, 1
+HIT_BLOCKED = -2
 
 
 class PtOptionsC(C.Structure):
@@ -133,6 +142,9 @@
     "trhip_scene_set_light_accel": (_i, [_vp, _i]),
     "trhip_scene_get_light_accel": (_i, [_vp, C.POINTER(LightAccelInfoC)]),
     "trhip_pt_get_light_counters": (_i, [_vp, C.POINTER(LightCountersC)]),
+    "trhip_pt_set_terminal_query": (_i, [_vp, _i]),
+    "trhip_pt_get_terminal_counters": (_i, [_vp, C.POINTER(TerminalCountersC)]),
+    "trhip_trace_terminal": (_i, [_vp, _u32, _vp, _vp, _vp, _vp, _vp]),
     "trhip_stitch_batch": (_i, [_vp, _u32, _vp, _vp, _vp, _vp, _vp, _u32, C.c_float, _vp]),
     "trhip_stream_create": (_i, [_vp, C.POINTER(C.c_void_p)]),
     "trhip_stream_destroy": (_i, [_vp, _vp]),
diff --git a/tauray_amd/csrc/api.hip b/tauray_amd/csrc/api.hip
--- a/tauray_amd/csrc/api.hip
+++ b/tauray_amd/csrc/api.hip
@@ -148,6 +148,32 @@
     }
     if (overflow) *overflow_flag = 1;
 }
+__global__ __launch_bounds__(KB) void k_query_terminal(SceneView sv, uint n, const float* rays, const uint* seeds, const uint* fallback, HitRecord* out, uint* overflow_flag,
+                                                       int* qspill) {
+    __shared__ int s_stack_rows[TR_STACK_WORDS];
+    int* const s_stack = s_stack_rows + TR_STACK_ROW0;
+    __shared__ int s_owner[(KB / 64) * TR_OWNER_WORDS];
+    int* my_stack = s_stack + threadIdx.x;
+    QuadCtx qc;
+    qc.wave_stack = s_stack + (threadIdx.x & ~63u);
+    qc.owner_tab = s_owner + (threadIdx.x >> 6) * TR_OWNER_WORDS;
+    qc.spill = qspill + ((size_t)blockIdx.x * (KB / 64) + (threadIdx.x >> 6)) * (16u * TR_QSPILL);
+    int overflow = 0;
+    TraceStats st = {};
+    for (uint base = blockIdx.x * KB; base < n; base += gridDim.x * KB) {
+        const uint i = base + threadIdx.x;
+        const bool valid = i < n;
+        float r[8] = {0, 0, 0, 0, 0, 0, 0, 0};
+        if (valid) for (int k = 0; k < 8; ++k) r[k] = rays[(size_t)i * 8 + k];
+        const uint seed = (valid && seeds) ? seeds[i] : 0u;
+        TerminalRay term = {valid && !(fallback && fallback[i] != 0u), false};
+        HitRecord hit;
+        if (seeds) trace_closest_wave4<0, false, false, true>(sv, valid, F3(r[0], r[1], r[2]), F3(r[4], r[5], r[6]), r[3], r[7], seed, my_stack, qc, hit, st, overflow, &term);
+        else trace_closest_wave4<1, false, false, true>(sv, valid, F3(r[0], r[1], r[2]), F3(r[4], r[5], r[6]), r[3], r[7], 0u, my_stack, qc, hit, st, overflow, &term);
+        if (valid) out[i] = term.blocked ? HitRecord{TR_HIT_BLOCKED, -1, 0.0f, 0.0f, -1.0f} : hit;
+    }
+    if (overflow) *overflow_flag = 1;
+}
 template <bool TWO_LEVEL>
 __global__ __launch_bounds__(KB) void k_query_shadow(SceneView sv, uint n, const float* rays, float* out, uint* overflow_flag) {
     __shared__ int s_stack_rows[TR_STACK_WORDS];
@@ -827,6 +853,20 @@
     DEVCHK(pt->dev);
     return pt->stage->get_light_counters(out, pt->stage->last_stream);
 }
+int trhip_pt_set_terminal_query(trhip_pt* pt, int mode) {
+    if (!pt) return set_error("null trhip_pt");
+    if (mode != TRHIP_TERMINAL_QUERY_AUTO && mode != TRHIP_TERMINAL_QUERY_OFF)
+        return set_error("trhip_pt_set_terminal_query: unknown mode " + std::to_string(mode) + " (0 auto, 1 off)");
+    pt->stage->terminal_query = mode;
+    return 0;
+}
+int trhip_pt_get_terminal_counters(trhip_pt* pt, trhip_terminal_counters* out) {
+    if (!pt) return set_error("null trhip_pt");
+    if (!out) return set_error("trhip_pt_get_terminal_counters: null output");
+    DEVCHK(pt->dev);
+    if (pt->stage->terminal_query_in_effect() < 0) return set_error("trhip_pt_get_terminal_counters: TRHIP_TERMINAL_QUERY is not auto or off");
+    return pt->stage->get_terminal_counters(out, pt->stage->last_stream);
+}
 int trhip_pt_reset_counters(trhip_pt* pt) { if (!pt) return set_error("null trhip_pt"); DEVCHK(pt->dev); HIPCHK(hipStreamSynchronize(pt->stage->last_stream)); return pt->stage->reset_counters(); }
 int trhip_pt_get_timings(trhip_pt* pt, trhip_timings* out) { if (!pt) return set_error("null trhip_pt"); DEVCHK(pt->dev); return pt->stage->get_timings(out); }
 int trhip_pt_get_program(trhip_pt* pt, trhip_program_info* out) { if (!pt) return set_error("null trhip_pt"); if (!out) return set_error("trhip_pt_get_program: null out"); DEVCHK(pt->dev); return pt->stage->get_program(out); }
@@ -921,6 +961,20 @@
     HIPCHK(hipGetLastError());
     return 0;
 }
+int trhip_trace_terminal(trhip_device* dev, uint32_t n, const void* rays_dev, const void* seeds_dev, const void* fallback_dev, void* hits_dev, void* stream) {
+    DEVCHK(dev);
+    const DeviceScene& s = dev->scene;
+    if (!s.accel_built) return set_error("trhip_trace_terminal: call trhip_scene_build_accel first");
+    if (s.two_level || !s.tris) return set_error("trhip_trace_terminal: the terminal query walks an all-merged structure");
+    if (s.emitter_count > TR_EMITTER_MAX) return set_error("trhip_trace_terminal: " + std::to_string(s.emitter_count) + " emitter triangles, the query tests at most " + std::to_string(TR_EMITTER_MAX));
+    if (n == 0) return 0;
+    uint blocks = std::min((n + KB - 1) / KB, QUERY_BLOCKS);
+    if (!dev->qspill) HIPCHK(hipMalloc(&dev->qspill, (size_t)QUERY_BLOCKS * (KB / 64) * 16u * TR_QSPILL * sizeof(int)));
+    hipLaunchKernelGGL(k_query_terminal, dim3(blocks), dim3(KB), 0, (hipStream_t)stream, s.view(), n, (const float*)rays_dev, (const uint*)seeds_dev, (const uint*)fallback_dev,
+                       (HitRecord*)hits_dev, dev->overflow_flag, dev->qspill);
+    HIPCHK(hipGetLastError());
+    return 0;
+}
 int trhip_trace_shadow(trhip_device* dev, uint32_t n, const void* rays_dev, void* visibility_dev, void* stream) {
     DEVCHK(dev);
     if (!dev->scene.accel_built) return set_error("trhip_trace_shadow: call trhip_scene_build_accel first");
diff --git a/tauray_amd/csrc/build.h b/tauray_amd/csrc/build.h
--- a/tauray_amd/csrc/build.h
+++ b/tauray_amd/csrc/build.h
@@ -98,6 +98,8 @@
     uint light_tree_nodes = 0;
     float light_ms = 0.0f;
     int light_last_refit = -1;
+    uint sphere_light_count() const { uint c = 0; for (const PointLight& pl : host_point_lights) c += pl.radius != 0.0f ? 1u : 0u; return c; }
+    uint emitter_count = 0xFFFFFFFFu;
 
     SceneView view() const {
         SceneView v;
@@ -124,6 +126,7 @@
         tlas = nullptr; tlas_src_leaves = nullptr; tlas_capacity = 0; node_capacity = 0; tri_capacity = 0; two_level = false;
         blases.clear(); inst_blas.clear(); tlas_src.clear(); blas_dirty.clear(); static_dirty = false;
         nodes = nullptr; nodes4 = nullptr; tris = nullptr; tri_lights = nullptr; node_count = 0; tri_light_count = 0; accel_built = false;
+        emitter_count = 0xFFFFFFFFu;
         accel_capacity = 0xFFFFFFFFu;
         if (level_nodes) (void)hipFree(level_nodes);
         if (node_bounds) (void)hipFree(node_bounds);
diff --git a/tauray_amd/csrc/bvh_build.hip b/tauray_amd/csrc/bvh_build.hip
--- a/tauray_amd/csrc/bvh_build.hip
+++ b/tauray_amd/csrc/bvh_build.hip
@@ -454,6 +454,38 @@
     out[(uint)o.light_base_id + prim] = l;
 }
 
+__global__ __launch_bounds__(BT) void k_emitter_gather(const Instance* instances, const TriRecord* tris, uint n, EmitterSet* es) {
+    const uint i = blockIdx.x * BT + threadIdx.x;
+    if (i >= n) return;
+    const Instance& o = instances[tris[i].inst_flags & 0x7FFFFFFFu];
+    const f4 e = o.mat.emission_factor;
+    if (!(e.x != 0.0f || e.y != 0.0f || e.z != 0.0f || o.light_base_id >= 0)) return;
+    const uint slot = atomicAdd(&es->count, 1u);
+    if (slot < TR_EMITTER_MAX) es->index[slot] = i;
+}
+__global__ void k_emitter_finish(const TriRecord* tris, EmitterSet* es) {
+    const uint c = es->count <= TR_EMITTER_MAX ? es->count : 0u;
+    for (uint a = 1; a < c; ++a) {
+        const uint v = es->index[a];
+        uint b = a;
+        for (; b > 0 && es->index[b - 1] > v; --b) es->index[b] = es->index[b - 1];
+        es->index[b] = v;
+    }
+    float lo[3] = {__builtin_huge_valf(), __builtin_huge_valf(), __builtin_huge_valf()}, hi[3] = {-__builtin_huge_valf(), -__builtin_huge_valf(), -__builtin_huge_valf()};
+    for (uint a = 0; a < c; ++a) {
+        const TriRecord& t = tris[es->index[a]];
+        for (int k = 0; k < 3; ++k) {
+            lo[k] = fminf(fminf(lo[k], t.v0[k]), fminf(t.v1[k], t.v2[k]));
+            hi[k] = fmaxf(fmaxf(hi[k], t.v0[k]), fmaxf(t.v1[k], t.v2[k]));
+        }
+    }
+    for (int k = 0; k < 3; ++k)
+        for (int slot = 0; slot < 4; ++slot) {
+            es->planes[8 * k + slot] = slot == 0 ? lo[k] : __builtin_huge_valf();
+            es->planes[8 * k + 4 + slot] = slot == 0 ? hi[k] : -__builtin_huge_valf();
+        }
+}
+
 #define HIPCHK(x) do { hipError_t e_ = (x); if (e_ != hipSuccess) return set_error(std::string(#x) + ": " + hipGetErrorString(e_)); } while (0)
 
 }
@@ -473,6 +505,19 @@
     v.tangent = F4(t, v.tangent.w);
     if (det < 0) { v.normal = -v.normal; v.tangent = F4(-t.x, -t.y, -t.z, -v.tangent.w); }
     out[i] = v;
+}
+
+static int gather_emitters(DeviceScene& ds, hipStream_t stream) {
+    ds.emitter_count = 0xFFFFFFFFu;
+    if (!ds.tris || ds.leaf_count != ds.tri_count) return 0;
+    EmitterSet* es = reinterpret_cast<EmitterSet*>(ds.tris + ds.tri_count);
+    HIPCHK(hipMemsetAsync(es, 0, sizeof(EmitterSet), stream));
+    hipLaunchKernelGGL(k_emitter_gather, dim3((ds.tri_count + BT - 1) / BT), dim3(BT), 0, stream, ds.instances, ds.tris, ds.tri_count, es);
+    hipLaunchKernelGGL(k_emitter_finish, dim3(1), dim3(1), 0, stream, ds.tris, es);
+    HIPCHK(hipGetLastError());
+    HIPCHK(hipMemcpyAsync(&ds.emitter_count, &es->count, sizeof(uint), hipMemcpyDeviceToHost, stream));
+    HIPCHK(hipStreamSynchronize(stream));
+    return 0;
 }
 
 int ensure_world_vertices(DeviceScene& ds, hipStream_t stream) {
@@ -723,6 +768,7 @@
         SceneView sv2 = ds.view();
         hipLaunchKernelGGL(k_extract_tri_lights, dim3((ds.tri_count + BT - 1) / BT), dim3(BT), 0, stream, sv2, ds.tri_prefix, ds.tri_lights);
     }
+    if (int rc = gather_emitters(ds, stream)) return rc;
     HIPCHK(hipEventRecord(e1, stream));
     HIPCHK(hipEventSynchronize(e1));
     float ms = 0;
@@ -1118,7 +1164,7 @@
     }
     if (ds.accel_capacity != n_cap) {
         ds.free_accel();
-        if (n_cap > 0) HIPCHK(hipMalloc(&ds.tris, (size_t)n_cap * sizeof(TriRecord)));
+        if (n_cap > 0) HIPCHK(hipMalloc(&ds.tris, (size_t)n_cap * sizeof(TriRecord) + sizeof(EmitterSet)));
         if (n1 > 0) {
             if ((uint64_t)n1 * sizeof(Bvh4Node) > 0xFFFFFFFFull) return set_error("trhip_scene_build_accel: more than 2^25 nodes");
             HIPCHK(hipMalloc(&ds.nodes4, n1 * sizeof(Bvh4Node)));
@@ -1144,6 +1190,7 @@
         hipLaunchKernelGGL(k_extract_tri_lights, dim3((n_tri + BT - 1) / BT), dim3(BT), 0, stream, sv2, ds.tri_prefix, ds.tri_lights);
         HIPCHK(hipGetLastError());
     }
+    if (int rc = gather_emitters(ds, stream)) return rc;
     HIPCHK(hipEventRecord(e1, stream));
     HIPCHK(hipEventSynchronize(e1));
     float ms = 0;
diff --git a/tauray_amd/csrc/common.h b/tauray_amd/csrc/common.h
--- a/tauray_amd/csrc/common.h
+++ b/tauray_amd/csrc/common.h
@@ -208,4 +208,10 @@
     return reinterpret_cast<const Bvh4Node*>(reinterpret_cast<const char*>(sv.point_lights) + light_tree_node_offset(sv.point_light_count));
 }
 
+
+#define TR_EMITTER_MAX 16
+struct alignas(16) EmitterSet { float planes[24]; uint count, pad[3]; uint index[TR_EMITTER_MAX]; };
+static_assert(sizeof(EmitterSet) == 176 && sizeof(TriRecord) % 16 == 0, "emitter set layout");
+TR_HD const EmitterSet* emitter_set(const SceneView& sv) { return reinterpret_cast<const EmitterSet*>(sv.tris + sv.tri_count); }
+
 }
diff --git a/tauray_amd/csrc/path_tracer.hip b/tauray_amd/csrc/path_tracer.hip
--- a/tauray_amd/csrc/path_tracer.hip
+++ b/tauray_amd/csrc/path_tracer.hip
@@ -17,6 +17,9 @@
 #endif
 #ifndef TR_SHADOW_WAVES
 #define TR_SHADOW_WAVES 8
+#endif
+#ifndef TR_TERMINAL_WAVES
+#define TR_TERMINAL_WAVES TR_CLOSEST_WAVES
 #endif
 #ifndef TR_CLOSEST_WAVES_2L
 #define TR_CLOSEST_WAVES_2L 5
@@ -138,6 +141,91 @@
         const uint slot = lane < size ? off + lane : 0xFFFFFFFFu;
         if (g < chunks_c) closest_lane<false, TWO_LEVEL>(sv, P, pb, bounce, queue, slot == 0xFFFFFFFFu ? slot : (g << 6) + slot, nc, s_stack + threadIdx.x, qc, st, overflow, max_vis, closest_rays);
         else shadow_lane<false, TWO_LEVEL>(sv, P, pb, slot == 0xFFFFFFFFu ? slot : ((g - chunks_c) << 6) + slot, ns, s_stack + threadIdx.x, qc, st, overflow, shadow_rays);
+    }
+    flush_trace_counters<false>(P, pb, overflow, 3000 + bounce, closest_rays, shadow_rays, st, max_vis);
+}
+
+
+template <bool COUNT, bool SOLO, bool WIDE = true>
+__global__ __launch_bounds__(KB, TR_TERMINAL_WAVES) void k_trace_closest_terminal(SceneView sv, PtParams P, PathBuffers pb, int bounce, const uint* queue, uint* bc,
+                                                                                   uint* next_queue) {
+    if (!WIDE) sv.wide_textures = 0;
+    __shared__ int s_stack_rows[TR_STACK_WORDS];
+    int* const s_stack = s_stack_rows + TR_STACK_ROW0;
+    __shared__ int s_owner[(KB / 64) * TR_OWNER_WORDS];
+    TL(__shared__ uint s_tl[(KB / 64) * TL_WORDS]; for (uint i = threadIdx.x; i < (KB / 64) * TL_WORDS; i += KB) s_tl[i] = 0; __syncthreads();)
+    const QuadCtx qc = make_quad_ctx(s_stack, s_owner, pb TL(, s_tl));
+    const uint n = bc[BC_QUEUE];
+    TerminalCounts tc = {0u, 0u};
+    TraceStats st = {};
+    uint rays = 0, max_vis = 0;
+    int overflow = 0;
+    const uint wave_id = (blockIdx.x * KB + threadIdx.x) >> 6, n_waves = (gridDim.x * KB) >> 6;
+    bool first = true;
+    while (true) {
+        uint base = 0;
+        if (first) base = wave_id * 64u;
+        else {
+            if (n <= n_waves * 64u) break;
+            if ((threadIdx.x & 63) == 0) base = n_waves * 64u + atomicAdd(&bc[BC_CUR_CLOSEST], 64u);
+            base = __shfl(base, 0);
+        }
+        first = false;
+        if (base >= n) break;
+        closest_lane<COUNT, false, true>(sv, P, pb, bounce, queue, base + (threadIdx.x & 63), n, s_stack + threadIdx.x, qc, st, overflow, max_vis, rays, next_queue,
+                                         &bc[BC_STRIDE + BC_QUEUE], &tc);
+    }
+    flush_trace_counters<COUNT>(P, pb, overflow, 1000 + bounce, rays, 0u, st, max_vis);
+    if (COUNT) flush_terminal_counters(P, pb, tc);
+    TL(__syncthreads(); for (uint i = threadIdx.x; i < (KB / 64) * TL_WORDS; i += KB) if (s_tl[i]) atomicAdd(&g_timeline[i % TL_WORDS], (unsigned long long)s_tl[i]);)
+}
+
+template <bool WIDE>
+__global__ __launch_bounds__(KB, TR_TERMINAL_WAVES) void k_trace_fused_terminal(SceneView sv, PtParams P, PathBuffers pb, int bounce, const uint* queue, uint* bc, uint* bc_prev,
+                                                                                 uint* next_queue) {
+    if (!WIDE) sv.wide_textures = 0;
+    __shared__ int s_stack_rows[TR_STACK_WORDS];
+    int* const s_stack = s_stack_rows + TR_STACK_ROW0;
+    __shared__ int s_owner[(KB / 64) * TR_OWNER_WORDS];
+    const QuadCtx qc = make_quad_ctx(s_stack, s_owner, pb);
+    const uint nc = bc[BC_QUEUE], ns = bc_prev[BC_SHADOW];
+    const uint chunks_c = (nc + 63u) >> 6, total = chunks_c + ((ns + 63u) >> 6);
+    TraceStats st = {};
+    uint closest_rays = 0, shadow_rays = 0, max_vis = 0;
+    int overflow = 0;
+    const uint wave_id = (blockIdx.x * KB + threadIdx.x) >> 6, n_waves = (gridDim.x * KB) >> 6;
+#if TR_TAIL_PIECES
+    const uint dyn = total > n_waves ? total - n_waves : 0u;
+    const uint tail16 = dyn < n_waves / TR_TAIL16_DIV ? dyn : n_waves / TR_TAIL16_DIV;
+    const uint tail32 = dyn - tail16 < n_waves / TR_TAIL32_DIV ? dyn - tail16 : n_waves / TR_TAIL32_DIV;
+    const uint full = total - tail16 - tail32, pieces = full + 2u * tail32 + 4u * tail16;
+#else
+    const uint pieces = total;
+#endif
+    bool first = true;
+    while (true) {
+        uint p = 0;
+        if (first) p = wave_id;
+        else {
+            if (pieces <= n_waves) break;
+            if ((threadIdx.x & 63) == 0) p = n_waves + atomicAdd(&bc[BC_CUR_CLOSEST], 1u);
+            p = __shfl(p, 0);
+        }
+        first = false;
+        if (p >= pieces) break;
+        uint g = p, off = 0u, size = 64u;
+#if TR_TAIL_PIECES
+        if (p >= full) {
+            const uint q = p - full;
+            if (q < 2u * tail32) { g = full + (q >> 1); off = (q & 1u) << 5; size = 32u; }
+            else { const uint r = q - 2u * tail32; g = full + tail32 + (r >> 2); off = (r & 3u) << 4; size = 16u; }
+        }
+#endif
+        const uint lane = threadIdx.x & 63;
+        const uint slot = lane < size ? off + lane : 0xFFFFFFFFu;
+        if (g < chunks_c) closest_lane<false, false, true>(sv, P, pb, bounce, queue, slot == 0xFFFFFFFFu ? slot : (g << 6) + slot, nc, s_stack + threadIdx.x, qc, st, overflow, max_vis, closest_rays,
+                                                           next_queue, &bc[BC_STRIDE + BC_QUEUE]);
+        else shadow_lane<false, false>(sv, P, pb, slot == 0xFFFFFFFFu ? slot : ((g - chunks_c) << 6) + slot, ns, s_stack + threadIdx.x, qc, st, overflow, shadow_rays);
     }
     flush_trace_counters<false>(P, pb, overflow, 3000 + bounce, closest_rays, shadow_rays, st, max_vis);
 }
@@ -612,6 +700,9 @@
     }
     const bool count = count_work != 0;
     const bool two_level = scene->two_level;
+    const int tq_in_effect = terminal_query_in_effect();
+    if (tq_in_effect < 0) return set_error("trhip_pt_render: TRHIP_TERMINAL_QUERY is not auto or off");
+    const bool terminal_query = tq_in_effect != 0;
     const Program prog = choose_program();
     const bool wide = prog.wide, cli_set = prog.cli_set, shade_fast = prog.shade_fast;
     const SpecKernels *spec_shade = prog.shade, *spec_raygen = prog.raygen;
@@ -832,10 +923,19 @@
                     const uint* q = bounce == 0 ? nullptr : lb.queue[bounce & 1];
                     uint* qn = lb.queue[(bounce + 1) & 1];
                     uint* bc = lb.bounce + BC_STRIDE * bounce;
-                    if (fused && bounce > 0) {
+                    const bool tq = terminal_query && bounce == opt.max_bounces - 1;
+                    if (fused && tq) {
+                        hipLaunchKernelGGL((wide ? k_trace_fused_terminal<true> : k_trace_fused_terminal<false>), dim3(blocks_f), dim3(KB), 0, ls, sv, LP, lb, bounce, q, bc, bc - BC_STRIDE, qn);
+                    } else if (fused && bounce > 0) {
                         hipLaunchKernelGGL((two_level ? k_trace_fused<true, true> : (wide ? k_trace_fused<true> : k_trace_fused<false>)), dim3(blocks_f), dim3(KB), 0, ls, sv, LP, lb, bounce, q, bc, bc - BC_STRIDE);
                     } else {
                         timed(T_CLOSEST, ls, [&] {
+                            if (tq) {
+                                auto kt = count ? k_trace_closest_terminal<true, false> : (timing ? (wide ? k_trace_closest_terminal<false, true, true> : k_trace_closest_terminal<false, true, false>)
+                                                                                                  : (wide ? k_trace_closest_terminal<false, false, true> : k_trace_closest_terminal<false, false, false>));
+                                hipLaunchKernelGGL(kt, dim3(std::min(blocks_all, closest_cap)), dim3(KB), 0, ls, sv, LP, lb, bounce, q, bc, qn);
+                                return;
+                            }
                             auto kc = two_level ? (count ? k_trace_closest<true, false, true, true> : k_trace_closest<false, false, true, true>)
                                     : count ? k_trace_closest<true, false> : (timing ? (wide ? k_trace_closest<false, true, true> : k_trace_closest<false, true, false>)
                                                                                      : (wide ? k_trace_closest<false, false, true> : k_trace_closest<false, false, false>));
@@ -853,7 +953,8 @@
 #endif
                         static const bool last_variant = !(getenv("TRHIP_SHADE_LAST") && atoi(getenv("TRHIP_SHADE_LAST")) == 0);
                         const bool last = last_variant && bounce == opt.max_bounces - 1;
-                        launch_shade(count, last, blocks_s, ls, LP, lb, bounce, q, bc, qn);
+                        if (tq) launch_shade(count, last, blocks_s, ls, LP, lb, bounce, qn, bc + BC_STRIDE, const_cast<uint*>(q));
+                        else launch_shade(count, last, blocks_s, ls, LP, lb, bounce, q, bc, qn);
                     });
                     if (bounce == 0 && first_hit_targets && s == opt.samples_per_pass - 1 && LP.samples_accumulated + LP.previous_samples == 0)
                         hipLaunchKernelGGL(k_first_hit_gbuffer, dim3(blocks_all), dim3(KB), 0, ls, sv, LP, lb);
@@ -990,6 +1091,35 @@
     return 0;
 }
 
+int PtStage::terminal_query_in_effect() const {
+    int mode = terminal_query;
+    if (mode < 0) {
+        const char* e = getenv("TRHIP_TERMINAL_QUERY");
+        std::string v = e ? e : "";
+        for (char& c : v) c = (char)tolower((unsigned char)c);
+        if (v.empty() || v == "auto") mode = TRHIP_TERMINAL_QUERY_AUTO;
+        else if (v == "off") mode = TRHIP_TERMINAL_QUERY_OFF;
+        else return -1;
+    }
+    if (mode != TRHIP_TERMINAL_QUERY_AUTO) return 0;
+    return (!direct && opt.max_bounces >= 2 && scene->accel_built && !scene->two_level && scene->tris && scene->emitter_count <= TR_EMITTER_MAX &&
+            scene->sphere_light_count() == 0) ? 1 : 0;
+}
+
+int PtStage::get_terminal_counters(trhip_terminal_counters* out, hipStream_t stream) {
+    memset(out, 0, sizeof(*out));
+    out->in_effect = terminal_query_in_effect() > 0 ? 1u : 0u;
+    out->emitter_triangles = scene->emitter_count;
+    out->threshold = TR_EMITTER_MAX;
+    if (!impl->pb.counters) return 0;
+    HIPCHK(hipStreamSynchronize(stream));
+    uint hl[PT_LANES][CNT_WORDS];
+    HIPCHK(hipMemcpy(hl, impl->pb.counters, sizeof(hl), hipMemcpyDeviceToHost));
+    auto rd = [&](int i) { uint64_t v = 0; for (int l = 0; l < PT_LANES; ++l) v += (uint64_t)hl[l][i] | ((uint64_t)hl[l][i + 1] << 32); return v; };
+    out->blocked_rays = rd(CNT_TQ_BLOCKED); out->fallback_rays = rd(CNT_TQ_FALLBACK);
+    return 0;
+}
+
 int PtStage::reset_counters() {
     if (impl->pb.counters) HIPCHK(hipMemset(impl->pb.counters, 0, PT_LANES * CNT_WORDS * sizeof(uint)));
     if (int rc = resolve_pending()) return rc;
diff --git a/tauray_amd/csrc/pt.h b/tauray_amd/csrc/pt.h
--- a/tauray_amd/csrc/pt.h
+++ b/tauray_amd/csrc/pt.h
@@ -20,7 +20,9 @@
     int get_timings(trhip_timings* out);
     int get_phase_counters(trhip_phase_counters* out, hipStream_t stream);
     int get_light_counters(trhip_light_counters* out, hipStream_t stream);
+    int get_terminal_counters(trhip_terminal_counters* out, hipStream_t stream);
     int get_program(trhip_program_info* out);
+    int terminal_query_in_effect() const;
 
     DeviceScene* scene;
     trhip_pt_options opt;
@@ -38,6 +40,7 @@
     uint frame_batch = 1;
     int ieee_shading = -1;
     int specialize = -1;
+    int terminal_query = -1;
     bool direct = false;
     hipStream_t last_stream = nullptr;
 
diff --git a/tauray_amd/csrc/pt_state.h b/tauray_amd/csrc/pt_state.h
--- a/tauray_amd/csrc/pt_state.h
+++ b/tauray_amd/csrc/pt_state.h
@@ -37,7 +37,7 @@
 
 enum { BC_QUEUE = 0, BC_SHADOW = 64, BC_CUR_CLOSEST = 128, BC_CUR_SHADOW = 192, BC_STRIDE = 256 };
 enum { CNT_OVERFLOW = 2, CNT_CLOSEST = 4, CNT_SHADOWRAYS = 6, CNT_NODES = 8, CNT_TRIS = 10, CNT_ALPHA = 12, CNT_SURF = 14, CNT_MAXVIS = 16, CNT_DBG = 17,
-       CNT_MAXSP = 30, CNT_CNODES = 32, CNT_PH_NODE = 34, CNT_PH_TRI = 36, CNT_PH_NODE16 = 38, CNT_PH_NODE8 = 40, CNT_LV_NODE16 = 42, CNT_PH_QNODE = 44, CNT_PH_QTRI = 46, CNT_PH_HIST = 48, CNT_LTESTS = 64, CNT_LNODES = 66, CNT_LFALLBACKS = 68, CNT_WORDS = 70 };
+       CNT_MAXSP = 30, CNT_CNODES = 32, CNT_PH_NODE = 34, CNT_PH_TRI = 36, CNT_PH_NODE16 = 38, CNT_PH_NODE8 = 40, CNT_LV_NODE16 = 42, CNT_PH_QNODE = 44, CNT_PH_QTRI = 46, CNT_PH_HIST = 48, CNT_LTESTS = 64, CNT_LNODES = 66, CNT_LFALLBACKS = 68, CNT_TQ_BLOCKED = 70, CNT_TQ_FALLBACK = 72, CNT_WORDS = 74 };
 
 struct PtParams {
     trhip_pt_options opt;
diff --git a/tauray_amd/csrc/trace.h b/tauray_amd/csrc/trace.h
--- a/tauray_amd/csrc/trace.h
+++ b/tauray_amd/csrc/trace.h
@@ -64,6 +64,15 @@
 #else
 #define TR_LEAF_MEMBERS(ref, more) constexpr uint member = 0;
 #endif
+
+struct TerminalRay { bool early, blocked; };
+#define TR_HIT_BLOCKED (-2)
+
+TR_DEV bool terminal_early_ok(float bsdf_pdf, f3 attenuation) {
+    const float lo = 9.094947017729282e-13f, hi = 1099511627776.0f;
+    const bool pdf_ok = bsdf_pdf == 0.0f || (bsdf_pdf >= lo && bsdf_pdf <= hi);
+    return pdf_ok && fabsf(attenuation.x) <= hi && fabsf(attenuation.y) <= hi && fabsf(attenuation.z) <= hi;
+}
 
 struct TriHit { float t, bu, bv; uint inst_flags, prim, alpha; };
 
diff --git a/tauray_amd/csrc/trace_lanes.h b/tauray_amd/csrc/trace_lanes.h
--- a/tauray_amd/csrc/trace_lanes.h
+++ b/tauray_amd/csrc/trace_lanes.h
@@ -7,13 +7,36 @@
 
 namespace {
 
-template <bool COUNT, bool TWO_LEVEL = false>
+struct TerminalCounts { uint blocked, fallback; };
+template <bool COUNT, bool TWO_LEVEL = false, bool TERMINAL = false>
 TR_DEV void closest_lane(const SceneView& sv, const PtParams& P, const PathBuffers& pb, int bounce, const uint* queue, uint qi, uint n, int* lds_stack,
-                         const QuadCtx& qc, TraceStats& st, int& overflow, uint& max_vis, uint& rays) {
+                         const QuadCtx& qc, TraceStats& st, int& overflow, uint& max_vis, uint& rays, uint* next_queue = nullptr, uint* next_count = nullptr,
+                         TerminalCounts* tc = nullptr) {
     bool valid = qi < n;
     uint id = 0;
     u4 misc = {0, 0, 0, 1};
     f4 o = F4(0), d = F4(0);
+    if constexpr (TERMINAL) {
+        f4 a = F4(0);
+        if (valid) { id = queue[qi]; misc = pb.misc[id]; o = pb.org_pdf[id]; d = pb.dir_reg[id]; a = pb.atten_alpha[id]; }
+        for (int b = 0; b < bounce; ++b) pcg(misc.x);
+        TerminalRay term = {valid && terminal_early_ok(o.w, F3(a)), false};
+        HitRecord hit;
+        const uint before = st.nodes;
+        trace_closest_wave4<0, COUNT, false, true>(sv, valid, F3(o), F3(d), P.opt.min_ray_dist, __builtin_huge_valf(), misc.x, lds_stack, qc, hit, st, overflow, &term);
+        if (COUNT) st.cnodes += st.nodes - before;
+        const bool keep = valid && !term.blocked;
+        const uint slot = wave_append(next_count, keep);
+        if (keep) {
+            next_queue[slot] = id;
+            pb.hit[id] = make_int4(hit.instance_id, hit.primitive_id, __float_as_int(hit.u), __float_as_int(hit.v));
+        }
+        if (valid) {
+            rays++;
+            if (COUNT) { tc->blocked += term.blocked ? 1u : 0u; tc->fallback += term.early ? 0u : 1u; }
+        }
+        return;
+    }
     TL(const unsigned long long tl_chunk = tl_now();)
     if (valid) { id = queue ? queue[qi] : qi + P.id_offset; misc = pb.misc[id]; o = pb.org_pdf[id]; d = pb.dir_reg[id]; valid = !(misc.w & 1u); }
     TL(tl_data_arrived(); tl_misc(qc.tl, 3, tl_now() - tl_chunk);)
@@ -94,6 +117,16 @@
     shadow_ray<COUNT, TWO_LEVEL>(sv, P, pb, valid, o, d, [&] { return pb.sh_contrib[qi]; }, [&] { return pb.sh_lobes[qi]; }, lds_stack, qc, st, overflow, rays);
 }
 
+TR_DEV void flush_terminal_counters(const PtParams& P, const PathBuffers& pb, TerminalCounts tc) {
+    if (!P.count_work) return;
+    for (int off = 32; off > 0; off >>= 1) { tc.blocked += __shfl_xor(tc.blocked, off); tc.fallback += __shfl_xor(tc.fallback, off); }
+    if ((threadIdx.x & 63) == 0) {
+        add64(pb.counters, CNT_SURF, tc.blocked);
+        add64(pb.counters, CNT_TQ_BLOCKED, tc.blocked);
+        add64(pb.counters, CNT_TQ_FALLBACK, tc.fallback);
+    }
+}
+
 template <bool COUNT>
 TR_DEV void flush_trace_counters(const PtParams& P, const PathBuffers& pb, int overflow, int overflow_tag, uint closest_rays, uint shadow_rays,
                                  TraceStats st, uint max_vis) {
diff --git a/tauray_amd/csrc/trace_quad.h b/tauray_amd/csrc/trace_quad.h
--- a/tauray_amd/csrc/trace_quad.h
+++ b/tauray_amd/csrc/trace_quad.h
@@ -8,6 +8,12 @@
 #endif
 #ifndef TR_QUAD_VOTE
 #define TR_QUAD_VOTE 4
+#endif
+#ifndef TR_TERMINAL_SLOT_ORDER
+#define TR_TERMINAL_SLOT_ORDER 1
+#endif
+#ifndef TR_TERMINAL_QUADS
+#define TR_TERMINAL_QUADS 1
 #endif
 #define TR_QSPILL TR_SPILL_STACK
 static_assert(TR_QUAD_SWITCH <= 16, "a wave has sixteen quads");
@@ -204,9 +210,10 @@
     else { qs.sp--; qnode = qs.load(qs.sp); }
 }
 
-template <int ALPHA_MODE, bool COUNT, bool TWO_LEVEL = false>
+template <int ALPHA_MODE, bool COUNT, bool TWO_LEVEL = false, bool TERMINAL = false>
 TR_DEV void trace_closest_wave4(const SceneView& sv, bool valid, f3 org, f3 dir, float tmin, float tmax, uint seed,
-                                int* lds_stack, const QuadCtx& qc, HitRecord& hit, TraceStats& st, int& overflow) {
+                                int* lds_stack, const QuadCtx& qc, HitRecord& hit, TraceStats& st, int& overflow, TerminalRay* term = nullptr) {
+    static_assert(!(TERMINAL && TWO_LEVEL), "the terminal query walks the all-merged structure");
     hit.instance_id = -1; hit.primitive_id = -1; hit.u = 0; hit.v = 0; hit.t = -1.0f;
     if constexpr (TWO_LEVEL) {
         if (valid) trace_closest4_2l<ALPHA_MODE, COUNT>(sv, org, dir, tmin, tmax, seed, lds_stack, hit, st, overflow);
@@ -223,9 +230,21 @@
     int node = sv.node_count > 0 ? 0 : -1;
     TL(const unsigned long long tl_enter = tl_now(), tl_wall0 = tl_wall();)
 
-    auto consider = [&](const TriHit& tr, float t, float bu, float bv) {
+    auto consider = [&](const TriHit& tr, float t, float bu, float bv) -> bool {
         const uint inst = tr.inst_flags & 0x7FFFFFFFu;
         const bool closer = t < best_t || (t == best_t && best_inst != 0xFFFFFFFFu && (inst < best_inst || (inst == best_inst && tr.prim < best_prim)));
+        if constexpr (TERMINAL) {
+            bool accept = closer;
+            if (accept && (tr.inst_flags & 0x80000000u)) {
+                if (COUNT) st.alpha++;
+                const float a = candidate_alpha(sv, tr.alpha, bu, bv);
+                const float cutoff = ALPHA_MODE == 0 ? alpha_cutoff_hash(seed, (int)inst, (int)tr.prim) : 0.0001f;
+                accept = !(a <= cutoff);
+            }
+            best_t = accept ? t : best_t; best_u = accept ? bu : best_u; best_v = accept ? bv : best_v;
+            best_inst = accept ? inst : best_inst; best_prim = accept ? tr.prim : best_prim;
+            return accept;
+        }
         if (closer) {
             bool accept = true;
             if (tr.inst_flags & 0x80000000u) {
@@ -236,11 +255,34 @@
             }
             if (accept) { best_t = t; best_inst = inst; best_prim = tr.prim; best_u = bu; best_v = bv; }
         }
+        return false;
     };
+
+    bool early = false, blocked = false;
+    if constexpr (TERMINAL) {
+        early = term->early;
+        const EmitterSet* es = emitter_set(sv);
+        const uint n_emit = es->count;
+        if (n_emit > 0 && live) {
+            const char* base = reinterpret_cast<const char*>(es);
+            const float nx = *reinterpret_cast<const float*>(base + r.nkx), fx = *reinterpret_cast<const float*>(base + (r.nkx ^ 16u));
+            const float ny = *reinterpret_cast<const float*>(base + r.nky), fy = *reinterpret_cast<const float*>(base + (r.nky ^ 16u));
+            const float nz = *reinterpret_cast<const float*>(base + r.nkz), fz = *reinterpret_cast<const float*>(base + (r.nkz ^ 16u));
+            const float t0 = fmaxf(fmaxf((nx - r.op.x) * r.ip.x, (ny - r.op.y) * r.ip.y), fmaxf((nz - r.op.z) * r.ip.z, tmin));
+            const float t1 = fminf(fminf(fminf((fx - r.op.x) * r.ip.x, (fy - r.op.y) * r.ip.y), (fz - r.op.z) * r.ip.z), tmax) * TR_SLAB_PAD;
+            if (t0 <= t1) {
+                for (uint e = 0; e < n_emit; ++e) {
+                    TriHit tr;
+                    if (COUNT) st.tris++;
+                    if (tri_intersect(r, sv.tris, es->index[e], tmin, __builtin_huge_valf(), tr)) consider(tr, tr.t, tr.bu, tr.bv);
+                }
+            }
+        }
+    }
 
     while (true) {
         const unsigned long long act = __ballot(live);
-        if (__popcll(act) <= TR_QUAD_SWITCH) break;
+        if (__popcll(act) <= ((TERMINAL && !TR_TERMINAL_QUADS) ? 0 : TR_QUAD_SWITCH)) break;
         if (live) {
             const bool at_leaf = node < 0;
 #if TR_VOTE > 0
@@ -263,6 +305,8 @@
                     Hit4 h;
                     box4_intersect(r, sv.nodes4, node, tmin, best_t, h TL(, &tlp));
                     if (COUNT) st.nodes++;
+                    if constexpr (TERMINAL && TR_TERMINAL_SLOT_ORDER) descend = shadow_descend(h, stk, spill, node);
+                    else {
                     TR_CE4(0, 1) TR_CE4(2, 3) TR_CE4(0, 2) TR_CE4(1, 3) TR_CE4(1, 2)
                     TL(asm volatile("" : "+v"(h.t[0]), "+v"(h.t[1]), "+v"(h.t[2]), "+v"(h.t[3]), "+v"(h.c[0]), "+v"(h.c[1]), "+v"(h.c[2]), "+v"(h.c[3])); tlp.mark_a();)
                     if (h.t[0] < __builtin_huge_valf()) {
@@ -271,6 +315,7 @@
                         if (COUNT) st.maxsp = max(st.maxsp, (uint)stk.sp);
                         node = h.c[0];
                         descend = true;
+                    }
                     }
                 } else {
                     TriHit tr;
@@ -282,13 +327,17 @@
                     tlp.mark_b();
 #else
                     TR_LEAF_MEMBERS((uint)~node, true)
-                    if (tri_intersect(r, sv.tris, leaf_index((uint)~node) + member, tmin, __builtin_huge_valf(), tr)) consider(tr, tr.t, tr.bu, tr.bv);
+                    if (tri_intersect(r, sv.tris, leaf_index((uint)~node) + member, tmin, __builtin_huge_valf(), tr)) {
+                        const bool took = consider(tr, tr.t, tr.bu, tr.bv);
+                        if constexpr (TERMINAL) blocked = blocked || (took && early);
+                    }
 #endif
                 }
                 if (!descend) {
                     if (stk.sp == 0) live = false;
                     else node = stk.pop(spill);
                 }
+                if constexpr (TERMINAL) live = live && !blocked;
                 TL(tlp.end(qc.tl, leaf_phase ? TL_LT : TL_LN, tl_units, (tl_units - 1) >> 3, leaf_phase ? TL_LT_WAIT_HIST : TL_LN_WAIT_HIST);)
             }
         }
@@ -311,6 +360,8 @@
         float qbest = lt;
         bool qlive = deal.has_ray;
         int pend = -1;
+        const bool qearly = TERMINAL ? bperm(src, early ? 1 : 0) != 0 : false;
+        bool qblocked = false;
 #if TR_TAIL_PREFETCH
         int qpf = 0;
 #endif
@@ -324,6 +375,7 @@
             const bool tri_phase = __popcll(__ballot(pend >= 0)) >= TR_QUAD_VOTE || __ballot(can_node) == 0;
             if (COUNT && (threadIdx.x & 63) == 0) { if (tri_phase) st.ph_qtri++; else st.ph_qnode++; }
             if (tri_phase) {
+                bool took = false;
                 if (pend >= 0) {
                     TL(TlPhase tlp; const int tl_units = __popcll(__ballot(true)); tlp.begin();)
                     TriHit tr;
@@ -341,10 +393,16 @@
                         }
                         lt = accept ? t : lt; lu = accept ? bu : lu; lv = accept ? bv : lv;
                         linst = accept ? inst : linst; lprim = accept ? tr.prim : lprim;
+                        if constexpr (TERMINAL) took = accept;
                     }
                     TL(tlp.end(qc.tl, TL_QT, tl_units, (tl_units - 1) >> 3, -1);)
                 }
                 pend = -1;
+                if constexpr (TERMINAL) {
+                    int z = took ? 1 : 0;
+                    z |= qrot1(z); z |= qrot2(z);
+                    if (z != 0 && qearly) { qblocked = true; qlive = false; }
+                }
                 float m = lt;
                 m = fminf(m, qrot1f(m)); m = fminf(m, qrot2f(m));
                 qbest = fminf(qbest, m);
@@ -384,7 +442,12 @@
         const uint ri = (uint)bperm(back, (int)linst), rp = (uint)bperm(back, (int)lprim);
         const int ro = bperm(back, qo);
         if (live) { best_t = rt; best_u = ru; best_v = rv; best_inst = ri; best_prim = rp; overflow += ro; }
-    }
+        if constexpr (TERMINAL) {
+            const int rb = bperm(back, qblocked ? 1 : 0);
+            if (live) blocked = blocked || rb != 0;
+        }
+    }
+    if constexpr (TERMINAL) term->blocked = blocked;
     overflow += stk.overflow ? 1 : 0;
     TL(tl_misc(qc.tl, 0, 1); tl_misc(qc.tl, 1, tl_now() - tl_enter); tl_misc(qc.tl, 4, tl_wall() - tl_wall0);)
 
diff --git a/tauray_amd/renderer.py b/tauray_amd/renderer.py
--- a/tauray_amd/renderer.py
+++ b/tauray_amd/renderer.py
@@ -8,7 +8,7 @@
 import numpy as np
 
 from . import _lib
-from ._lib import (AccelInfoC, AccelLayoutC, CountersC, DistributionC, LightAccelInfoC, LightCountersC, PtOptionsC, SceneDescC, TimingsC,
+from ._lib import (AccelInfoC, AccelLayoutC, CountersC, DistributionC, LightAccelInfoC, LightCountersC, PtOptionsC, TerminalCountersC, SceneDescC, TimingsC,
                    TonemapInfoC, TrhipError, check)
 from .distribution import (DISTRIBUTION_DUPLICATE, DISTRIBUTION_SCANLINE, DISTRIBUTION_SHUFFLED_STRIPS, DistributionParams,
                            get_device_distribution_params, get_distribution_target_size)
@@ -338,6 +338,25 @@
                                              1 if include_lights else 0, d_hits.ptr, None))
         return d_hits.download((n,), hit_dtype)
 
+    def trace_terminal(self, rays: np.ndarray, seeds: Optional[np.ndarray] = None, fallback: Optional[np.ndarray] = None) -> np.ndarray:
+        rays = np.ascontiguousarray(rays, dtype=np.float32).reshape(-1, 8)
+        n = len(rays)
+        hit_dtype = np.dtype([("instance_id", "<i4"), ("primitive_id", "<i4"), ("bary_u", "<f4"), ("bary_v", "<f4"), ("t", "<f4")])
+        if n == 0:
+            return np.zeros(0, dtype=hit_dtype)
+        d_rays = self.ctx.alloc(rays.nbytes).upload(rays)
+        d_seeds = d_fb = None
+        if seeds is not None:
+            seeds = np.ascontiguousarray(seeds, dtype=np.uint32)
+            d_seeds = self.ctx.alloc(seeds.nbytes).upload(seeds)
+        if fallback is not None:
+            fallback = np.ascontiguousarray(fallback, dtype=np.uint32)
+            d_fb = self.ctx.alloc(fallback.nbytes).upload(fallback)
+        d_hits = self.ctx.alloc(n * 20)
+        check(_lib.lib().trhip_trace_terminal(self.ctx.h, n, d_rays.ptr, d_seeds.ptr if d_seeds else None, d_fb.ptr if d_fb else None,
+                                              d_hits.ptr, None))
+        return d_hits.download((n,), hit_dtype)
+
     def trace_shadow(self, rays: np.ndarray) -> np.ndarray:
         rays = np.ascontiguousarray(rays, dtype=np.float32).reshape(-1, 8)
         n = len(rays)
@@ -443,6 +462,14 @@
         c = LightCountersC()
         check(_lib.lib().trhip_pt_get_light_counters(self.h, C.byref(c)))
         return {n: int(getattr(c, n)) for n, _ in LightCountersC._fields_}
+
+    def set_terminal_query(self, mode: int):
+        check(_lib.lib().trhip_pt_set_terminal_query(self.h, mode))
+
+    def terminal_counters(self) -> dict:
+        c = TerminalCountersC()
+        check(_lib.lib().trhip_pt_get_terminal_counters(self.h, C.byref(c)))
+        return {n: int(getattr(c, n)) for n, _ in TerminalCountersC._fields_ if n != "pad"}
 
     def timings(self) -> dict:
         t = TimingsC()
```
